# davidnabergoj/nfmc

Hardware: AMD Instinct MI355X
Metric: chain-steps/sec (n_chains x iters / s), jump_mala + RealNVP, d=64 (higher is better)
Workload: dtype f32

## Files before the change

### include/nfmc_hip.h

```cpp
#ifndef NFMC_HIP_H
#define NFMC_HIP_H

#include <stdint.h>

#ifdef __cplusplus
extern "C" {
#endif

typedef void* nfmc_stream_t;

#define NFMC_ABI_VERSION 4

enum {
    NFMC_OK = 0,
    NFMC_EINVAL = -1,
    NFMC_ESHAPE = -2,
    NFMC_EALIGN = -3,
    NFMC_EUNSUPPORTED = -4,
    NFMC_ESCRATCH = -5
};

enum {
    NFMC_POT_QUADRATIC = 0,
    NFMC_POT_FUNNEL = 1,
    NFMC_POT_GAUSSIAN_MIXTURE = 2,
    NFMC_POT_LOGISTIC_REGRESSION = 3,
    NFMC_POT_GAUSSIAN_FULL = 4,
    NFMC_POT_ROSENBROCK = 5,
    NFMC_POT_STOCHASTIC_VOLATILITY = 6,
    NFMC_POT_SPARSE_LOGISTIC_REGRESSION = 7,
    NFMC_POT_LATTICE_PHI4 = 8,
    NFMC_POT_ITEM_RESPONSE = 9,
    NFMC_POT_VARYING_EFFECTS = 10,
    NFMC_POT_PARTICLES = 11,
    NFMC_POT_LATENT_GAUSSIAN = 12
};

typedef struct {
    int32_t kind;
    int32_t n_components;
    const float* a;
    const float* b;
    float a_scalar;
    float b_scalar;
} NfmcPotential;

typedef struct {
    uint64_t seed;
    uint64_t chain_offset;
    uint32_t step0;
    uint32_t rounds;
    const float* replay_normals;
    const float* replay_uniforms;
} NfmcRng;

enum { NFMC_CNT_ACCEPTED = 0, NFMC_CNT_ATTEMPTED = 1, NFMC_CNT_NONFINITE = 2, NFMC_CNT_WORDS = 4 };

typedef struct {
    double* sum_x;
    double* sum_x2;
    unsigned long long* counters;
    double* scratch;
    int64_t scratch_bytes;
    int32_t defer;
    int32_t tail_slot;
} NfmcStats;

int64_t nfmc_stats_scratch_bytes(int32_t d);

int nfmc_stats_fold_f32(const NfmcStats* stats, int32_t d, uint64_t attempted, unsigned long long* jump_counters,
                        uint64_t jump_attempted, nfmc_stream_t stream);

typedef struct {
    int32_t d;
    int32_t n_coupling;
    int32_t n_hidden;
    int32_t n_hidden_layers;
    float min_scale;
    int32_t n_bins;
    const float* ea0_log_scale;
    const float* ea0_shift;
    const float* ea1_log_scale;
    const float* ea1_shift;
    const float* weights;
    int64_t layer_stride;
    float spline_bound;
    int32_t reserved;
    float* scratch;
    int64_t scratch_bytes;
} NfmcRealNVP;

int64_t nfmc_flow_scratch_bytes(const NfmcRealNVP* flow, int64_t n, int32_t with_gradient);

int32_t nfmc_realnvp_padded_hidden(int32_t n_hidden);
int64_t nfmc_realnvp_layer_floats(int32_t d, int32_t n_hidden, int32_t n_hidden_layers);
int64_t nfmc_coupling_layer_floats(int32_t d, int32_t n_hidden, int32_t n_hidden_layers, int32_t n_bins);

typedef struct {
    float* base;
    int32_t stride;
    int32_t countdown;
    int32_t ring_rows;
    int32_t row;
} NfmcSampleStore;

enum {
    NFMC_TUNE_STEP_SIZE = 0,
    NFMC_TUNE_LOG_SMOOTH = 1,
    NFMC_TUNE_ERROR_SUM = 2,
    NFMC_TUNE_ITERATION = 3,
    NFMC_TUNE_ANCHOR = 4,
    NFMC_TUNE_LOG_RAW = 5,
    NFMC_TUNE_TARGET = 6,
    NFMC_TUNE_KAPPA = 7,
    NFMC_TUNE_GAMMA = 8,
    NFMC_TUNE_IMD_ADJUSTMENT = 9,
    NFMC_TUNE_TICKET = 10,
    NFMC_TUNE_WORDS = 12
};
typedef struct {
    double* state;
    float* inv_mass_diag;
    int32_t tune_step_size;
    int32_t tune_inv_mass_diag;
    int32_t every;
    int32_t reserved;
} NfmcTune;
int64_t nfmc_tune_state_doubles(int32_t d);

int nfmc_sampler_layout(int32_t d, int32_t pot_kind, int32_t* cpl, int32_t* lpc);

typedef struct {
    NfmcRealNVP flow;
    int32_t adjusted;
    int32_t reserved;
    unsigned long long* counters;
    const float* replay_latent;
    const float* replay_uniform;
    uint8_t* mask_out;
    float* log_ratio_out;
} NfmcJumpTail;

typedef struct {
    float* x;
    int64_t n;
    int32_t d;
    int32_t n_steps;
    float step_size;
    int32_t adjust;
    const float* inv_mass_diag;
    NfmcPotential pot;
    NfmcRng rng;
    NfmcStats stats;
    NfmcSampleStore samples;
    uint8_t* masks_out;
    float* log_ratio_out;
    const NfmcJumpTail* jump;
    NfmcTune tune;
} NfmcMalaArgs;

int nfmc_mala_steps_f32(const NfmcMalaArgs* args, nfmc_stream_t stream);

typedef struct {
    float* x;
    int64_t n;
    int32_t d;
    int32_t n_steps;
    float step_size;
    int32_t n_leapfrog;
    int32_t adjust;
    int32_t reserved;
    const float* inv_mass_diag;
    NfmcPotential pot;
    NfmcRng rng;
    NfmcStats stats;
    NfmcSampleStore samples;
    uint8_t* masks_out;
    float* log_ratio_out;
    const NfmcJumpTail* jump;
    NfmcTune tune;
} NfmcHmcArgs;

int nfmc_hmc_steps_f32(const NfmcHmcArgs* args, nfmc_stream_t stream);

int nfmc_realnvp_forward_f32(const NfmcRealNVP* flow, const float* x, int64_t n, float* z, float* logdet,
                             float* log_prob, nfmc_stream_t stream);

int nfmc_realnvp_inverse_f32(const NfmcRealNVP* flow, const float* z, int64_t n, float* x, float* logdet,
                             float* log_q, const NfmcRng* rng, nfmc_stream_t stream);

typedef struct {
    float* x;
    float* logq;
    int64_t n;
    int32_t n_steps;
    int32_t logq_cached;
    int32_t adjusted;
    int32_t reserved;
    NfmcRealNVP flow;
    NfmcPotential pot;
    NfmcRng rng;
    NfmcStats stats;
    NfmcSampleStore samples;
    uint8_t* masks_out;
    float* log_ratio_out;
} NfmcFlowMhArgs;

int nfmc_flow_mh_steps_f32(const NfmcFlowMhArgs* args, nfmc_stream_t stream);

int nfmc_flow_mh_supported_f32(const NfmcFlowMhArgs* args);

enum { NFMC_INNER_MALA = 0, NFMC_INNER_HMC = 1 };
#define NFMC_JUMP_RUN_MAX_PARTS 4
typedef struct {
    int32_t inner_kind;
    int32_t n_parts;
    const void* inner;
    const NfmcFlowMhArgs* jump;
    int32_t n_outer;
    int32_t n_inner;
} NfmcJumpRun;

int nfmc_jump_run_f32(const NfmcJumpRun* run, nfmc_stream_t stream);

#define NFMC_IMH_PARALLEL_MAX_STEPS 65536
int64_t nfmc_imh_parallel_work_bytes(int64_t n, int32_t d, int32_t n_steps);
int nfmc_imh_parallel_f32(const NfmcFlowMhArgs* args, void* work, int64_t work_bytes, nfmc_stream_t stream);
int nfmc_imh_parallel_supported_f32(const NfmcFlowMhArgs* args);

typedef struct {
    float* z;
    int64_t n;
    int32_t n_steps;
    int32_t n_leapfrog;
    float step_size;
    int32_t adjust;
    const float* inv_mass_diag;
    NfmcRealNVP flow;
    NfmcPotential pot;
    NfmcRng rng;
    NfmcStats stats;
    NfmcSampleStore samples;
    uint8_t* masks_out;
    float* log_ratio_out;
    float* scratch;
    int64_t scratch_bytes;
} NfmcNeutraHmcArgs;

int64_t nfmc_neutra_scratch_bytes(int64_t n, int32_t d, int32_t n_hidden, int32_t n_hidden_layers, int32_t n_coupling);

int nfmc_neutra_hmc_steps_f32(const NfmcNeutraHmcArgs* args, nfmc_stream_t stream);

int nfmc_neutra_potential_grad_f32(const NfmcRealNVP* flow, const NfmcPotential* pot, const float* z, int64_t n,
                                   float* u_out, float* grad_out, nfmc_stream_t stream);

typedef struct {
    NfmcRealNVP flow;
    const float* x;
    int64_t n;
    float* grad_out;
    float* logq_out;
} NfmcFlowLogqGradArgs;

int nfmc_flow_logq_grad_f32(const NfmcFlowLogqGradArgs* args, nfmc_stream_t stream);
int nfmc_flow_logq_grad_supported_f32(const NfmcFlowLogqGradArgs* args);

typedef struct {
    NfmcRealNVP flow;
    NfmcPotential pot;
    float* x;
    const float* grad_u;
    float* logq_out;
    int64_t n;
    float step_size;
    int32_t reserved;
} NfmcDlmcStepArgs;

int nfmc_dlmc_step_f32(const NfmcDlmcStepArgs* args, nfmc_stream_t stream);
int nfmc_dlmc_step_supported_f32(const NfmcDlmcStepArgs* args);

typedef struct {
    float* x;
    const float* x_prime;
    int64_t n;
    int32_t d;
    int32_t n_carry;
    const float* log_ratio;
    const float* uniforms;
    float* carry[2];
    const float* carry_prime[2];
    NfmcRng rng;
    int32_t rng_tag;
    int32_t reserved;
    NfmcStats stats;
    uint8_t* mask_out;
} NfmcSelectArgs;

int nfmc_mh_accept_select_f32(const NfmcSelectArgs* args, nfmc_stream_t stream);

int nfmc_langevin_propose_f32(const float* x, const float* grad_u, const float* inv_mass_diag, float step_size,
                              int64_t n, int32_t d, const NfmcRng* rng, float* x_prime, nfmc_stream_t stream);
int nfmc_langevin_log_ratio_f32(const float* x, const float* x_prime, const float* u, const float* u_prime,
                                const float* grad_u, const float* grad_u_prime, const float* inv_mass_diag,
                                float step_size, int64_t n, int32_t d, float* log_ratio, nfmc_stream_t stream);

int nfmc_moments_update_f32(const float* x, int64_t rows, int32_t d, const NfmcStats* stats, nfmc_stream_t stream);

int nfmc_philox_normals_f32(const NfmcRng* rng, int32_t tag, int64_t n, int32_t d, float* out, nfmc_stream_t stream);
int nfmc_philox_uniforms_f32(const NfmcRng* rng, int32_t tag, int64_t n, float* out, nfmc_stream_t stream);

#define NFMC_MAX_STEPS_PER_CALL 512
typedef struct {
    float lr, beta1, beta2, eps, weight_decay;
    int32_t step;
} NfmcAdamW;

typedef struct {
    NfmcRealNVP flow;
    float* params;
    float* adam_m;
    float* adam_v;
    int64_t n_params;
    int64_t ea_off;
    float* partial;
    int64_t partial_floats;
    float* status;
    const float* x_val;
    int64_t n_val;
    float* params_prev;
    float* best;
    float* run_state;
    float* scratch;
    int64_t scratch_bytes;
} NfmcFlowFit;

typedef struct {
    int32_t n_epochs;
    int32_t early_stopping;
    int32_t early_stopping_threshold;
    int32_t keep_best_weights;
    int32_t skip_nonfinite;
    int32_t reserved;
} NfmcFitControl;
enum {
    NFMC_FIT_BEST_LOSS = 0,
    NFMC_FIT_SINCE_BEST = 1,
    NFMC_FIT_APPLIED = 2,
    NFMC_FIT_STOPPED = 3,
    NFMC_FIT_DIVERGED = 4,
    NFMC_FIT_LAST_LOSS = 5,
    NFMC_FIT_LAST_VAL = 6,
    NFMC_FIT_BOOKED = 7,
    NFMC_FIT_STATE_FLOATS = 8
};

int nfmc_flow_fit_supported_f32(const NfmcRealNVP* flow);
int64_t nfmc_flow_fit_partial_floats(int64_t n, int64_t n_params);
int64_t nfmc_flow_fit_workspace(const NfmcRealNVP* flow, int64_t n, int64_t n_val, int64_t n_params, int64_t* partial_floats);
int nfmc_flow_fit_step_f32(const NfmcFlowFit* fit, const float* x, int64_t n, const NfmcAdamW* opt, nfmc_stream_t stream);
int nfmc_flow_variational_fit_step_f32(const NfmcFlowFit* fit, const NfmcPotential* pot, const float* z, int64_t n,
                                       const NfmcAdamW* opt, nfmc_stream_t stream);
int nfmc_flow_fit_epochs_f32(const NfmcFlowFit* fit, const NfmcPotential* pot, const float* x, int64_t n,
                             int64_t epoch_stride, const NfmcAdamW* opt, const NfmcFitControl* ctl, int32_t first_call,
                             int32_t n_calls, nfmc_stream_t stream);

#define NFMC_BLOB_MAX_PIECES 16
typedef struct {
    float* param;
    int64_t vec_off;
    int32_t rows, cols;
    int32_t vec_row_stride, vec_col_stride;
} NfmcBlobPiece;
int nfmc_flow_blob_copy_f32(float* vec, const NfmcBlobPiece* pieces, int32_t n_pieces, int32_t to_vector, nfmc_stream_t stream);

#define NFMC_PRP_ROUNDS 6
int nfmc_rows_sample_f32(const float* x, int64_t n, int32_t d, uint64_t seed, int64_t first, float* out, int64_t m,
                         int64_t* index_out, nfmc_stream_t stream);
int64_t nfmc_rows_sample_index(int64_t n, uint64_t seed, int64_t i);

typedef struct {
    int32_t abi_version;
    int32_t max_d_sampler;
    int32_t max_d_flow;
    int32_t max_hidden_valu;
    int32_t max_hidden;
    int32_t max_steps_per_call;
} NfmcLimits;

int nfmc_limits(NfmcLimits* out);
const char* nfmc_error_string(int code);
const char* nfmc_build_digest(void);

#ifdef __cplusplus
}
#endif
#endif
```

### nfmc_amd/csrc/misc_kernels.hip

```cpp
#include "common.hpp"

namespace nfmc {

__global__ void __launch_bounds__(kBlock) philox_normals_kernel(NfmcRng rng, uint32_t tag, int64_t n, int d, int nblk,
                                                                float* __restrict__ out) {
    const int64_t total = n * nblk;
    for (int64_t t = (int64_t)blockIdx.x * kBlock + threadIdx.x; t < total; t += (int64_t)gridDim.x * kBlock) {
        const int64_t row = t / nblk;
        const int blk = (int)(t - row * nblk);
        float z[4];
        if (rng.rounds == 7)
            philox_normal4<7>((uint32_t)(rng.chain_offset + (uint64_t)row), rng.step0, (uint32_t)blk, tag, (uint32_t)rng.seed,
                              (uint32_t)(rng.seed >> 32), z);
        else
            philox_normal4<10>((uint32_t)(rng.chain_offset + (uint64_t)row), rng.step0, (uint32_t)blk, tag, (uint32_t)rng.seed,
                               (uint32_t)(rng.seed >> 32), z);
#pragma unroll
        for (int k = 0; k < 4; ++k)
            if (4 * blk + k < d) out[row * d + 4 * blk + k] = z[k];
    }
}

__device__ __forceinline__ float stream_uniform(const NfmcRng& rng, uint32_t tag, int64_t row) {
    const uint32_t gchain = (uint32_t)(rng.chain_offset + (uint64_t)row);
    const uint32_t k0 = (uint32_t)rng.seed, k1 = (uint32_t)(rng.seed >> 32);
    const bool r7 = rng.rounds == 7;
    if (tag == kTagAccept) {
        const uint4 r = r7 ? philox4x32<7>(gchain, rng.step0 >> 2, 0u, kTagAccept, k0, k1)
                           : philox4x32<10>(gchain, rng.step0 >> 2, 0u, kTagAccept, k0, k1);
        return u32_to_uniform(pick_word(r, rng.step0 & 3u));
    }
    const uint4 r = r7 ? philox4x32<7>(gchain, rng.step0, 0u, tag, k0, k1) : philox4x32<10>(gchain, rng.step0, 0u, tag, k0, k1);
    return u32_to_uniform(r.x);
}

__global__ void __launch_bounds__(kBlock) philox_uniforms_kernel(NfmcRng rng, uint32_t tag, int64_t n,
                                                                 float* __restrict__ out) {
    for (int64_t row = (int64_t)blockIdx.x * kBlock + threadIdx.x; row < n; row += (int64_t)gridDim.x * kBlock)
        out[row] = stream_uniform(rng, tag, row);
}

__global__ void __launch_bounds__(kBlock) moments_kernel(const float* __restrict__ x, int64_t rows, int d, int dp,
                                                         double* __restrict__ scratch) {
    const int64_t per = (rows + gridDim.x - 1) / gridDim.x;
    const int64_t r0 = (int64_t)blockIdx.x * per;
    const int64_t r1 = r0 + per < rows ? r0 + per : rows;
    double* out = scratch + (size_t)blockIdx.x * (2 * dp + kStatTail);
    for (int c = threadIdx.x; c < dp; c += kBlock) {
        double s = 0.0, s2 = 0.0;
        if (c < d)
            for (int64_t r = r0; r < r1; ++r) {
                const float v = x[r * d + c];
                s += (double)v;
                s2 += (double)v * (double)v;
            }
        out[c] = s;
        out[dp + c] = s2;
    }
    if (threadIdx.x < kStatTail) out[2 * dp + threadIdx.x] = 0.0;
}

template <int CPL, int LPC>
__global__ void __launch_bounds__(kBlock) select_kernel(NfmcSelectArgs a, int64_t tiles) {
    constexpr int CPW = kWave / LPC;
    const int lane = threadIdx.x & 63, wave = threadIdx.x >> 6;
    const int g = lane % LPC, cw = lane / LPC;
    const int d = a.d;
    float sx[CPL], sxx[CPL];
#pragma unroll
    for (int i = 0; i < CPL; ++i) sx[i] = sxx[i] = 0.f;
    uint32_t n_acc = 0, n_bad = 0;
    for (int64_t tile = blockIdx.x; tile < tiles; tile += gridDim.x) {
        const int64_t row = (tile * kWavesPerBlock + wave) * CPW + cw;
        const bool active = row < a.n;
        bool accept = active;
        if (a.log_ratio && active) {
            const float lr = a.log_ratio[row];
            const float u = a.uniforms ? a.uniforms[row] : stream_uniform(a.rng, (uint32_t)a.rng_tag, row);
            accept = fast_ln(u) < lr;
            if (g == 0 && !(fabsf(lr) <= 3.0e38f)) n_bad++;
        }
        float x[CPL], xp[CPL];
        load_row<CPL, LPC, false>(a.x, row, d, g, active, x);
        load_row<CPL, LPC, false>(a.x_prime, row, d, g, active, xp);
        const uint64_t am = __ballot(accept);
#pragma unroll
        for (int i = 0; i < CPL; ++i) {
            x[i] = select_f32(am, xp[i], x[i]);
            sx[i] += x[i];
            sxx[i] = fmaf(x[i], x[i], sxx[i]);
        }
        if (accept) store_row<CPL, LPC, false>(a.x, row, d, g, true, x);
        if (g == 0 && active) {
            if (accept) {
                n_acc++;
                for (int k = 0; k < a.n_carry; ++k) a.carry[k][row] = a.carry_prime[k][row];
            }
            if (a.mask_out) a.mask_out[row] = accept ? 1 : 0;
        }
    }
    for (int m = 1; m < kWave; m <<= 1) {
        n_acc += __shfl_xor(n_acc, m, kWave);
        n_bad += __shfl_xor(n_bad, m, kWave);
    }
    if (a.stats.sum_x) block_stats_flush<CPL, LPC>(sx, sxx, n_acc, n_bad, a.stats);
}

__global__ void __launch_bounds__(kBlock) langevin_propose_kernel(const float* __restrict__ x,
                                                                  const float* __restrict__ grad_u,
                                                                  const float* __restrict__ imd, float h, float sqrt2h,
                                                                  int64_t n, int d, NfmcRng rng,
                                                                  float* __restrict__ x_prime) {
    const int nblk = (d + 3) / 4;
    const int64_t total = n * nblk;
    for (int64_t t = (int64_t)blockIdx.x * kBlock + threadIdx.x; t < total; t += (int64_t)gridDim.x * kBlock) {
        const int64_t row = t / nblk;
        const int blk = (int)(t - row * nblk);
        float z[4];
        if (rng.replay_normals) {
#pragma unroll
            for (int k = 0; k < 4; ++k) z[k] = (4 * blk + k < d) ? rng.replay_normals[row * d + 4 * blk + k] : 0.f;
        } else {
            philox_normal4((uint32_t)(rng.chain_offset + (uint64_t)row), rng.step0, (uint32_t)blk, kTagNoise,
                           (uint32_t)rng.seed, (uint32_t)(rng.seed >> 32), z);
        }
#pragma unroll
        for (int k = 0; k < 4; ++k) {
            const int c = 4 * blk + k;
            if (c < d) {
                const float m = imd ? imd[c] : 1.f;
                const int64_t o = row * d + c;
                x_prime[o] = fmaf(sqrt2h / m, z[k], fmaf((-h) / (m * m), grad_u[o], x[o]));
            }
        }
    }
}

__global__ void __launch_bounds__(kBlock) langevin_log_ratio_kernel(
    const float* __restrict__ x, const float* __restrict__ xp, const float* __restrict__ u,
    const float* __restrict__ up, const float* __restrict__ gu, const float* __restrict__ gup,
    const float* __restrict__ imd, float h, int64_t n, int d, float* __restrict__ out) {
    const int lane = threadIdx.x & 63;
    const int64_t wid = ((int64_t)blockIdx.x * kBlock + threadIdx.x) >> 6;
    const int64_t nw = ((int64_t)gridDim.x * kBlock) >> 6;
    const float inv4h = 1.f / (4.f * h);
    for (int64_t row = wid; row < n; row += nw) {
        float acc = 0.f;
        for (int c = lane; c < d; c += kWave) {
            const float m = imd ? imd[c] : 1.f;
            const float A = 1.f / (m * m);
            const int64_t o = row * d + c;
            const float tf = (xp[o] - x[o]) + h * A * gu[o];
            const float tb = (x[o] - xp[o]) + h * A * gup[o];
            acc += inv4h * (1.f / A) * (tf * tf - tb * tb);
        }
        acc = group_allreduce<64>(acc);
        if (lane == 0) out[row] = (u[row] - up[row]) + acc;
    }
}

static int grid_for(int64_t work_items) {
    int64_t g = (work_items + kBlock - 1) / kBlock;
    return (int)(g < 1 ? 1 : (g > kMaxGrid ? kMaxGrid : g));
}

}

using namespace nfmc;

extern "C" int nfmc_philox_normals_f32(const NfmcRng* rng, int32_t tag, int64_t n, int32_t d, float* out,
                                       nfmc_stream_t stream) {
    if (!rng || !out || n <= 0 || d <= 0 || !rng_rounds_ok(*rng, true)) return NFMC_EINVAL;
    const int nblk = (d + 3) / 4;
    hipLaunchKernelGGL(philox_normals_kernel, dim3(grid_for(n * nblk)), dim3(kBlock), 0, (hipStream_t)stream, *rng,
                       (uint32_t)tag, n, d, nblk, out);
    NFMC_HIP_CHECK_LAUNCH();
    return NFMC_OK;
}

extern "C" int nfmc_philox_uniforms_f32(const NfmcRng* rng, int32_t tag, int64_t n, float* out, nfmc_stream_t stream) {
    if (!rng || !out || n <= 0 || !rng_rounds_ok(*rng, true)) return NFMC_EINVAL;
    if (tag != (int)kTagAccept && tag != (int)kTagJump) return NFMC_EINVAL;
    hipLaunchKernelGGL(philox_uniforms_kernel, dim3(grid_for(n)), dim3(kBlock), 0, (hipStream_t)stream, *rng,
                       (uint32_t)tag, n, out);
    NFMC_HIP_CHECK_LAUNCH();
    return NFMC_OK;
}

extern "C" int nfmc_moments_update_f32(const float* x, int64_t rows, int32_t d, const NfmcStats* stats,
                                       nfmc_stream_t stream) {
    if (!x || !stats || !stats->sum_x || !stats->sum_x2 || !stats->counters || !stats->scratch) return NFMC_EINVAL;
    if (rows <= 0 || d <= 0) return NFMC_EINVAL;
    if (d > 1024) return NFMC_ESHAPE;
    const int dp = padded_d(d);
    int grid = (int)(rows < 1024 ? (rows + 3) / 4 : 256);
    if (grid < 1) grid = 1;
    if (stats->scratch_bytes < (int64_t)grid * (2 * dp + kStatTail) * (int64_t)sizeof(double)) return NFMC_ESCRATCH;
    if (stats->defer) return NFMC_EUNSUPPORTED;
    hipStream_t st = (hipStream_t)stream;
    hipLaunchKernelGGL(moments_kernel, dim3(grid), dim3(kBlock), 0, st, x, rows, (int)d, dp, stats->scratch);
    NFMC_HIP_CHECK_LAUNCH();
    hipLaunchKernelGGL(stats_finish_kernel<true>, dim3(stats_finish_grid(dp)), dim3(kFinishBlock), 0, st, stats->scratch, grid, dp, (int)d, *stats, 0ull);
    NFMC_HIP_CHECK_LAUNCH();
    return NFMC_OK;
}

extern "C" int nfmc_stats_fold_f32(const NfmcStats* stats, int32_t d, uint64_t attempted,
                                   unsigned long long* jump_counters, uint64_t jump_attempted, nfmc_stream_t stream) {
    if (!stats || !stats->sum_x || !stats->sum_x2 || !stats->counters || !stats->scratch) return NFMC_EINVAL;
    if (d <= 0) return NFMC_EINVAL;
    if (d > 1024) return NFMC_ESHAPE;
    const int dp = padded_d(d);
    if (stats->scratch_bytes < stats_scratch_doubles(dp) * (int64_t)sizeof(double)) return NFMC_ESCRATCH;
    hipLaunchKernelGGL(stats_finish_kernel<true>, dim3(stats_finish_grid(dp)), dim3(kFinishBlock), 0, (hipStream_t)stream,
                       stats->scratch, kMaxGrid, dp, (int)d, *stats, (unsigned long long)attempted, jump_counters,
                       (unsigned long long)jump_attempted);
    NFMC_HIP_CHECK_LAUNCH();
    return NFMC_OK;
}

template <int CPL, int LPC>
static void launch_select(const NfmcSelectArgs& a, int64_t tiles, int grid, hipStream_t st) {
    hipLaunchKernelGGL((select_kernel<CPL, LPC>), dim3(grid), dim3(kBlock), 0, st, a, tiles);
}

extern "C" int nfmc_mh_accept_select_f32(const NfmcSelectArgs* args, nfmc_stream_t stream) {
    if (!args || !args->x || !args->x_prime) return NFMC_EINVAL;
    NfmcSelectArgs a = *args;
    if (a.n <= 0 || a.d <= 0 || a.n_carry < 0 || a.n_carry > 2) return NFMC_EINVAL;
    if (int rr = rng_default_only(a.rng)) return rr;
    if (a.d > 1024) return NFMC_ESHAPE;
    for (int k = 0; k < a.n_carry; ++k)
        if (!a.carry[k] || !a.carry_prime[k]) return NFMC_EINVAL;
    if (a.stats.sum_x && (!a.stats.sum_x2 || !a.stats.counters || !a.stats.scratch)) return NFMC_EINVAL;
    if (a.rng_tag != (int)kTagAccept && a.rng_tag != (int)kTagJump) return NFMC_EINVAL;
    const int dp = padded_d(a.d);
    const int lpc = dp / 4 > 64 ? 64 : dp / 4;
    const int cpl = dp / lpc;
    const int cpw = kWave / lpc;
    const int64_t tiles = (a.n + (int64_t)kWavesPerBlock * cpw - 1) / ((int64_t)kWavesPerBlock * cpw);
    const int grid = (int)(tiles < kMaxGrid ? tiles : kMaxGrid);
    if (a.stats.sum_x && a.stats.scratch_bytes < (int64_t)grid * (2 * dp + kStatTail) * (int64_t)sizeof(double))
        return NFMC_ESCRATCH;
    if (check_defer(a.stats, dp, a.d)) return NFMC_EINVAL;
    hipStream_t st = (hipStream_t)stream;
    if (cpl == 4) {
        switch (lpc) {
            case 1: launch_select<4, 1>(a, tiles, grid, st); break;
            case 2: launch_select<4, 2>(a, tiles, grid, st); break;
            case 4: launch_select<4, 4>(a, tiles, grid, st); break;
            case 8: launch_select<4, 8>(a, tiles, grid, st); break;
            case 16: launch_select<4, 16>(a, tiles, grid, st); break;
            case 32: launch_select<4, 32>(a, tiles, grid, st); break;
            default: launch_select<4, 64>(a, tiles, grid, st); break;
        }
    } else if (cpl == 8) {
        launch_select<8, 64>(a, tiles, grid, st);
    } else {
        launch_select<16, 64>(a, tiles, grid, st);
    }
    NFMC_HIP_CHECK_LAUNCH();
    if (a.stats.sum_x && !a.stats.defer) {
        hipLaunchKernelGGL(stats_finish_kernel<true>, dim3(stats_finish_grid(dp)), dim3(kFinishBlock), 0, st, a.stats.scratch, grid, dp, a.d, a.stats,
                           (unsigned long long)a.n);
        NFMC_HIP_CHECK_LAUNCH();
    }
    return NFMC_OK;
}

extern "C" int nfmc_langevin_propose_f32(const float* x, const float* grad_u, const float* inv_mass_diag,
                                         float step_size, int64_t n, int32_t d, const NfmcRng* rng, float* x_prime,
                                         nfmc_stream_t stream) {
    if (!x || !grad_u || !rng || !x_prime || n <= 0 || d <= 0 || !(step_size > 0.f)) return NFMC_EINVAL;
    if (int rr = rng_default_only(*rng)) return rr;
    const float sqrt2h = (float)sqrt(2.0 * (double)step_size);
    hipLaunchKernelGGL(langevin_propose_kernel, dim3(grid_for(n * ((d + 3) / 4))), dim3(kBlock), 0, (hipStream_t)stream,
                       x, grad_u, inv_mass_diag, step_size, sqrt2h, n, (int)d, *rng, x_prime);
    NFMC_HIP_CHECK_LAUNCH();
    return NFMC_OK;
}

extern "C" int nfmc_langevin_log_ratio_f32(const float* x, const float* x_prime, const float* u, const float* u_prime,
                                           const float* grad_u, const float* grad_u_prime, const float* inv_mass_diag,
                                           float step_size, int64_t n, int32_t d, float* log_ratio,
                                           nfmc_stream_t stream) {
    if (!x || !x_prime || !u || !u_prime || !grad_u || !grad_u_prime || !log_ratio) return NFMC_EINVAL;
    if (n <= 0 || d <= 0 || !(step_size > 0.f)) return NFMC_EINVAL;
    hipLaunchKernelGGL(langevin_log_ratio_kernel, dim3(grid_for(n * 64)), dim3(kBlock), 0, (hipStream_t)stream, x,
                       x_prime, u, u_prime, grad_u, grad_u_prime, inv_mass_diag, step_size, n, (int)d, log_ratio);
    NFMC_HIP_CHECK_LAUNCH();
    return NFMC_OK;
}

extern "C" int nfmc_limits(NfmcLimits* out) {
    if (!out) return NFMC_EINVAL;
    out->abi_version = NFMC_ABI_VERSION;
    out->max_d_sampler = 1024;
    out->max_d_flow = 512;
    out->max_hidden_valu = 32;
    out->max_hidden = 128;
    out->max_steps_per_call = NFMC_MAX_STEPS_PER_CALL;
    return NFMC_OK;
}

extern "C" const char* nfmc_error_string(int code) {
    switch (code) {
        case NFMC_OK: return "ok";
        case NFMC_EINVAL: return "invalid argument (NULL pointer or non-positive size)";
        case NFMC_ESHAPE: return "shape outside the supported range (see nfmc_limits)";
        case NFMC_EALIGN: return "pointer alignment";
        case NFMC_EUNSUPPORTED: return "no kernel for this request";
        case NFMC_ESCRATCH: return "statistics scratch buffer too small (nfmc_stats_scratch_bytes)";
        default: return code > 0 ? hipGetErrorString((hipError_t)code) : "unknown nfmc error";
    }
}
```

### nfmc_amd/csrc/sampler_impl.hpp

```cpp
#pragma once

#include "flow_b.hpp"

namespace nfmc {

template <int CPL, int LPC, bool FAST>
struct MassCoef {
    float c1_s, c2_s, hA_s, cg_s, kap_s;
    float c1[FAST ? 1 : CPL], c2[FAST ? 1 : CPL], hA[FAST ? 1 : CPL], invA[FAST ? 1 : CPL];
    float m[FAST ? 1 : CPL], rs[FAST ? 1 : CPL], cg[FAST ? 1 : CPL], kap[FAST ? 1 : CPL];

    template <class PotT>
    __device__ __forceinline__ void init_quadratic(const PotT& pot, bool rw) {
        cg_s = rw ? 0.f : c1_s * (2.f * pot.aa(0));
        kap_s = rw ? pot.aa(0) : pot.aa(0) * pot.aa(0) * hA_s;
        if constexpr (!FAST) {
#pragma unroll
            for (int i = 0; i < CPL; ++i) {
                cg[i] = rw ? 0.f : c1[i] * (2.f * pot.aa(i));
                kap[i] = rw ? pot.aa(i) : pot.aa(i) * pot.aa(i) * hA[i];
            }
        }
    }
    __device__ __forceinline__ float CG(int i) const { return FAST ? cg_s : cg[FAST ? 0 : i]; }
    __device__ __forceinline__ float KAP(int i) const { return FAST ? kap_s : kap[FAST ? 0 : i]; }

    __device__ __forceinline__ void init(float h, float sqrt2h, const float* __restrict__ imd, int g, int d,
                                         bool rw = false) {
        c1_s = rw ? 0.f : -h;
        c2_s = rw ? 1.f : sqrt2h;
        hA_s = h;
        if constexpr (!FAST) {
#pragma unroll
            for (int i = 0; i < CPL; ++i) {
                const int c = coord_of<CPL, LPC>(g, i);
                const bool ok = c < d;
                const float mm = (ok && imd) ? imd[c] : 1.f;
                const float A = 1.f / (mm * mm);
                c1[i] = (ok && !rw) ? (-h) / (mm * mm) : 0.f;
                c2[i] = ok ? (rw ? mm : sqrt2h / mm) : 0.f;
                hA[i] = ok ? h * A : 0.f;
                invA[i] = ok ? 1.f / A : 0.f;
                m[i] = ok ? mm : 0.f;
                rs[i] = ok ? 1.f / sqrtf(mm) : 0.f;
            }
        }
    }
    __device__ __forceinline__ float C1(int i) const { return FAST ? c1_s : c1[FAST ? 0 : i]; }
    __device__ __forceinline__ float C2(int i) const { return FAST ? c2_s : c2[FAST ? 0 : i]; }
    __device__ __forceinline__ float HA(int i) const { return FAST ? hA_s : hA[FAST ? 0 : i]; }
    __device__ __forceinline__ float IA(int i) const { return FAST ? 1.f : invA[FAST ? 0 : i]; }
    __device__ __forceinline__ float M(int i) const { return FAST ? 1.f : m[FAST ? 0 : i]; }
    __device__ __forceinline__ float RS(int i) const { return FAST ? 1.f : rs[FAST ? 0 : i]; }
};

template <int CPL, int LPC, bool ON>
struct StatShift {
    float c[ON ? CPL : 1];
    __device__ __forceinline__ void init(const NfmcTune& tn, int g, int d, bool active) {
        if constexpr (ON) {
            const double* __restrict__ src = tn.state + NFMC_TUNE_WORDS + 2 * CPL * LPC + kStatTail;
#pragma unroll
            for (int i = 0; i < CPL; ++i) {
                const int k = coord_of<CPL, LPC>(g, i);
                c[i] = (active && k < d) ? (float)src[k] : 0.f;
            }
        }
    }
    __device__ __forceinline__ float operator()(const float (&x)[CPL], int i) const {
        if constexpr (ON) return x[i] - c[i];
        else return x[i];
    }
};

template <int CPL, int LPC, int R = 10, bool REPLAY = true>
__device__ __forceinline__ void draw_normals(const NfmcRng& rng, uint32_t tag, uint32_t gchain, int64_t row, int64_t n,
                                             int d, int g, int s, float (&e)[CPL]) {
    if (REPLAY && rng.replay_normals) {
        const float* p = rng.replay_normals + ((int64_t)s * n + row) * d;
#pragma unroll
        for (int i = 0; i < CPL; ++i) {
            const int c = coord_of<CPL, LPC>(g, i);
            e[i] = (row < n && c < d) ? p[c] : 0.f;
        }
    } else {
        const uint32_t k0 = (uint32_t)rng.seed, k1 = (uint32_t)(rng.seed >> 32);
#pragma unroll
        for (int b = 0; b < CPL / 4; ++b) {
            const uint4 r = philox4x32<R, true>(gchain, rng.step0 + (uint32_t)s, (uint32_t)(b * LPC + g), tag, k0, k1);
            const nfmc_f2 z0 = box_muller_pk(r.x, r.y), z1 = box_muller_pk(r.z, r.w);
            e[4 * b] = z0.x;
            e[4 * b + 1] = z0.y;
            e[4 * b + 2] = z1.x;
            e[4 * b + 3] = z1.y;
        }
    }
}

template <int LPC, int R = 10, bool REPLAY = true>
struct AcceptLnU {
    uint4 r;
    float4* mine;
    const float* chain;
    uint32_t base;
    __device__ __forceinline__ AcceptLnU(float4* slab, int g) {
        if constexpr (LPC > 1) {
            mine = slab + threadIdx.x;
            chain = reinterpret_cast<const float*>(slab + (threadIdx.x - g));
        }
    }
    __device__ __forceinline__ float draw(const NfmcRng& rng, uint32_t gchain, int64_t row, int64_t n, int g, int s) {
        if (REPLAY && rng.replay_uniforms) return fast_ln(row < n ? rng.replay_uniforms[(int64_t)s * n + row] : 0.5f);
        const uint32_t step = rng.step0 + (uint32_t)s, k0 = (uint32_t)rng.seed, k1 = (uint32_t)(rng.seed >> 32);
        if constexpr (LPC == 1) {
            if (s == 0 || (step & 3u) == 0u) r = philox4x32<R>(gchain, step >> 2, 0u, kTagAccept, k0, k1);
            return fast_ln(u32_to_uniform(pick_word(r, step & 3u)));
        } else {
            if (s == 0 || step - base == 4u * LPC || step == 0u) {
                base = step & ~3u;
                const uint4 w = philox4x32<R>(gchain, (base >> 2) + (uint32_t)g, 0u, kTagAccept, k0, k1);
                *mine = make_float4(fast_ln(u32_to_uniform(w.x)), fast_ln(u32_to_uniform(w.y)),
                                    fast_ln(u32_to_uniform(w.z)), fast_ln(u32_to_uniform(w.w)));
                __builtin_amdgcn_wave_barrier();
            }
            return chain[step - base];
        }
    }
};

struct JumpDev {
    NfmcRealNVP flow;
    int adjusted;
    const float* replay_latent;
    const float* replay_uniform;
    uint8_t* mask_out;
    float* log_ratio_out;
};

template <int CPL, int LPC, int HP, class FlowT, class PotT>
__device__ __forceinline__ bool jump_once(float (&x)[CPL], const FlowT& fl, const PotT& pot,
                                          const JumpDev& j, uint64_t seed, uint32_t step, uint32_t gchain, int64_t row,
                                          int64_t n, int d, int g, bool active, float& lr_out, bool& bad) {
    const bool revl = (j.flow.n_coupling & 1) != 0;
    float part;
    {
        const auto ctx = pot.prepare(x, g, d);
        float w[CPL];
        part = 0.f;
#pragma unroll
        for (int i = 0; i < CPL; ++i) {
            part += pot.term(ctx, i, x[i]);
            w[i] = x[i];
        }
        part += fl.forward(w);
#pragma unroll
        for (int i = 0; i < CPL; ++i) part = fmaf(-0.5f * w[i], w[i], part);
    }
    float xp[CPL];
    draw_latent<CPL, LPC>(xp, j.replay_latent, seed, step, gchain, row, n, d, g, revl);
#pragma unroll
    for (int i = 0; i < CPL; ++i) part = fmaf(0.5f * xp[i], xp[i], part);
    part += fl.inverse(xp);
    {
        const auto ctx = pot.prepare(xp, g, d);
#pragma unroll
        for (int i = 0; i < CPL; ++i) part -= pot.term(ctx, i, xp[i]);
    }
    const float lr = group_allreduce<LPC>(part);
    bool accept = true;
    bad = false;
    if (j.adjusted) {
        float u;
        if (j.replay_uniform) {
            u = active ? j.replay_uniform[row] : 0.5f;
        } else {
            const uint4 r = philox4x32_10(gchain, step, 0u, kTagJump, (uint32_t)seed, (uint32_t)(seed >> 32));
            u = u32_to_uniform(r.x);
        }
        accept = fast_ln(u) < lr;
        bad = active && !(fabsf(lr) <= 3.0e38f);
    }
    accept = accept && active;
    const uint64_t am = __ballot(accept);
#pragma unroll
    for (int i = 0; i < CPL; ++i) x[i] = select_f32(am, xp[i], x[i]);
    lr_out = lr;
    return accept;
}

template <int CPL, int LPC, template <int, int, bool> class Pot, bool FAST, int JHP, int RR = 10, bool LEAN = false,
          bool TUNE = false>
__global__ void __launch_bounds__(kBlock, NFMC_WPE) mala_kernel(NfmcMalaArgs a, float sqrt2h, int64_t tiles, JumpDev jd) {
    static_assert(!LEAN || JHP == 0, "the jump tail keeps its own outputs");
    static_assert(!TUNE || (JHP == 0 && !FAST && !LEAN), "tuning launches run the general kernels without a jump tail");
    extern __shared__ __attribute__((aligned(16))) float flow_lds[];
    __shared__ float4 accept_slab[LPC > 1 ? kBlock : 1];
    constexpr int CPW = kWave / LPC;
    const int lane = threadIdx.x & 63, wave = threadIdx.x >> 6;
    const int g = lane % LPC, cw = lane / LPC;
    const int d = a.d;
    const int64_t n = a.n;
    const double h_dev = a.tune.state ? a.tune.state[NFMC_TUNE_STEP_SIZE] : 0.0;
    const float h = a.tune.state ? (float)h_dev : a.step_size;
    if (a.tune.state) sqrt2h = (float)sqrt(2.0 * h_dev);
    const bool adjust = (a.adjust & 1) != 0, rw = (a.adjust & 2) != 0;
    const float inv4h = rw ? 0.f : 1.f / (4.f * h);

    MassCoef<CPL, LPC, FAST> mc;
    mc.init(h, sqrt2h, a.inv_mass_diag, g, d, rw);
    Pot<CPL, LPC, FAST> pot;
    if constexpr (!Pot<CPL, LPC, FAST>::kStaged) pot.init(a.pot, g, d);
    if constexpr (Pot<CPL, LPC, FAST>::kQuadratic) mc.init_quadratic(pot, rw);
    FlowB<CPL, LPC, JHP == 0 ? 4 : JHP, true, (FAST && CPL >= 8 && JHP > 0)> fl;
    if constexpr (JHP > 0) {
        decltype(fl)::Img::stage(flow_lds, jd.flow, kBlock);
        __syncthreads();
        fl.init(flow_lds, jd.flow, g);
    }
    if constexpr (Pot<CPL, LPC, FAST>::kStaged)
        init_staged(pot, a.pot, g, d, flow_lds,
                    JHP > 0 ? decltype(fl)::Img::total_floats(jd.flow.n_hidden_layers, jd.flow.n_coupling) : 0);

    float sx[CPL], sxx[CPL];
#pragma unroll
    for (int i = 0; i < CPL; ++i) sx[i] = sxx[i] = 0.f;
    StatShift<CPL, LPC, TUNE> shift;
    uint32_t n_acc = 0, n_bad = 0, j_acc = 0, j_bad = 0;
    constexpr unsigned long long leaders = group_leaders(LPC);

    for (int64_t tile = blockIdx.x; tile < tiles; tile += gridDim.x) {
        const int64_t row = (tile * kWavesPerBlock + wave) * CPW + cw;
        const bool active = row < n;
        const uint32_t gchain = (uint32_t)(a.rng.chain_offset + (uint64_t)row);
        float x[CPL];
        load_row<CPL, LPC, FAST>(a.x, row, d, g, active, x);
        shift.init(a.tune, g, d, active);
        AcceptLnU<LPC, RR, !LEAN> au(accept_slab, g);
        StoreCursor keep(a.samples);
        const uint64_t live = __ballot(active);
        float sq = 0.f, sq_prop = 0.f;
        if constexpr (Pot<CPL, LPC, FAST>::kQuadratic && FAST) {
#pragma unroll
            for (int i = 0; i < CPL; ++i) sq = fmaf(x[i], x[i], sq);
        }

        for (int s = 0; s < a.n_steps; ++s) {
            float e[CPL], xp[CPL];
            draw_normals<CPL, LPC, RR, !LEAN>(a.rng, kTagNoise, gchain, row, n, d, g, s, e);
            float lr = 0.f;
            if constexpr (Pot<CPL, LPC, FAST>::kQuadratic && FAST) {
                nfmc_f2 sp = {0.f, 0.f};
                const nfmc_f2 cg = {mc.CG(0), mc.CG(0)}, c2 = {mc.C2(0), mc.C2(0)};
#pragma unroll
                for (int i = 0; i < CPL; i += 2) {
                    const nfmc_f2 xi = {x[i], x[i + 1]}, ei = {e[i], e[i + 1]};
                    const nfmc_f2 p = __builtin_elementwise_fma(c2, ei, __builtin_elementwise_fma(cg, xi, xi));
                    xp[i] = p.x;
                    xp[i + 1] = p.y;
                    sp = __builtin_elementwise_fma(p, p, sp);
                }
                sq_prop = sp.x + sp.y;
                {
#pragma clang fp contract(off)
                    lr = mc.KAP(0) * (sq - sq_prop);
                }
            } else if constexpr (Pot<CPL, LPC, FAST>::kQuadratic) {
#pragma unroll
                for (int i = 0; i < CPL; ++i) {
                    const float t = x[i] - pot.bb(i);
                    xp[i] = fmaf(mc.C2(i), e[i], fmaf(mc.CG(i), t, x[i]));
                    const float tp = xp[i] - pot.bb(i);
                    lr = fmaf(mc.KAP(i) * (t - tp), t + tp, lr);
                }
            } else {
                const auto ctx = pot.prepare(x, g, d);
#pragma unroll
                for (int i = 0; i < CPL; ++i)
                    xp[i] = fmaf(mc.C2(i), e[i], fmaf(mc.C1(i), pot.grad(ctx, i, x[i]), x[i]));
                if (adjust) {
                    const auto ctxp = pot.prepare(xp, g, d);
#pragma unroll
                    for (int i = 0; i < CPL; ++i) {
                        const float gj = pot.grad(ctx, i, x[i]), gp = pot.grad(ctxp, i, xp[i]);
                        const float tf = (xp[i] - x[i]) + mc.HA(i) * gj;
                        const float tb = (x[i] - xp[i]) + mc.HA(i) * gp;
                        lr += (pot.term(ctx, i, x[i]) - pot.term(ctxp, i, xp[i])) +
                              inv4h * mc.IA(i) * (tf * tf - tb * tb);
                    }
                }
            }
            uint64_t am = live;
            if (adjust) {
                lr = group_allreduce<LPC, Pot<CPL, LPC, FAST>::kQuadratic && FAST>(lr);
                const float ln_u = au.draw(a.rng, gchain, row, n, g, s);
                am &= __ballot(ln_u < lr);
                n_bad += (uint32_t)__popcll(__ballot(!(fabsf(lr) <= 3.0e38f)) & live & leaders);
            }
            n_acc += (uint32_t)__popcll(am & leaders);
            if constexpr (Pot<CPL, LPC, FAST>::kQuadratic && FAST) assign_where<CPL>(am, x, xp, sq, sq_prop);
#pragma unroll
            for (int i = 0; i < CPL; ++i) {
                if constexpr (!(Pot<CPL, LPC, FAST>::kQuadratic && FAST)) x[i] = select_f32(am, xp[i], x[i]);
                const float xs = shift(x, i);
                sx[i] += xs;
                sxx[i] = fmaf(xs, xs, sxx[i]);
            }
            if constexpr (!LEAN) {
                if (float* kept = keep.next(n * d)) store_row<CPL, LPC, FAST>(kept, row, d, g, active, x);
                if (g == 0 && active) {
                    if (a.masks_out) a.masks_out[(int64_t)s * n + row] = (am >> lane) & 1u;
                    if (a.log_ratio_out) a.log_ratio_out[(int64_t)s * n + row] = lr;
                }
            }
        }
        if constexpr (JHP > 0) {
            float lr;
            bool bad;
            fl.launder();
            const bool acc = jump_once<CPL, LPC, JHP>(x, fl, pot, jd, a.rng.seed, a.rng.step0 + (uint32_t)a.n_steps, gchain,
                                                      row, n, d, g, active, lr, bad);
            j_acc += (uint32_t)__popcll(__ballot(acc) & leaders);
            j_bad += (uint32_t)__popcll(__ballot(bad) & leaders);
#pragma unroll
            for (int i = 0; i < CPL; ++i) {
                const float xs = shift(x, i);
                sx[i] += xs;
                sxx[i] = fmaf(xs, xs, sxx[i]);
            }
            if (float* kept = keep.next(n * d)) store_row<CPL, LPC, FAST>(kept, row, d, g, active, x);
            if (g == 0 && active) {
                if (jd.mask_out) jd.mask_out[row] = acc ? 1 : 0;
                if (jd.log_ratio_out) jd.log_ratio_out[row] = lr;
            }
        }
        store_row<CPL, LPC, FAST>(a.x, row, d, g, active, x);
    }
    if (a.stats.sum_x) block_stats_flush<CPL, LPC>(sx, sxx, n_acc, n_bad, a.stats, j_acc, j_bad);
}

template <int CPL, int LPC, template <int, int, bool> class Pot, bool FAST, int JHP, int RR = 10, bool TUNE = false>
__global__ void __launch_bounds__(kBlock, NFMC_WPE) hmc_kernel(NfmcHmcArgs a, int64_t tiles, JumpDev jd) {
    static_assert(!TUNE || (JHP == 0 && !FAST), "tuning launches run the general kernels without a jump tail");
    extern __shared__ __attribute__((aligned(16))) float flow_lds[];
    __shared__ float4 accept_slab[LPC > 1 ? kBlock : 1];
    constexpr int CPW = kWave / LPC;
    const int lane = threadIdx.x & 63, wave = threadIdx.x >> 6;
    const int g = lane % LPC, cw = lane / LPC;
    const int d = a.d;
    const int64_t n = a.n;
    const float h = a.tune.state ? (float)a.tune.state[NFMC_TUNE_STEP_SIZE] : a.step_size, hh = h / 2;

    MassCoef<CPL, LPC, FAST> mc;
    mc.init(h, 0.f, a.inv_mass_diag, g, d);
    Pot<CPL, LPC, FAST> pot;
    if constexpr (!Pot<CPL, LPC, FAST>::kStaged) pot.init(a.pot, g, d);
    FlowB<CPL, LPC, JHP == 0 ? 4 : JHP, true, (FAST && CPL >= 8 && JHP > 0)> fl;
    if constexpr (JHP > 0) {
        decltype(fl)::Img::stage(flow_lds, jd.flow, kBlock);
        __syncthreads();
        fl.init(flow_lds, jd.flow, g);
    }
    if constexpr (Pot<CPL, LPC, FAST>::kStaged)
        init_staged(pot, a.pot, g, d, flow_lds,
                    JHP > 0 ? decltype(fl)::Img::total_floats(jd.flow.n_hidden_layers, jd.flow.n_coupling) : 0);

    float sx[CPL], sxx[CPL];
#pragma unroll
    for (int i = 0; i < CPL; ++i) sx[i] = sxx[i] = 0.f;
    StatShift<CPL, LPC, TUNE> shift;
    uint32_t n_acc = 0, n_bad = 0, j_acc = 0, j_bad = 0;
    constexpr unsigned long long leaders = group_leaders(LPC);

    for (int64_t tile = blockIdx.x; tile < tiles; tile += gridDim.x) {
        const int64_t row = (tile * kWavesPerBlock + wave) * CPW + cw;
        const bool active = row < n;
        const uint32_t gchain = (uint32_t)(a.rng.chain_offset + (uint64_t)row);
        float x[CPL];
        load_row<CPL, LPC, FAST>(a.x, row, d, g, active, x);
        shift.init(a.tune, g, d, active);
        AcceptLnU<LPC, RR> au(accept_slab, g);
        StoreCursor keep(a.samples);

        for (int s = 0; s < a.n_steps; ++s) {
            float p[CPL], q[CPL];
            draw_normals<CPL, LPC, RR>(a.rng, kTagNoise, gchain, row, n, d, g, s, p);
            float dh = 0.f;
            {
                const auto ctx = pot.prepare(x, g, d);
#pragma unroll
                for (int i = 0; i < CPL; ++i) {
                    p[i] *= mc.RS(i);
                    q[i] = x[i];
                    dh += pot.term(ctx, i, x[i]) + 0.5f * (p[i] * p[i] * mc.M(i));
                }
            }
            if constexpr (Pot<CPL, LPC, FAST>::kQuadratic && FAST) {
                const float cq = hh * (2.f * pot.aa(0)), cq2 = 2.f * cq;
                const int L = a.n_leapfrog;
                if (L > 0) {
#pragma unroll
                    for (int i = 0; i < CPL; ++i) p[i] = fmaf(-cq, q[i], p[i]);
                    for (int l = 0; l + 1 < L; ++l) {
#pragma unroll
                        for (int i = 0; i < CPL; ++i) {
                            q[i] = fmaf(h, p[i], q[i]);
                            p[i] = fmaf(-cq2, q[i], p[i]);
                        }
                    }
#pragma unroll
                    for (int i = 0; i < CPL; ++i) {
                        q[i] = fmaf(h, p[i], q[i]);
                        p[i] = fmaf(-cq, q[i], p[i]);
                    }
                }
            } else {
                const int L = a.n_leapfrog;
                if (L > 0) {
                    const auto c0 = pot.prepare(q, g, d);
#pragma unroll
                    for (int i = 0; i < CPL; ++i) p[i] = fmaf(-hh, pot.grad(c0, i, q[i]), p[i]);
                    for (int l = 0; l < L; ++l) {
#pragma unroll
                        for (int i = 0; i < CPL; ++i) q[i] = fmaf(h, p[i] * mc.M(i), q[i]);
                        const auto c1 = pot.prepare(q, g, d);
                        const float hs = l + 1 < L ? h : hh;
#pragma unroll
                        for (int i = 0; i < CPL; ++i) p[i] = fmaf(-hs, pot.grad(c1, i, q[i]), p[i]);
                    }
                }
            }
            bool accept = true;
            float lr = 0.f;
            if (a.adjust) {
                const auto ctx = pot.prepare(q, g, d);
#pragma unroll
                for (int i = 0; i < CPL; ++i) dh -= pot.term(ctx, i, q[i]) + 0.5f * (p[i] * p[i] * mc.M(i));
                lr = group_allreduce<LPC>(dh);
                accept = au.draw(a.rng, gchain, row, n, g, s) < lr;
                n_bad += (uint32_t)__popcll(__ballot(active && !(fabsf(lr) <= 3.0e38f)) & leaders);
            }
            accept = accept && active;
            const uint64_t am = __ballot(accept);
            n_acc += (uint32_t)__popcll(am & leaders);
#pragma unroll
            for (int i = 0; i < CPL; ++i) {
                x[i] = select_f32(am, q[i], x[i]);
                const float xs = shift(x, i);
                sx[i] += xs;
                sxx[i] = fmaf(xs, xs, sxx[i]);
            }
            if (float* kept = keep.next(n * d)) store_row<CPL, LPC, FAST>(kept, row, d, g, active, x);
            if (g == 0 && active) {
                if (a.masks_out) a.masks_out[(int64_t)s * n + row] = accept ? 1 : 0;
                if (a.log_ratio_out) a.log_ratio_out[(int64_t)s * n + row] = lr;
            }
        }
        if constexpr (JHP > 0) {
            float lr;
            bool bad;
            fl.launder();
            const bool acc = jump_once<CPL, LPC, JHP>(x, fl, pot, jd, a.rng.seed, a.rng.step0 + (uint32_t)a.n_steps, gchain,
                                                      row, n, d, g, active, lr, bad);
            j_acc += (uint32_t)__popcll(__ballot(acc) & leaders);
            j_bad += (uint32_t)__popcll(__ballot(bad) & leaders);
#pragma unroll
            for (int i = 0; i < CPL; ++i) {
                const float xs = shift(x, i);
                sx[i] += xs;
                sxx[i] = fmaf(xs, xs, sxx[i]);
            }
            if (float* kept = keep.next(n * d)) store_row<CPL, LPC, FAST>(kept, row, d, g, active, x);
            if (g == 0 && active) {
                if (jd.mask_out) jd.mask_out[row] = acc ? 1 : 0;
                if (jd.log_ratio_out) jd.log_ratio_out[row] = lr;
            }
        }
        store_row<CPL, LPC, FAST>(a.x, row, d, g, active, x);
    }
    if (a.stats.sum_x) block_stats_flush<CPL, LPC>(sx, sxx, n_acc, n_bad, a.stats, j_acc, j_bad);
}


struct Cfg {
    int cpl, lpc;
};

constexpr bool is_default_cfg(int cpl, int lpc) {
    return !((cpl == 4 && lpc == 16) || (cpl == 16 && lpc != 64));
}
template <int CPL, int LPC, int JHP>
constexpr bool cfg_instantiated(int kind) {
    return !pot_kind(kind)->own_units && (JHP > 0 || is_default_cfg(CPL, LPC) || !pot_kind(kind)->default_cfg_only);
}

template <int CPL, int LPC, int JHP>
size_t sampler_lds(const NfmcPotential& p, const JumpDev& jd) {
    size_t lds = 0;
    if constexpr (JHP > 0)
        lds = (size_t)FlowImage<CPL, LPC, JHP>::total_floats(jd.flow.n_hidden_layers, jd.flow.n_coupling) * sizeof(float);
    return lds_with_potential(lds, p, CPL, LPC);
}

template <int CPL, int LPC, template <int, int, bool> class POT, bool F, int JHP>
int launch_mala_kernel(const NfmcMalaArgs& a, const JumpDev& jd, size_t lds, int64_t tiles, int grid, float sqrt2h,
                       hipStream_t st) {
    auto kern = mala_kernel<CPL, LPC, POT, F, JHP>;
    if constexpr (JHP == 0 && !F) {
        if (a.tune.state) kern = mala_kernel<CPL, LPC, POT, F, JHP, 10, false, true>;
    }
    return launch_lds(kern, grid, kBlock, lds, st, a, sqrt2h, tiles, jd);
}

template <int CPL, int LPC, template <int, int, bool> class POT, bool F, int JHP>
int launch_hmc_kernel(const NfmcHmcArgs& a, const JumpDev& jd, size_t lds, int64_t tiles, int grid, hipStream_t st) {
    auto kern = hmc_kernel<CPL, LPC, POT, F, JHP>;
    if constexpr (JHP == 0 && !F) {
        if (a.tune.state) kern = hmc_kernel<CPL, LPC, POT, F, JHP, 10, true>;
    }
    return launch_lds(kern, grid, kBlock, lds, st, a, tiles, jd);
}

template <int CPL, int LPC, int JHP>
int launch_mala_cfg(const NfmcMalaArgs& a, const JumpDev& jd, bool fast, int64_t tiles, int grid, float sqrt2h,
                    hipStream_t st) {
    const size_t lds = sampler_lds<CPL, LPC, JHP>(a.pot, jd);
    if (lds > 120 * 1024 || !cfg_instantiated<CPL, LPC, JHP>(a.pot.kind)) return NFMC_EUNSUPPORTED;
    const bool lean = !a.masks_out && !a.log_ratio_out && !a.samples.base && !a.rng.replay_normals && !a.rng.replay_uniforms;
#define NFMC_L(POT, F) return launch_mala_kernel<CPL, LPC, POT, F, JHP>(a, jd, lds, tiles, grid, sqrt2h, st);
    if (rng_rounds(a.rng) == 7) {
        if constexpr (JHP == 0) {
            if (fast && a.pot.kind == NFMC_POT_QUADRATIC) {
                auto kern = lean ? mala_kernel<CPL, LPC, QuadraticPot, true, 0, 7, true>
                                 : mala_kernel<CPL, LPC, QuadraticPot, true, 0, 7>;
                hipLaunchKernelGGL(kern, dim3(grid), dim3(kBlock), lds, st, a, sqrt2h, tiles, jd);
                return NFMC_OK;
            }
        }
        return NFMC_EUNSUPPORTED;
    }
    if (a.pot.kind == NFMC_POT_GAUSSIAN_MIXTURE) {
        NFMC_L(MixturePot, false)
    } else if (a.pot.kind == NFMC_POT_LOGISTIC_REGRESSION) {
        if constexpr (cfg_instantiated<CPL, LPC, JHP>(NFMC_POT_LOGISTIC_REGRESSION)) NFMC_L(LogRegPot, false)
    } else if (a.pot.kind == NFMC_POT_FUNNEL) {
        if (fast) NFMC_L(FunnelPot, true) else NFMC_L(FunnelPot, false)
    } else {
        if constexpr (JHP == 0) {
            if (fast && lean) {
                auto kern = mala_kernel<CPL, LPC, QuadraticPot, true, 0, 10, true>;
                hipLaunchKernelGGL(kern, dim3(grid), dim3(kBlock), lds, st, a, sqrt2h, tiles, jd);
                return NFMC_OK;
            }
        }
        if (fast) NFMC_L(QuadraticPot, true) else NFMC_L(QuadraticPot, false)
    }
#undef NFMC_L
    return NFMC_EUNSUPPORTED;
}

template <int CPL, int LPC, int JHP>
int launch_hmc_cfg(const NfmcHmcArgs& a, const JumpDev& jd, bool fast, int64_t tiles, int grid, hipStream_t st) {
    const size_t lds = sampler_lds<CPL, LPC, JHP>(a.pot, jd);
    if (lds > 120 * 1024 || !cfg_instantiated<CPL, LPC, JHP>(a.pot.kind)) return NFMC_EUNSUPPORTED;
#define NFMC_L(POT, F) return launch_hmc_kernel<CPL, LPC, POT, F, JHP>(a, jd, lds, tiles, grid, st);
    if (rng_rounds(a.rng) == 7) {
        if constexpr (JHP == 0) {
            if (fast && a.pot.kind == NFMC_POT_QUADRATIC) {
                auto kern = hmc_kernel<CPL, LPC, QuadraticPot, true, 0, 7>;
                hipLaunchKernelGGL(kern, dim3(grid), dim3(kBlock), lds, st, a, tiles, jd);
                return NFMC_OK;
            }
        }
        return NFMC_EUNSUPPORTED;
    }
    if (a.pot.kind == NFMC_POT_GAUSSIAN_MIXTURE) {
        NFMC_L(MixturePot, false)
    } else if (a.pot.kind == NFMC_POT_LOGISTIC_REGRESSION) {
        if constexpr (cfg_instantiated<CPL, LPC, JHP>(NFMC_POT_LOGISTIC_REGRESSION)) NFMC_L(LogRegPot, false)
    } else if (a.pot.kind == NFMC_POT_FUNNEL) {
        if (fast) NFMC_L(FunnelPot, true) else NFMC_L(FunnelPot, false)
    } else {
        if (fast) NFMC_L(QuadraticPot, true) else NFMC_L(QuadraticPot, false)
    }
#undef NFMC_L
    return NFMC_EUNSUPPORTED;
}

#define NFMC_FOR_CFG(M)                                                                                             \
    M(4, 1) M(4, 2) M(4, 4) M(4, 8) M(4, 16) M(8, 8) M(16, 4) M(8, 16) M(16, 8) M(8, 32) M(16, 16) M(8, 64) M(16, 32) \
        M(16, 64)
#define NFMC_FOR_DEFAULT_CFG(M) M(4, 1) M(4, 2) M(4, 4) M(4, 8) M(8, 8) M(8, 16) M(8, 32) M(8, 64) M(16, 64)
#define NFMC_FOR_JUMP_CFG(M) M(4, 1) M(4, 2) M(4, 4) M(4, 8) M(8, 8) M(8, 16) M(8, 32) M(8, 64)
#define NFMC_CFG_ENTRY(CPL, LPC) {CPL, LPC},
constexpr Cfg kJumpCfgs[] = {NFMC_FOR_JUMP_CFG(NFMC_CFG_ENTRY)};

template <template <int, int, bool> class POT>
int launch_mala_kind(const NfmcMalaArgs& a, const JumpDev& jd, Cfg c, int jhp, int64_t tiles, int grid, float sqrt2h,
                     hipStream_t st) {
    if (rng_rounds(a.rng) != 10) return NFMC_EUNSUPPORTED;
#define NFMC_AT(JHP, CPL, LPC)                                                       \
    if (jhp == JHP && c.cpl == CPL && c.lpc == LPC) {                                \
        const size_t lds = sampler_lds<CPL, LPC, JHP>(a.pot, jd);                    \
        if (lds > 120 * 1024) return NFMC_EUNSUPPORTED;                              \
        return launch_mala_kernel<CPL, LPC, POT, false, JHP>(a, jd, lds, tiles, grid, sqrt2h, st); \
    }
#define M0(CPL, LPC) NFMC_AT(0, CPL, LPC)
#define M4(CPL, LPC) NFMC_AT(4, CPL, LPC)
#define M8(CPL, LPC) NFMC_AT(8, CPL, LPC)
    NFMC_FOR_DEFAULT_CFG(M0) NFMC_FOR_JUMP_CFG(M4) NFMC_FOR_JUMP_CFG(M8)
#undef NFMC_AT
    return NFMC_EUNSUPPORTED;
}
template <template <int, int, bool> class POT>
int launch_hmc_kind(const NfmcHmcArgs& a, const JumpDev& jd, Cfg c, int jhp, int64_t tiles, int grid, hipStream_t st) {
    if (rng_rounds(a.rng) != 10) return NFMC_EUNSUPPORTED;
#define NFMC_AT(JHP, CPL, LPC)                                                       \
    if (jhp == JHP && c.cpl == CPL && c.lpc == LPC) {                                \
        const size_t lds = sampler_lds<CPL, LPC, JHP>(a.pot, jd);                    \
        if (lds > 120 * 1024) return NFMC_EUNSUPPORTED;                              \
        return launch_hmc_kernel<CPL, LPC, POT, false, JHP>(a, jd, lds, tiles, grid, st); \
    }
    NFMC_FOR_DEFAULT_CFG(M0) NFMC_FOR_JUMP_CFG(M4) NFMC_FOR_JUMP_CFG(M8)
#undef NFMC_AT
#undef M0
#undef M4
#undef M8
    return NFMC_EUNSUPPORTED;
}
#define NFMC_EXTERN_KIND(KIND, POT)                                                                                       \
    static_assert(kPotKinds[KIND].own_units, #POT);                                                                       \
    extern template int launch_mala_kind<POT>(const NfmcMalaArgs&, const JumpDev&, Cfg, int, int64_t, int, float, hipStream_t); \
    extern template int launch_hmc_kind<POT>(const NfmcHmcArgs&, const JumpDev&, Cfg, int, int64_t, int, hipStream_t);
NFMC_FOR_OWN_UNIT_POT(NFMC_EXTERN_KIND)
#undef NFMC_EXTERN_KIND

int launch_mala_j0(const NfmcMalaArgs&, const JumpDev&, Cfg, bool, int64_t, int, float, hipStream_t);
int launch_mala_j4(const NfmcMalaArgs&, const JumpDev&, Cfg, bool, int64_t, int, float, hipStream_t);
int launch_mala_j8(const NfmcMalaArgs&, const JumpDev&, Cfg, bool, int64_t, int, float, hipStream_t);
int launch_hmc_j0(const NfmcHmcArgs&, const JumpDev&, Cfg, bool, int64_t, int, hipStream_t);
int launch_hmc_j4(const NfmcHmcArgs&, const JumpDev&, Cfg, bool, int64_t, int, hipStream_t);
int launch_hmc_j8(const NfmcHmcArgs&, const JumpDev&, Cfg, bool, int64_t, int, hipStream_t);

}
```

### nfmc_amd/csrc/sampler_kernels.hip

```cpp
#include <mutex>

#include "run_parts.hpp"
#include "sampler_impl.hpp"

namespace nfmc {

static const Cfg kCfgs[] = {{4, 1}, {4, 2}, {4, 4}, {4, 8}, {8, 8}, {4, 16}, {16, 4}, {8, 16}, {16, 8}, {8, 32}, {16, 16}, {8, 64}, {16, 32}, {16, 64}};

static Cfg choose_cfg(int d, bool with_jump, bool default_only) {
    const Cfg* list = with_jump ? kJumpCfgs : kCfgs;
    const int len = with_jump ? (int)(sizeof(kJumpCfgs) / sizeof(Cfg)) : (int)(sizeof(kCfgs) / sizeof(Cfg));
    int c = 0, l = 0;
    const char* e = getenv("NFMC_SAMPLER_CFG");
    const bool named = e && sscanf(e, "%d,%d", &c, &l) == 2 && (!default_only || is_default_cfg(c, l));
    Cfg best = {0, 0};
    for (int i = 0; i < len; ++i) {
        const Cfg& k = list[i];
        if (k.cpl * k.lpc < d) continue;
        if (named && k.cpl == c && k.lpc == l) return k;
        if (best.cpl == 0 || k.cpl * k.lpc < best.cpl * best.lpc) best = k;
    }
    return best;
}

static bool aligned16(const void* p) { return ((uintptr_t)p & 15u) == 0; }

template <class Args>
static int check_common(const Args* a) {
    if (!a || !a->x) return NFMC_EINVAL;
    if (a->n <= 0 || a->d <= 0 || a->n_steps <= 0) return NFMC_EINVAL;
    if (a->n_steps > NFMC_MAX_STEPS_PER_CALL) return NFMC_ESHAPE;
    if (a->d > 1024) return NFMC_ESHAPE;
    if (!(a->step_size > 0.f)) return NFMC_EINVAL;
    if (int rc = check_potential(a->pot, a->d, PotFamily::kRegister)) return rc;
    if (((uintptr_t)a->x & 3u) != 0) return NFMC_EALIGN;
    if (!store_ok(a->samples)) return NFMC_EINVAL;
    if (!rng_rounds_ok(a->rng, true)) return NFMC_EINVAL;
    if ((a->rng.replay_normals == nullptr) != (a->rng.replay_uniforms == nullptr) && (a->adjust & 1)) return NFMC_EINVAL;
    if (a->stats.sum_x && (!a->stats.sum_x2 || !a->stats.counters || !a->stats.scratch)) return NFMC_EINVAL;
    if (a->jump) {
        const NfmcJumpTail& j = *a->jump;
        if (j.flow.d != a->d || !j.counters) return NFMC_EINVAL;
        if (!j.flow.ea0_log_scale || !j.flow.ea0_shift || !j.flow.ea1_log_scale || !j.flow.ea1_shift) return NFMC_EINVAL;
        if (j.flow.n_coupling > 0 && !j.flow.weights) return NFMC_EINVAL;
        if (j.flow.n_hidden <= 0 || j.flow.n_hidden_layers <= 0) return NFMC_EINVAL;
        if (j.flow.n_hidden > 8 || a->d > 512 || j.flow.n_bins != 0) return NFMC_EUNSUPPORTED;
        if (!a->stats.sum_x) return NFMC_EINVAL;
        if (j.adjusted && (j.replay_latent != nullptr) != (j.replay_uniform != nullptr)) return NFMC_EINVAL;
    }
    return NFMC_OK;
}

template <class Args>
static bool fast_path(const Args* a, const Cfg& c) {
    return a->d == c.cpl * c.lpc && a->inv_mass_diag == nullptr && a->pot.a == nullptr && a->pot.b == nullptr &&
           (a->pot.kind != NFMC_POT_QUADRATIC || a->pot.b_scalar == 0.f) && aligned16(a->x) &&
           (!a->samples.base || aligned16(a->samples.base));
}

constexpr int kTuneGrid = 256;
template <int NCHUNK>
__global__ void __launch_bounds__(kFinishBlock) tune_finish_kernel(double* __restrict__ scratch, int nblocks, int dp, int d,
                                                                   NfmcStats st, NfmcTune tn, unsigned long long attempted) {
    __shared__ double part[kFinishSlices][kFinishCols];
    const int width = 2 * dp + kStatTail;
    const int col = threadIdx.x % kFinishCols, slice = threadIdx.x / kFinishCols;
    double* __restrict__ totals = tn.state + NFMC_TUNE_WORDS;
    constexpr int kGroups = 5, kRows = 8;
    for (int t0 = 0; t0 < width; t0 += kGroups * kFinishCols) {
        double acc[kGroups];
#pragma unroll
        for (int gi = 0; gi < kGroups; ++gi) acc[gi] = 0.0;
#pragma unroll
        for (int r0 = 0; r0 < NCHUNK * kRows * kFinishSlices; r0 += kRows * kFinishSlices) {
            double v[kGroups][kRows];
#pragma unroll
            for (int gi = 0; gi < kGroups; ++gi) {
                const int t = t0 + gi * kFinishCols + col;
#pragma unroll
                for (int u = 0; u < kRows; ++u) {
                    const int b = r0 + slice + u * kFinishSlices;
                    v[gi][u] = (t < width && b < nblocks) ? scratch[(size_t)b * width + t] : 0.0;
                }
            }
#pragma unroll
            for (int gi = 0; gi < kGroups; ++gi) {
                const int t = t0 + gi * kFinishCols + col;
#pragma unroll
                for (int u = 0; u < kRows; ++u) acc[gi] += v[gi][u];
#pragma unroll
                for (int u = 0; u < kRows; ++u) {
                    const int b = r0 + slice + u * kFinishSlices;
                    if (t < width && b < nblocks) scratch[(size_t)b * width + t] = 0.0;
                }
            }
            __builtin_amdgcn_sched_barrier(0);
        }
#pragma unroll
        for (int gi = 0; gi < kGroups; ++gi) {
            const int t = t0 + gi * kFinishCols + col;
            const double p0 = acc[gi];
            __syncthreads();
            part[slice][col] = p0;
            __syncthreads();
            if (slice == 0 && t < width) {
                double s = 0.0;
#pragma unroll
                for (int k = 0; k < kFinishSlices; ++k) s += part[k][col];
                totals[t] = s;
                if (t == 2 * dp) {
                    st.counters[NFMC_CNT_ACCEPTED] += (unsigned long long)(s + 0.5);
                    st.counters[NFMC_CNT_ATTEMPTED] += attempted;
                } else if (t == 2 * dp + 1) {
                    st.counters[NFMC_CNT_NONFINITE] += (unsigned long long)(s + 0.5);
                }
            }
        }
    }
    __syncthreads();
    const double n_tot = (double)attempted;
    double* __restrict__ shift = tn.state + NFMC_TUNE_WORDS + 2 * dp + kStatTail;
    const bool tune_imd = tn.tune_inv_mass_diag && tn.inv_mass_diag && n_tot > 1.0;
    const double beta = tn.state[NFMC_TUNE_IMD_ADJUSTMENT];
    for (int j = threadIdx.x; j < d; j += kFinishBlock) {
        const double c = shift[j], s1 = totals[j], s2 = totals[dp + j];
        st.sum_x[j] += s1 + n_tot * c;
        st.sum_x2[j] += s2 + c * (2.0 * s1 + n_tot * c);
        if (tune_imd) {
            double var = (s2 - s1 * s1 / n_tot) / (n_tot - 1.0);
            var = var > 0.0 ? var : 0.0;
            tn.inv_mass_diag[j] = (float)(beta * var + (1.0 - beta) * (double)tn.inv_mass_diag[j]);
        }
        if (n_tot > 0.0) shift[j] = (double)(float)(c + s1 / n_tot);
    }
    if (threadIdx.x == 0 && tn.tune_step_size) {
        const double acc = totals[2 * dp];
        const double err = tn.state[NFMC_TUNE_TARGET] - acc / n_tot;
        const double S = tn.state[NFMC_TUNE_ERROR_SUM] + err;
        const double it = tn.state[NFMC_TUNE_ITERATION];
        const double log_raw = tn.state[NFMC_TUNE_ANCHOR] - S / (sqrt(it) * tn.state[NFMC_TUNE_GAMMA]);
        const double w = pow(it, -tn.state[NFMC_TUNE_KAPPA]);
        const double log_smooth = w * log_raw + (1.0 - w) * tn.state[NFMC_TUNE_LOG_SMOOTH];
        tn.state[NFMC_TUNE_ERROR_SUM] = S;
        tn.state[NFMC_TUNE_LOG_RAW] = log_raw;
        tn.state[NFMC_TUNE_LOG_SMOOTH] = log_smooth;
        tn.state[NFMC_TUNE_ITERATION] = it + 1.0;
        tn.state[NFMC_TUNE_STEP_SIZE] = exp(log_smooth);
    }
}

constexpr int kTuneFoldSlabs = 128, kTuneFoldWgs = 16;
__global__ void __launch_bounds__(kFinishBlock) tune_fold_kernel(double* __restrict__ scratch, int nblocks, int width,
                                                                 double* __restrict__ partial) {
    __shared__ double part[kFinishSlices][kFinishCols];
    const int col = threadIdx.x % kFinishCols, slice = threadIdx.x / kFinishCols;
    const int b0 = blockIdx.x * kTuneFoldSlabs;
    double* __restrict__ dst = partial + (size_t)blockIdx.x * width;
    constexpr int kGroups = 5, kRows = kTuneFoldSlabs / kFinishSlices;
    for (int t0 = 0; t0 < width; t0 += kGroups * kFinishCols) {
        double v[kGroups][kRows];
#pragma unroll
        for (int gi = 0; gi < kGroups; ++gi) {
            const int t = t0 + gi * kFinishCols + col;
#pragma unroll
            for (int u = 0; u < kRows; ++u) {
                const int b = b0 + slice + u * kFinishSlices;
                v[gi][u] = (t < width && b < nblocks) ? scratch[(size_t)b * width + t] : 0.0;
            }
        }
#pragma unroll
        for (int gi = 0; gi < kGroups; ++gi) {
            const int t = t0 + gi * kFinishCols + col;
            double acc = 0.0;
#pragma unroll
            for (int u = 0; u < kRows; ++u) acc += v[gi][u];
#pragma unroll
            for (int u = 0; u < kRows; ++u) {
                const int b = b0 + slice + u * kFinishSlices;
                if (t < width && b < nblocks) scratch[(size_t)b * width + t] = 0.0;
            }
            __syncthreads();
            part[slice][col] = acc;
            __syncthreads();
            if (slice == 0 && t < width) {
                double sum = 0.0;
#pragma unroll
                for (int k = 0; k < kFinishSlices; ++k) sum += part[k][col];
                dst[t] = sum;
            }
        }
    }
}

static int tune_grid(int64_t tiles, int dp, int64_t scratch_bytes, bool* two_level) {
    const int64_t width = 2 * dp + kStatTail;
    *two_level = tiles > kTuneGrid && scratch_bytes >= (int64_t)kMaxGrid * width * (int64_t)sizeof(double) && !getenv("NFMC_TUNE_ONE_LEVEL");
    const int cap = *two_level ? kMaxGrid - kTuneFoldWgs : kTuneGrid;
    return (int)(tiles < cap ? tiles : cap);
}

static void tune_update(const NfmcStats& stats, const NfmcTune& tune, int grid, bool two_level, int dp, int d, unsigned long long attempted,
                        hipStream_t st) {
    const int width = 2 * dp + kStatTail;
    if (two_level) {
        double* partial = stats.scratch + (size_t)(kMaxGrid - kTuneFoldWgs) * width;
        const int wgs = (grid + kTuneFoldSlabs - 1) / kTuneFoldSlabs;
        hipLaunchKernelGGL(tune_fold_kernel, dim3(wgs), dim3(kFinishBlock), 0, st, stats.scratch, grid, width, partial);
        hipLaunchKernelGGL(tune_finish_kernel<1>, dim3(1), dim3(kFinishBlock), 0, st, partial, wgs, dp, d, stats, tune, attempted);
    } else {
        hipLaunchKernelGGL(tune_finish_kernel<1>, dim3(1), dim3(kFinishBlock), 0, st, stats.scratch, grid, dp, d, stats, tune, attempted);
    }
}

template <class Args>
static int check_tune(const Args& a, int dp) {
    if (!a.tune.state) return NFMC_OK;
    if (!a.stats.sum_x || a.stats.defer || a.jump) return NFMC_EINVAL;
    if (a.tune.tune_inv_mass_diag && (!a.tune.inv_mass_diag || a.tune.inv_mass_diag != a.inv_mass_diag)) return NFMC_EINVAL;
    if (dp != padded_d(a.d)) return NFMC_EINVAL;
    return NFMC_OK;
}

#define NFMC_KIND_CASE(KIND, POT) \
    case KIND: return launch_mala_kind<POT>(a, jd, c, jhp, tiles, grid, sqrt2h, st);
static int launch_mala(const NfmcMalaArgs& a, const JumpDev& jd, Cfg c, int jhp, bool fast, int64_t tiles, int grid,
                       float sqrt2h, hipStream_t st) {
    switch (a.pot.kind) { NFMC_FOR_OWN_UNIT_POT(NFMC_KIND_CASE) }
    return jhp == 0 ? launch_mala_j0(a, jd, c, fast, tiles, grid, sqrt2h, st)
                    : (jhp == 4 ? launch_mala_j4(a, jd, c, fast, tiles, grid, sqrt2h, st)
                                : launch_mala_j8(a, jd, c, fast, tiles, grid, sqrt2h, st));
}
#undef NFMC_KIND_CASE
#define NFMC_KIND_CASE(KIND, POT) \
    case KIND: return launch_hmc_kind<POT>(a, jd, c, jhp, tiles, grid, st);
static int launch_hmc(const NfmcHmcArgs& a, const JumpDev& jd, Cfg c, int jhp, bool fast, int64_t tiles, int grid,
                      hipStream_t st) {
    switch (a.pot.kind) { NFMC_FOR_OWN_UNIT_POT(NFMC_KIND_CASE) }
    return jhp == 0 ? launch_hmc_j0(a, jd, c, fast, tiles, grid, st)
                    : (jhp == 4 ? launch_hmc_j4(a, jd, c, fast, tiles, grid, st) : launch_hmc_j8(a, jd, c, fast, tiles, grid, st));
}
#undef NFMC_KIND_CASE

static JumpDev jump_dev(const NfmcJumpTail* j) {
    JumpDev jd = {};
    if (j) {
        jd.flow = j->flow;
        jd.adjusted = j->adjusted;
        jd.replay_latent = j->replay_latent;
        jd.replay_uniform = j->replay_uniform;
        jd.mask_out = j->mask_out;
        jd.log_ratio_out = j->log_ratio_out;
    }
    return jd;
}

}

using namespace nfmc;

extern "C" int64_t nfmc_stats_scratch_bytes(int32_t d) {
    if (d <= 0 || d > 1024) return 0;
    return stats_scratch_doubles(padded_d(d)) * (int64_t)sizeof(double);
}

extern "C" int64_t nfmc_tune_state_doubles(int32_t d) {
    if (d <= 0 || d > 1024) return 0;
    return NFMC_TUNE_WORDS + 3 * padded_d(d) + kStatTail;
}

extern "C" int nfmc_sampler_layout(int32_t d, int32_t pot_kind_id, int32_t* cpl, int32_t* lpc) {
    if (!cpl || !lpc || d <= 0) return NFMC_EINVAL;
    if (d > 1024) return NFMC_ESHAPE;
    const PotKind* pk = pot_kind(pot_kind_id);
    if (!pk) return NFMC_EUNSUPPORTED;
    const Cfg c = choose_cfg(d, false, pk->default_cfg_only);
    if (!c.cpl) return NFMC_ESHAPE;
    *cpl = c.cpl;
    *lpc = c.lpc;
    return NFMC_OK;
}

template <class Args, class Launch>
static int sampler_steps(const Args* args, hipStream_t st, Launch launch, const LaunchPart* part = nullptr) {
    Args a = *args;
    const int jhp = a.jump ? (a.jump->flow.n_hidden <= 4 ? 4 : 8) : 0;
    const Cfg c = choose_cfg(a.d, jhp > 0, pot_kind(a.pot.kind)->default_cfg_only);
    if (!c.cpl) return NFMC_ESHAPE;
    const bool fast = fast_path(&a, c) && !a.tune.state;
    const int dp = c.cpl * c.lpc;
    const int cpw = kWave / c.lpc;
    const int64_t tiles = (a.n + (int64_t)kWavesPerBlock * cpw - 1) / ((int64_t)kWavesPerBlock * cpw);
    bool two_level = false;
    const int gcap = part ? part->grid_cap : kMaxGrid;
    const int grid = a.tune.state ? tune_grid(tiles, dp, a.stats.scratch_bytes, &two_level) : (int)(tiles < gcap ? tiles : gcap);
    if (a.stats.sum_x && a.stats.scratch_bytes < (int64_t)grid * (2 * dp + kStatTail) * (int64_t)sizeof(double))
        return NFMC_ESCRATCH;
    if (check_defer(a.stats, dp, a.d)) return NFMC_EINVAL;
    if (int rc = check_tune(a, dp)) return rc;
    if (part && a.stats.sum_x) a.stats.scratch += (size_t)part->slab0 * (2 * dp + kStatTail);
    const JumpDev jd = jump_dev(a.jump);
    unsigned long long* jc = a.jump ? a.jump->counters : nullptr;
    a.jump = nullptr;
    if (a.tune.state) {
        const int every = (a.tune.every > 0 && a.tune.every < a.n_steps) ? a.tune.every : a.n_steps;
        const int total = a.n_steps;
        for (int s0 = 0; s0 < total; s0 += every) {
            const int k = total - s0 < every ? total - s0 : every;
            Args b = a;
            b.n_steps = k;
            b.rng.step0 = a.rng.step0 + (uint32_t)s0;
            if (a.rng.replay_normals) b.rng.replay_normals = a.rng.replay_normals + (int64_t)s0 * a.n * a.d;
            if (a.rng.replay_uniforms) b.rng.replay_uniforms = a.rng.replay_uniforms + (int64_t)s0 * a.n;
            if (a.masks_out) b.masks_out = a.masks_out + (int64_t)s0 * a.n;
            if (a.log_ratio_out) b.log_ratio_out = a.log_ratio_out + (int64_t)s0 * a.n;
            if (int rc = launch(b, jd, c, 0, fast, tiles, grid)) return rc;
            tune_update(a.stats, a.tune, grid, two_level, dp, a.d, (unsigned long long)a.n * (unsigned long long)k, st);
            NFMC_HIP_CHECK_LAUNCH();
            store_advance(a.samples, k);
        }
        return NFMC_OK;
    }
    if (int rc = launch(a, jd, c, jhp, fast, tiles, grid)) return rc;
    NFMC_HIP_CHECK_LAUNCH();
    if (a.stats.sum_x && !a.stats.defer) {
        hipLaunchKernelGGL(stats_finish_kernel<true>, dim3(stats_finish_grid(dp)), dim3(kFinishBlock), 0, st, a.stats.scratch,
                           grid, dp, a.d, a.stats, (unsigned long long)a.n * (unsigned long long)a.n_steps, jc,
                           (unsigned long long)a.n);
        NFMC_HIP_CHECK_LAUNCH();
    }
    return NFMC_OK;
}

static int mala_steps(const NfmcMalaArgs* args, hipStream_t st, const LaunchPart* part) {
    if (int rc = check_common(args)) return rc;
    const float sqrt2h = (float)sqrt(2.0 * (double)args->step_size);
    return sampler_steps(args, st, [=](const NfmcMalaArgs& a, const JumpDev& jd, Cfg c, int jhp, bool fast, int64_t tiles, int grid) {
        return launch_mala(a, jd, c, jhp, fast, tiles, grid, sqrt2h, st);
    }, part);
}

static int hmc_steps(const NfmcHmcArgs* args, hipStream_t st, const LaunchPart* part) {
    if (int rc = check_common(args)) return rc;
    if (args->n_leapfrog <= 0) return NFMC_EINVAL;
    return sampler_steps(args, st, [=](const NfmcHmcArgs& a, const JumpDev& jd, Cfg c, int jhp, bool fast, int64_t tiles, int grid) {
        return launch_hmc(a, jd, c, jhp, fast, tiles, grid, st);
    }, part);
}

extern "C" int nfmc_mala_steps_f32(const NfmcMalaArgs* args, nfmc_stream_t stream) {
    return mala_steps(args, (hipStream_t)stream, nullptr);
}

extern "C" int nfmc_hmc_steps_f32(const NfmcHmcArgs* args, nfmc_stream_t stream) {
    return hmc_steps(args, (hipStream_t)stream, nullptr);
}


static int side_streams(int count, hipStream_t* out) {
    constexpr int kMaxDevices = 64;
    static std::mutex mu;
    static hipStream_t streams[kMaxDevices][NFMC_JUMP_RUN_MAX_PARTS - 1] = {};
    int dev = 0;
    if (hipError_t e = hipGetDevice(&dev)) return (int)e;
    if (dev < 0 || dev >= kMaxDevices) return NFMC_EUNSUPPORTED;
    std::lock_guard<std::mutex> lock(mu);
    for (int i = 0; i < count; ++i) {
        if (!streams[dev][i])
            if (hipError_t e = hipStreamCreateWithFlags(&streams[dev][i], hipStreamNonBlocking)) return (int)e;
        out[i] = streams[dev][i];
    }
    return NFMC_OK;
}

static int64_t sampler_tile_chains(int d, int pot_kind_id) {
    const PotKind* pk = pot_kind(pot_kind_id);
    const Cfg c = choose_cfg(d, false, pk && pk->default_cfg_only);
    return c.cpl ? (int64_t)kWavesPerBlock * (kWave / c.lpc) : 0;
}

template <class Args, class Steps>
static int jump_run(const NfmcJumpRun& r, const Args& inner, hipStream_t st, Steps steps) {
    const NfmcFlowMhArgs& jump = *r.jump;
    const int64_t n = inner.n;
    const int d = inner.d, K = r.n_inner, T = r.n_outer;
    if (T <= 0 || K <= 0 || r.n_parts < 1 || r.n_parts > NFMC_JUMP_RUN_MAX_PARTS) return NFMC_EINVAL;
    if (!inner.x || n <= 0 || d <= 0 || jump.x != inner.x || jump.n != n || jump.flow.d != d || !jump.logq) return NFMC_EINVAL;
    if (jump.rng.seed != inner.rng.seed || jump.rng.chain_offset != inner.rng.chain_offset || jump.rng.rounds != inner.rng.rounds)
        return NFMC_EINVAL;
    if (inner.jump || inner.tune.state || inner.samples.base || jump.samples.base || inner.masks_out || jump.masks_out ||
        inner.log_ratio_out || jump.log_ratio_out || inner.rng.replay_normals || inner.rng.replay_uniforms ||
        jump.rng.replay_normals || jump.rng.replay_uniforms)
        return NFMC_EINVAL;
    if ((inner.stats.sum_x != nullptr) != (jump.stats.sum_x != nullptr)) return NFMC_EINVAL;
    if (inner.stats.sum_x && (!inner.stats.defer || !jump.stats.defer || inner.stats.scratch != jump.stats.scratch)) return NFMC_EINVAL;

    int parts = r.n_parts;
    int64_t m = n;
    if (parts > 1) {
        const int64_t ti = sampler_tile_chains(d, inner.pot.kind), tj = flow_mh_tile_chains(jump);
        if (ti <= 0 || tj <= 0) {
            parts = 1;
        } else {
            const int64_t tile = ti > tj ? ti : tj, per = (n + parts - 1) / parts;
            m = (per + tile - 1) / tile * tile;
        }
    }
    const int share = (kMaxGrid + parts - 1) / parts;
    int used = 0;
    while (used < parts && (int64_t)used * m < n) ++used;

    hipStream_t streams[NFMC_JUMP_RUN_MAX_PARTS] = {st};
    hipEvent_t events[2 * NFMC_JUMP_RUN_MAX_PARTS] = {};
    const int n_events = used > 1 ? 2 * (used - 1) : 0;
    if (used > 1) {
        if (int rc = side_streams(used - 1, streams + 1)) return rc;
        for (int p = 0; p < n_events; ++p)
            if (hipError_t e = hipEventCreateWithFlags(&events[p], hipEventDisableTiming)) {
                for (int q = 0; q < p; ++q) (void)hipEventDestroy(events[q]);
                return (int)e;
            }
    }
    const char* stagger_env = getenv("NFMC_JUMP_STAGGER");
    const bool stagger = !(stagger_env && atoi(stagger_env) == 0);

    int rc = NFMC_OK;
    for (int i = 0; i < T && !rc; ++i) {
        const uint32_t base = inner.rng.step0 + (uint32_t)i * (uint32_t)(K + 1);
        for (int p = 0; p < used && !rc; ++p) {
            const int64_t lo = (int64_t)p * m, np = (n - lo < m ? n - lo : m);
            const LaunchPart lp = {p * share, share < kMaxGrid - p * share ? share : kMaxGrid - p * share, n};
            const LaunchPart* part = parts > 1 ? &lp : nullptr;
            if (i == 0 && p > 0) {
                if (hipError_t e = hipStreamWaitEvent(streams[p], events[p - 1], 0)) rc = (int)e;
            }
            if (i == 0 && p + 1 < used && !stagger && !rc)
                if (hipError_t e = hipEventRecord(events[p], streams[p])) rc = (int)e;
            for (int off = 0; off < K && !rc; off += NFMC_MAX_STEPS_PER_CALL) {
                Args b = inner;
                b.x = inner.x + lo * d;
                b.n = np;
                b.n_steps = K - off < NFMC_MAX_STEPS_PER_CALL ? K - off : NFMC_MAX_STEPS_PER_CALL;
                b.rng.chain_offset = inner.rng.chain_offset + (uint64_t)lo;
                b.rng.step0 = base + (uint32_t)off;
                rc = steps(&b, streams[p], part);
            }
            if (i == 0 && p + 1 < used && (stagger || rc)) {
                hipError_t e = hipEventRecord(events[p], streams[p]);
                if (e != hipSuccess && !rc) rc = (int)e;
            }
            if (rc) break;
            NfmcFlowMhArgs j = jump;
            j.x = jump.x + lo * d;
            j.logq = jump.logq + lo;
            j.n = np;
            j.n_steps = 1;
            j.logq_cached = 0;
            j.rng.chain_offset = jump.rng.chain_offset + (uint64_t)lo;
            j.rng.step0 = base + (uint32_t)K;
            rc = flow_mh_steps(j, streams[p], part);
        }
    }

    for (int p = 1; p < used; ++p) {
        hipError_t e = hipEventRecord(events[used - 1 + p - 1], streams[p]);
        if (e == hipSuccess) e = hipStreamWaitEvent(st, events[used - 1 + p - 1], 0);
        if (e != hipSuccess && !rc) rc = (int)e;
    }
    for (int p = 0; p < n_events; ++p) (void)hipEventDestroy(events[p]);
    return rc;
}

extern "C" int nfmc_jump_run_f32(const NfmcJumpRun* run, nfmc_stream_t stream) {
    if (!run || !run->inner || !run->jump) return NFMC_EINVAL;
    hipStream_t st = (hipStream_t)stream;
    if (run->inner_kind == NFMC_INNER_MALA) return jump_run(*run, *(const NfmcMalaArgs*)run->inner, st, mala_steps);
    if (run->inner_kind == NFMC_INNER_HMC) return jump_run(*run, *(const NfmcHmcArgs*)run->inner, st, hmc_steps);
    return NFMC_EINVAL;
}
```

### nfmc_amd/flows.py

```python
import ctypes as C
import math
import os
from typing import Optional, Tuple

import numpy as np
import torch
import torch.nn as nn

from . import hip

MIN_SCALE = 1e-3


def default_hidden(d_a: int) -> int:
    return max(4, int(3 * math.log10(max(d_a, 1))))


class ElementwiseAffine(nn.Module):

    def __init__(self, d):
        super().__init__()
        self.log_scale = nn.Parameter(torch.zeros(d))
        self.shift = nn.Parameter(torch.zeros(d))


class ReversePermutation(nn.Module):
    """z[j] = x[d-1-j]; folded into the kernels' index arithmetic, never materialised."""


class AffineCoupling(nn.Module):

    def __init__(self, d, n_hidden=None, n_layers=2):
        super().__init__()
        self.d_a = d // 2
        self.d_b = d - self.d_a
        self.n_hidden = default_hidden(self.d_a) if n_hidden is None else int(n_hidden)
        self.n_layers = int(n_layers)
        if self.n_layers < 1:
            raise ValueError('conditioner needs at least one hidden layer')
        dims = [self.d_a] + [self.n_hidden] * self.n_layers + [2 * self.d_b]
        self.conditioner = nn.ModuleList([nn.Linear(dims[i], dims[i + 1]) for i in range(len(dims) - 1)])


RQS_BINS, RQS_BOUND = 8, 5.0


class RQSCoupling(AffineCoupling):

    def __init__(self, d, n_hidden=None, n_layers=2, n_bins=RQS_BINS):
        super().__init__(d, n_hidden, n_layers)
        self.n_bins = int(n_bins)
        dims = [self.d_a] + [self.n_hidden] * self.n_layers + [(3 * self.n_bins - 1) * self.d_b]
        self.conditioner = nn.ModuleList([nn.Linear(dims[i], dims[i + 1]) for i in range(len(dims) - 1)])


class RealNVP(nn.Module):

    min_scale = MIN_SCALE
    n_bins = 0
    spline_bound = RQS_BOUND
    coupling_class = AffineCoupling

    def __init__(self, event_shape, n_layers: int = 2, conditioner_kwargs: Optional[dict] = None, **kwargs):
        super().__init__()
        if isinstance(event_shape, int):
            event_shape = (event_shape,)
        self.event_shape = tuple(int(s) for s in event_shape)
        self.d = int(math.prod(self.event_shape))
        ck = dict(conditioner_kwargs or {})
        if 'n_hidden' in kwargs:
            ck.setdefault('n_hidden', kwargs['n_hidden'])
        self.n_coupling = int(n_layers)
        layers = [ElementwiseAffine(self.d)]
        for _ in range(self.n_coupling):
            layers += [ReversePermutation(), self._make_coupling(ck)]
        layers.append(ElementwiseAffine(self.d))
        self.layers = nn.ModuleList(layers)
        self._pack_cache = None

    def _make_coupling(self, ck):
        return AffineCoupling(self.d, ck.get('n_hidden'), ck.get('n_layers', 2))

    def __getstate__(self):
        state = self.__dict__.copy()
        state['_pack_cache'] = None
        state.pop('_mods_cache', None)
        state.pop('_device_fit', None)
        state.pop('_wide_scratch', None)
        return state

    @property
    def couplings(self):
        return [m for m in self.layers if isinstance(m, AffineCoupling)]

    @property
    def n_hidden(self):
        c = self.couplings
        return c[0].n_hidden if c else 4

    @property
    def n_hidden_layers(self):
        c = self.couplings
        return c[0].n_layers if c else 1

    def _version_key(self, device):
        mods = self.__dict__.get('_mods_cache')
        if mods is None:
            mods = self.__dict__['_mods_cache'] = [m for m in self.modules() if m._parameters]
        return (str(device),) + tuple((p.data_ptr(), p._version) for m in mods for p in m._parameters.values()
                                      if p is not None)

    def default_min_hidden(self) -> int:
        ok = (self.d in (64, 128) and 8 < self.n_hidden <= 32 and self.n_hidden_layers in (1, 2) and self.n_bins == 0
              and os.environ.get('NFMC_FLOW_NO_MFMA') is None)
        return 64 if ok else 0

    def packed(self, device, min_hidden: int = None):
        if min_hidden is None:
            min_hidden = self.default_min_hidden()
        key = self._version_key(device) + (int(min_hidden),)
        cache = self._pack_cache if isinstance(self._pack_cache, dict) else {}
        hit = cache.get(int(min_hidden))
        if hit is not None and hit[0] == key:
            return hit[1]
        lib = hip.lib()
        d, H, nhl = self.d, max(self.n_hidden, int(min_hidden)), self.n_hidden_layers
        hp = int(lib.nfmc_realnvp_padded_hidden(H))
        stride = int(lib.nfmc_coupling_layer_floats(d, H, nhl, self.n_bins))
        out_rows = (3 * self.n_bins - 1) * (d - d // 2) if self.n_bins else 2 * (d - d // 2)
        d_a, d_b = d // 2, d - d // 2
        if hp == 0:
            raise ValueError('RealNVP conditioner width %d is beyond the kernels (max 128)' % H)
        if stride == 0:
            raise ValueError('spline couplings run with conditioners of width <= 32 and %d bins' % RQS_BINS)
        with torch.no_grad():
            n_w = max(1, self.n_coupling * stride)
            ea_off = (n_w + 3) // 4 * 4
            d4 = (d + 3) // 4 * 4
            flat = np.zeros(ea_off + 4 * d4, dtype=np.float32)
            for li, cpl in enumerate(self.couplings):
                lin = list(cpl.conditioner)
                cur = [li * stride]

                def put(t, rows=None, cols=None, transpose=False):
                    t = t.detach().float().cpu().numpy()
                    if t.ndim == 1:
                        n_out = rows if rows is not None else t.shape[0]
                        flat[cur[0]:cur[0] + t.shape[0]] = t
                        cur[0] += n_out
                        return
                    if transpose:
                        view = flat[cur[0]:cur[0] + rows * cols].reshape(cols, rows)
                        view[:t.shape[1], :t.shape[0]] = t.T
                    else:
                        view = flat[cur[0]:cur[0] + rows * cols].reshape(rows, cols)
                        view[:t.shape[0], :t.shape[1]] = t
                    cur[0] += rows * cols

                if hp > 32:
                    put(lin[0].weight, hp, d_a)
                    put(lin[0].weight, hp, d_a, transpose=True)
                    put(lin[0].bias, hp)
                    for l in lin[1:-1]:
                        put(l.weight, hp, hp)
                        put(l.weight, hp, hp, transpose=True)
                        put(l.bias, hp)
                    put(lin[-1].weight, 2 * d_b, hp)
                    put(lin[-1].weight, 2 * d_b, hp, transpose=True)
                    put(lin[-1].bias)
                else:
                    put(lin[0].weight, hp, d_a, transpose=True)
                    put(lin[0].bias, hp)
                    for l in lin[1:-1]:
                        put(l.weight, hp, hp, transpose=True)
                        put(l.bias, hp)
                    put(lin[-1].weight, out_rows, hp)
                    put(lin[-1].bias)
                assert cur[0] == (li + 1) * stride, (cur[0], li, stride)
            ea0, ea1 = self.layers[0], self.layers[-1]
            for k, t in enumerate((ea0.log_scale, ea0.shift, ea1.log_scale, ea1.shift)):
                flat[ea_off + k * d4:ea_off + k * d4 + d] = t.detach().float().cpu().numpy()
            blob = torch.from_numpy(flat).to(device)
            keep = [blob] + [blob[ea_off + k * d4:ea_off + k * d4 + d] for k in range(4)]
        st = hip.NfmcRealNVP(d, self.n_coupling, H, nhl, float(self.min_scale), int(self.n_bins), hip.ptr(keep[1]),
                             hip.ptr(keep[2]), hip.ptr(keep[3]), hip.ptr(keep[4]), hip.ptr(keep[0]), stride,
                             float(self.spline_bound), 0)
        need = int(lib.nfmc_flow_scratch_bytes(C.byref(st), 1 << 40, 1))
        if need:
            ws = self.__dict__.get('_wide_scratch')
            if ws is None or ws.device != torch.device(device) or ws.numel() * 4 < need:
                ws = self.__dict__['_wide_scratch'] = torch.empty(need // 4, dtype=torch.float32, device=device)
            st.scratch, st.scratch_bytes = hip.ptr(ws), need
            keep.append(ws)
        cache[int(min_hidden)] = (key, (st, keep))
        self._pack_cache = cache
        return st, keep

    def _prep(self, v):
        dev = hip.require_gpu()
        n = v.shape[0]
        return dev, n, v.detach().to(dev, torch.float32).reshape(n, self.d).contiguous()

    def beyond_kernels(self) -> bool:
        lim = hip.limits()
        if self.d < 2 and self.n_coupling > 0:
            return True
        return self.d > lim.max_d_flow or self.n_hidden > (32 if self.n_bins else lim.max_hidden)

    def _composed(self, v, inverse: bool):
        from .flow_training import forward_torch, inverse_torch
        dev, n, vf = self._prep(v)
        if next(self.parameters()).device != dev:
            self.to(dev)
        with torch.no_grad():
            out, ld = (inverse_torch if inverse else forward_torch)(self, vf)
        return out.reshape(n, *self.event_shape), ld

    def forward(self, x):
        if self.beyond_kernels():
            return self._composed(x, False)
        dev, n, xf = self._prep(x)
        st, _keep = self.packed(dev)
        z = torch.empty_like(xf)
        ld = torch.empty(n, dtype=torch.float32, device=dev)
        hip.check(hip.lib().nfmc_realnvp_forward_f32(C.byref(st), hip.ptr(xf), n, hip.ptr(z), hip.ptr(ld), None,
                                                     hip.stream()), 'nfmc_realnvp_forward_f32')
        return z.reshape(n, *self.event_shape), ld

    def inverse(self, z):
        if self.beyond_kernels():
            return self._composed(z, True)
        dev, n, zf = self._prep(z)
        st, _keep = self.packed(dev)
        x = torch.empty_like(zf)
        ld = torch.empty(n, dtype=torch.float32, device=dev)
        hip.check(hip.lib().nfmc_realnvp_inverse_f32(C.byref(st), hip.ptr(zf), n, hip.ptr(x), hip.ptr(ld), None, None,
                                                     hip.stream()), 'nfmc_realnvp_inverse_f32')
        return x.reshape(n, *self.event_shape), ld


class NICE(RealNVP):

    min_scale = 1.0


class CRQNSF(RealNVP):

    n_bins = RQS_BINS

    def _make_coupling(self, ck):
        return RQSCoupling(self.d, ck.get('n_hidden'), ck.get('n_layers', 2), self.n_bins)


class Flow(nn.Module):

    def __init__(self, bijection: RealNVP):
        super().__init__()
        self.bijection = bijection
        self._sample_calls = 0
        self.seed = None

    @property
    def event_shape(self):
        return self.bijection.event_shape

    def get_device(self):
        return next(self.parameters()).device

    @staticmethod
    def _base_log_prob(z):
        zf = z.flatten(1)
        return -0.5 * (zf * zf).sum(-1) - 0.5 * zf.shape[1] * math.log(2.0 * math.pi)

    def log_prob(self, x):
        if self.bijection.beyond_kernels():
            z, ld = self.bijection.forward(x)
            return self._base_log_prob(z) + ld
        dev, n, xf = self.bijection._prep(x)
        st, _keep = self.bijection.packed(dev)
        lp = torch.empty(n, dtype=torch.float32, device=dev)
        hip.check(hip.lib().nfmc_realnvp_forward_f32(C.byref(st), hip.ptr(xf), n, None, None, hip.ptr(lp),
                                                     hip.stream()), 'nfmc_realnvp_forward_f32')
        return lp

    def sample(self, n, return_log_prob=False, no_grad=False, rng=None):
        dev = hip.require_gpu()
        if rng is None:
            if self.seed is None:
                self.seed = int(torch.randint(0, 2 ** 62, ()).item())
            rng = hip.make_rng(self.seed, 0, self._sample_calls)
            self._sample_calls += 1
        if self.bijection.beyond_kernels():
            z = torch.empty(n, self.bijection.d, dtype=torch.float32, device=dev)
            hip.check(hip.lib().nfmc_philox_normals_f32(C.byref(rng), hip.TAG_LATENT, n, self.bijection.d, hip.ptr(z),
                                                        hip.stream()), 'nfmc_philox_normals_f32')
            x, ld = self.bijection.inverse(z)
            return (x, self._base_log_prob(z) - ld) if return_log_prob else x
        st, _keep = self.bijection.packed(dev)
        x = torch.empty(n, self.bijection.d, dtype=torch.float32, device=dev)
        lq = torch.empty(n, dtype=torch.float32, device=dev) if return_log_prob else None
        hip.check(hip.lib().nfmc_realnvp_inverse_f32(C.byref(st), None, n, hip.ptr(x), None, hip.ptr(lq),
                                                     C.byref(rng), hip.stream()), 'nfmc_realnvp_inverse_f32')
        x = x.reshape(n, *self.event_shape)
        return (x, lq) if return_log_prob else x

    def fit(self, x_train, x_val=None, **kwargs):
        from .flow_training import fit as _fit
        return _fit(self, x_train, x_val, **kwargs)

    def variational_fit(self, log_prob_fn, **kwargs):
        from .flow_training import variational_fit as _vfit
        return _vfit(self, log_prob_fn, **kwargs)
```

### nfmc_amd/hip.py

```python
import ctypes as C
import os

import torch

HERE = os.path.dirname(os.path.abspath(__file__))
LIB_PATH = os.environ.get('NFMC_LIB', os.path.join(HERE, 'libnfmc_hip.so'))

OK, EINVAL, ESHAPE, EALIGN, EUNSUPPORTED, ESCRATCH = 0, -1, -2, -3, -4, -5
POT_QUADRATIC, POT_FUNNEL, POT_GAUSSIAN_MIXTURE, POT_LOGISTIC_REGRESSION, POT_GAUSSIAN_FULL, POT_ROSENBROCK = 0, 1, 2, 3, 4, 5
POT_STOCHASTIC_VOLATILITY = 6
POT_SPARSE_LOGISTIC_REGRESSION = 7
POT_LATTICE_PHI4 = 8
POT_ITEM_RESPONSE = 9
POT_VARYING_EFFECTS = 10
POT_PARTICLES = 11
POT_LATENT_GAUSSIAN = 12
MIXTURE_MAX_COMPONENTS = 8
TAG_NOISE, TAG_ACCEPT, TAG_LATENT, TAG_JUMP = 0, 1, 2, 3
CNT_ACCEPTED, CNT_ATTEMPTED, CNT_NONFINITE, CNT_WORDS = 0, 1, 2, 4
MAX_STEPS_PER_CALL = 512
IMH_PARALLEL_MAX_STEPS = 65536

c_fp = C.c_void_p
NFMC_ABI_VERSION = 4


class NfmcPotential(C.Structure):
    _fields_ = [('kind', C.c_int32), ('reserved', C.c_int32), ('a', c_fp), ('b', c_fp),
                ('a_scalar', C.c_float), ('b_scalar', C.c_float)]


class NfmcRng(C.Structure):
    _fields_ = [('seed', C.c_uint64), ('chain_offset', C.c_uint64), ('step0', C.c_uint32), ('rounds', C.c_uint32),
                ('replay_normals', c_fp), ('replay_uniforms', c_fp)]


class NfmcStats(C.Structure):
    _fields_ = [('sum_x', c_fp), ('sum_x2', c_fp), ('counters', c_fp), ('scratch', c_fp),
                ('scratch_bytes', C.c_int64), ('defer', C.c_int32), ('tail_slot', C.c_int32)]


class NfmcRealNVP(C.Structure):
    _fields_ = [('d', C.c_int32), ('n_coupling', C.c_int32), ('n_hidden', C.c_int32), ('n_hidden_layers', C.c_int32),
                ('min_scale', C.c_float), ('n_bins', C.c_int32),
                ('ea0_log_scale', c_fp), ('ea0_shift', c_fp), ('ea1_log_scale', c_fp), ('ea1_shift', c_fp),
                ('weights', c_fp), ('layer_stride', C.c_int64), ('spline_bound', C.c_float), ('reserved', C.c_int32),
                ('scratch', c_fp), ('scratch_bytes', C.c_int64)]


class NfmcSampleStore(C.Structure):
    _fields_ = [('base', c_fp), ('stride', C.c_int32), ('countdown', C.c_int32), ('ring_rows', C.c_int32), ('row', C.c_int32)]


class NfmcJumpTail(C.Structure):
    _fields_ = [('flow', NfmcRealNVP), ('adjusted', C.c_int32), ('reserved', C.c_int32), ('counters', c_fp),
                ('replay_latent', c_fp), ('replay_uniform', c_fp), ('mask_out', c_fp), ('log_ratio_out', c_fp)]


class NfmcTune(C.Structure):
    _fields_ = [('state', c_fp), ('inv_mass_diag', c_fp), ('tune_step_size', C.c_int32), ('tune_inv_mass_diag', C.c_int32),
                ('every', C.c_int32), ('reserved', C.c_int32)]


TUNE_STEP_SIZE, TUNE_LOG_SMOOTH, TUNE_ERROR_SUM, TUNE_ITERATION, TUNE_ANCHOR, TUNE_LOG_RAW = 0, 1, 2, 3, 4, 5
TUNE_TARGET, TUNE_KAPPA, TUNE_GAMMA, TUNE_IMD_ADJUSTMENT, TUNE_TICKET, TUNE_WORDS = 6, 7, 8, 9, 10, 12
STAT_TAIL = 4


def padded_d(d):
    p = 4
    while p < d:
        p <<= 1
    return p


def tune_shift_offset(d):
    return TUNE_WORDS + 2 * padded_d(d) + STAT_TAIL


WARMUP_STEP0 = 1 << 31


class NfmcMalaArgs(C.Structure):
    _fields_ = [('x', c_fp), ('n', C.c_int64), ('d', C.c_int32), ('n_steps', C.c_int32),
                ('step_size', C.c_float), ('adjust', C.c_int32), ('inv_mass_diag', c_fp),
                ('pot', NfmcPotential), ('rng', NfmcRng), ('stats', NfmcStats),
                ('samples', NfmcSampleStore), ('masks_out', c_fp), ('log_ratio_out', c_fp), ('jump', C.POINTER(NfmcJumpTail)),
                ('tune', NfmcTune)]


class NfmcHmcArgs(C.Structure):
    _fields_ = [('x', c_fp), ('n', C.c_int64), ('d', C.c_int32), ('n_steps', C.c_int32),
                ('step_size', C.c_float), ('n_leapfrog', C.c_int32), ('adjust', C.c_int32), ('reserved', C.c_int32),
                ('inv_mass_diag', c_fp), ('pot', NfmcPotential), ('rng', NfmcRng), ('stats', NfmcStats),
                ('samples', NfmcSampleStore), ('masks_out', c_fp), ('log_ratio_out', c_fp), ('jump', C.POINTER(NfmcJumpTail)),
                ('tune', NfmcTune)]


class NfmcFlowMhArgs(C.Structure):
    _fields_ = [('x', c_fp), ('logq', c_fp), ('n', C.c_int64), ('n_steps', C.c_int32), ('logq_cached', C.c_int32),
                ('adjusted', C.c_int32), ('reserved', C.c_int32), ('flow', NfmcRealNVP), ('pot', NfmcPotential),
                ('rng', NfmcRng), ('stats', NfmcStats), ('samples', NfmcSampleStore), ('masks_out', c_fp),
                ('log_ratio_out', c_fp)]


INNER_MALA, INNER_HMC = 0, 1
JUMP_RUN_MAX_PARTS = 4


class NfmcJumpRun(C.Structure):
    _fields_ = [('inner_kind', C.c_int32), ('n_parts', C.c_int32), ('inner', c_fp), ('jump', C.POINTER(NfmcFlowMhArgs)),
                ('n_outer', C.c_int32), ('n_inner', C.c_int32)]


class NfmcNeutraHmcArgs(C.Structure):
    _fields_ = [('z', c_fp), ('n', C.c_int64), ('n_steps', C.c_int32), ('n_leapfrog', C.c_int32),
                ('step_size', C.c_float), ('adjust', C.c_int32), ('inv_mass_diag', c_fp),
                ('flow', NfmcRealNVP), ('pot', NfmcPotential), ('rng', NfmcRng), ('stats', NfmcStats),
                ('samples', NfmcSampleStore), ('masks_out', c_fp), ('log_ratio_out', c_fp), ('scratch', c_fp),
                ('scratch_bytes', C.c_int64)]


class NfmcFlowLogqGradArgs(C.Structure):
    _fields_ = [('flow', NfmcRealNVP), ('x', c_fp), ('n', C.c_int64), ('grad_out', c_fp), ('logq_out', c_fp)]


class NfmcDlmcStepArgs(C.Structure):
    _fields_ = [('flow', NfmcRealNVP), ('pot', NfmcPotential), ('x', c_fp), ('grad_u', c_fp), ('logq_out', c_fp),
                ('n', C.c_int64), ('step_size', C.c_float), ('reserved', C.c_int32)]


class NfmcSelectArgs(C.Structure):
    _fields_ = [('x', c_fp), ('x_prime', c_fp), ('n', C.c_int64), ('d', C.c_int32), ('n_carry', C.c_int32),
                ('log_ratio', c_fp), ('uniforms', c_fp), ('carry', c_fp * 2), ('carry_prime', c_fp * 2),
                ('rng', NfmcRng), ('rng_tag', C.c_int32), ('reserved', C.c_int32), ('stats', NfmcStats),
                ('mask_out', c_fp)]


class NfmcAdamW(C.Structure):
    _fields_ = [('lr', C.c_float), ('beta1', C.c_float), ('beta2', C.c_float), ('eps', C.c_float),
                ('weight_decay', C.c_float), ('step', C.c_int32)]


class NfmcFlowFit(C.Structure):
    _fields_ = [('flow', NfmcRealNVP), ('params', c_fp), ('adam_m', c_fp), ('adam_v', c_fp), ('n_params', C.c_int64),
                ('ea_off', C.c_int64), ('partial', c_fp), ('partial_floats', C.c_int64), ('status', c_fp),
                ('x_val', c_fp), ('n_val', C.c_int64), ('params_prev', c_fp), ('best', c_fp), ('run_state', c_fp),
                ('scratch', c_fp), ('scratch_bytes', C.c_int64)]


class NfmcBlobPiece(C.Structure):
    _fields_ = [('param', c_fp), ('vec_off', C.c_int64), ('rows', C.c_int32), ('cols', C.c_int32),
                ('vec_row_stride', C.c_int32), ('vec_col_stride', C.c_int32)]


class NfmcFitControl(C.Structure):
    _fields_ = [('n_epochs', C.c_int32), ('early_stopping', C.c_int32), ('early_stopping_threshold', C.c_int32),
                ('keep_best_weights', C.c_int32), ('skip_nonfinite', C.c_int32), ('reserved', C.c_int32)]


FIT_BEST_LOSS, FIT_SINCE_BEST, FIT_APPLIED, FIT_STOPPED, FIT_DIVERGED, FIT_LAST_LOSS, FIT_LAST_VAL, FIT_BOOKED = range(8)
FIT_STATE_FLOATS = 8


class NfmcLimits(C.Structure):
    _fields_ = [('abi_version', C.c_int32), ('max_d_sampler', C.c_int32), ('max_d_flow', C.c_int32),
                ('max_hidden_valu', C.c_int32), ('max_hidden', C.c_int32), ('max_steps_per_call', C.c_int32)]


SYMBOLS = [
    ('nfmc_stats_scratch_bytes', C.c_int64, [C.c_int32]),
    ('nfmc_tune_state_doubles', C.c_int64, [C.c_int32]),
    ('nfmc_sampler_layout', C.c_int, [C.c_int32, C.c_int32, C.POINTER(C.c_int32), C.POINTER(C.c_int32)]),
    ('nfmc_mala_steps_f32', C.c_int, [C.POINTER(NfmcMalaArgs), c_fp]),
    ('nfmc_hmc_steps_f32', C.c_int, [C.POINTER(NfmcHmcArgs), c_fp]),
    ('nfmc_realnvp_padded_hidden', C.c_int32, [C.c_int32]),
    ('nfmc_realnvp_layer_floats', C.c_int64, [C.c_int32, C.c_int32, C.c_int32]),
    ('nfmc_coupling_layer_floats', C.c_int64, [C.c_int32, C.c_int32, C.c_int32, C.c_int32]),
    ('nfmc_flow_scratch_bytes', C.c_int64, [C.POINTER(NfmcRealNVP), C.c_int64, C.c_int32]),
    ('nfmc_realnvp_forward_f32', C.c_int, [C.POINTER(NfmcRealNVP), c_fp, C.c_int64, c_fp, c_fp, c_fp, c_fp]),
    ('nfmc_realnvp_inverse_f32', C.c_int, [C.POINTER(NfmcRealNVP), c_fp, C.c_int64, c_fp, c_fp, c_fp,
                                           C.POINTER(NfmcRng), c_fp]),
    ('nfmc_flow_mh_steps_f32', C.c_int, [C.POINTER(NfmcFlowMhArgs), c_fp]),
    ('nfmc_flow_mh_supported_f32', C.c_int, [C.POINTER(NfmcFlowMhArgs)]),
    ('nfmc_jump_run_f32', C.c_int, [C.POINTER(NfmcJumpRun), c_fp]),
    ('nfmc_imh_parallel_supported_f32', C.c_int, [C.POINTER(NfmcFlowMhArgs)]),
    ('nfmc_imh_parallel_work_bytes', C.c_int64, [C.c_int64, C.c_int32, C.c_int32]),
    ('nfmc_imh_parallel_f32', C.c_int, [C.POINTER(NfmcFlowMhArgs), c_fp, C.c_int64, c_fp]),
    ('nfmc_neutra_scratch_bytes', C.c_int64, [C.c_int64, C.c_int32, C.c_int32, C.c_int32, C.c_int32]),
    ('nfmc_neutra_hmc_steps_f32', C.c_int, [C.POINTER(NfmcNeutraHmcArgs), c_fp]),
    ('nfmc_neutra_potential_grad_f32', C.c_int, [C.POINTER(NfmcRealNVP), C.POINTER(NfmcPotential), c_fp, C.c_int64,
                                                 c_fp, c_fp, c_fp]),
    ('nfmc_flow_logq_grad_f32', C.c_int, [C.POINTER(NfmcFlowLogqGradArgs), c_fp]),
    ('nfmc_flow_logq_grad_supported_f32', C.c_int, [C.POINTER(NfmcFlowLogqGradArgs)]),
    ('nfmc_dlmc_step_f32', C.c_int, [C.POINTER(NfmcDlmcStepArgs), c_fp]),
    ('nfmc_dlmc_step_supported_f32', C.c_int, [C.POINTER(NfmcDlmcStepArgs)]),
    ('nfmc_mh_accept_select_f32', C.c_int, [C.POINTER(NfmcSelectArgs), c_fp]),
    ('nfmc_langevin_propose_f32', C.c_int, [c_fp, c_fp, c_fp, C.c_float, C.c_int64, C.c_int32, C.POINTER(NfmcRng),
                                            c_fp, c_fp]),
    ('nfmc_langevin_log_ratio_f32', C.c_int, [c_fp, c_fp, c_fp, c_fp, c_fp, c_fp, c_fp, C.c_float, C.c_int64,
                                              C.c_int32, c_fp, c_fp]),
    ('nfmc_moments_update_f32', C.c_int, [c_fp, C.c_int64, C.c_int32, C.POINTER(NfmcStats), c_fp]),
    ('nfmc_stats_fold_f32', C.c_int, [C.POINTER(NfmcStats), C.c_int32, C.c_uint64, c_fp, C.c_uint64, c_fp]),
    ('nfmc_philox_normals_f32', C.c_int, [C.POINTER(NfmcRng), C.c_int32, C.c_int64, C.c_int32, c_fp, c_fp]),
    ('nfmc_philox_uniforms_f32', C.c_int, [C.POINTER(NfmcRng), C.c_int32, C.c_int64, c_fp, c_fp]),
    ('nfmc_flow_fit_supported_f32', C.c_int, [C.POINTER(NfmcRealNVP)]),
    ('nfmc_flow_fit_partial_floats', C.c_int64, [C.c_int64, C.c_int64]),
    ('nfmc_flow_fit_workspace', C.c_int64, [C.POINTER(NfmcRealNVP), C.c_int64, C.c_int64, C.c_int64, C.POINTER(C.c_int64)]),
    ('nfmc_flow_fit_step_f32', C.c_int, [C.POINTER(NfmcFlowFit), c_fp, C.c_int64, C.POINTER(NfmcAdamW), c_fp]),
    ('nfmc_flow_variational_fit_step_f32', C.c_int, [C.POINTER(NfmcFlowFit), C.POINTER(NfmcPotential), c_fp, C.c_int64,
                                                    C.POINTER(NfmcAdamW), c_fp]),
    ('nfmc_flow_fit_epochs_f32', C.c_int, [C.POINTER(NfmcFlowFit), C.POINTER(NfmcPotential), c_fp, C.c_int64, C.c_int64,
                                          C.POINTER(NfmcAdamW), C.POINTER(NfmcFitControl), C.c_int32, C.c_int32, c_fp]),
    ('nfmc_flow_blob_copy_f32', C.c_int, [c_fp, C.POINTER(NfmcBlobPiece), C.c_int32, C.c_int32, c_fp]),
    ('nfmc_rows_sample_f32', C.c_int, [c_fp, C.c_int64, C.c_int32, C.c_uint64, C.c_int64, c_fp, C.c_int64, c_fp, c_fp]),
    ('nfmc_rows_sample_index', C.c_int64, [C.c_int64, C.c_uint64, C.c_int64]),
    ('nfmc_limits', C.c_int, [C.POINTER(NfmcLimits)]),
    ('nfmc_error_string', C.c_char_p, [C.c_int]),
    ('nfmc_build_digest', C.c_char_p, []),
]

_lib = None


def lib():
    global _lib
    if _lib is None:
        if not os.path.exists(LIB_PATH):
            raise RuntimeError(
                'nfmc_amd: %s is missing. Build it with `python -m nfmc_amd.build` (needs hipcc); the MI355X '
                'path has no CPU/eager fallback.' % LIB_PATH)
        handle = C.CDLL(LIB_PATH)
        probe = getattr(handle, 'nfmc_limits', None)
        if probe is None:
            raise RuntimeError('nfmc_amd: %s does not export nfmc_limits (not an nfmc_hip library?)' % LIB_PATH)
        probe.restype, probe.argtypes = C.c_int, [C.POINTER(NfmcLimits)]
        lim = NfmcLimits()
        rc = probe(C.byref(lim))
        if rc != 0 or lim.abi_version != NFMC_ABI_VERSION:
            raise RuntimeError('nfmc_amd: %s has ABI version %d (status %d); this package binds version %d. Rebuild it '
                               'with `python -m nfmc_amd.build --force`.' % (LIB_PATH, lim.abi_version, rc, NFMC_ABI_VERSION))
        for name, restype, argtypes in SYMBOLS:
            fn = getattr(handle, name)
            fn.restype = restype
            fn.argtypes = argtypes
        _lib = handle
    return _lib


class NfmcArgumentError(ValueError):

    def __init__(self, message, code):
        super().__init__(message)
        self.code = code

    @property
    def no_kernel(self):
        return self.code in (EUNSUPPORTED, ESHAPE)


def check(rc, what):
    if rc == 0:
        return
    msg = lib().nfmc_error_string(rc).decode()
    if rc < 0:
        raise NfmcArgumentError('%s: %s (code %d)' % (what, msg, rc), rc)
    raise RuntimeError('%s: HIP error %d: %s' % (what, rc, msg))


def supported(rc, what) -> bool:
    if rc in (EUNSUPPORTED, ESHAPE):
        return False
    check(rc, what)
    return True


def require_gpu():
    if not torch.cuda.is_available():
        raise RuntimeError('nfmc_amd needs a ROCm GPU (MI355X / gfx950); torch.cuda.is_available() is False. '
                           'There is no CPU fallback for the hot path.')
    return torch.device('cuda', torch.cuda.current_device())


def ptr(t, dtype=torch.float32):
    if t is None:
        return None
    if not t.is_cuda:
        raise ValueError('expected a GPU tensor')
    if t.dtype != dtype:
        raise ValueError('expected dtype %s, got %s' % (dtype, t.dtype))
    if not t.is_contiguous():
        raise ValueError('expected a contiguous tensor')
    return C.c_void_p(t.data_ptr())


_raw_stream = getattr(torch._C, '_cuda_getCurrentRawStream', None)


def stream():
    if _raw_stream is not None:
        return C.c_void_p(_raw_stream(torch.cuda.current_device()))
    return C.c_void_p(torch.cuda.current_stream().cuda_stream)


def build_digest():
    return lib().nfmc_build_digest().decode()


def limits():
    out = NfmcLimits()
    check(lib().nfmc_limits(C.byref(out)), 'nfmc_limits')
    return out


class DeviceStats:

    def __init__(self, d, device):
        self.d = d
        self.device = device
        self._buf = torch.zeros(2 * d + 2 * CNT_WORDS, dtype=torch.float64, device=device)
        self._sum_x = self._buf[:d]
        self._sum_x2 = self._buf[d:2 * d]
        self._counters = self._buf[2 * d:2 * d + CNT_WORDS].view(torch.int64)
        self._jump_counters = self._buf[2 * d + CNT_WORDS:].view(torch.int64)
        nbytes = int(lib().nfmc_stats_scratch_bytes(d))
        self.scratch = torch.zeros(nbytes // 8, dtype=torch.float64, device=device)
        self._pending = False
        self._attempted = 0
        self._jump_attempted = 0

    def _raw(self, defer=0, tail_slot=0, counters=None):
        return NfmcStats(ptr(self._sum_x, torch.float64), ptr(self._sum_x2, torch.float64),
                         ptr(self._counters if counters is None else counters, torch.int64),
                         ptr(self.scratch, torch.float64), self.scratch.numel() * 8, defer, tail_slot)

    def struct(self, defer=False, attempted=0, jump=False, jump_attempted=0):
        if not defer or os.environ.get('NFMC_STATS_DEFER', '1') == '0':
            self.fold()
            return self._raw(counters=self._jump_counters if jump else None)
        self._pending = True
        if jump:
            self._jump_attempted += int(attempted)
        else:
            self._attempted += int(attempted)
            self._jump_attempted += int(jump_attempted)
        return self._raw(1, 2 if jump else 0)

    def fold(self):
        if not self._pending:
            return
        st = self._raw()
        check(lib().nfmc_stats_fold_f32(C.byref(st), self.d, self._attempted, ptr(self._jump_counters, torch.int64),
                                        self._jump_attempted, stream()), 'nfmc_stats_fold_f32')
        self._pending = False
        self._attempted = 0
        self._jump_attempted = 0

    @property
    def sum_x(self):
        self.fold()
        return self._sum_x

    @property
    def sum_x2(self):
        self.fold()
        return self._sum_x2

    @property
    def counters(self):
        self.fold()
        return self._counters

    @property
    def jump_counters(self):
        self.fold()
        return self._jump_counters

    def host_totals(self):
        self.fold()
        h = self._buf.cpu()
        d = self.d
        return (h[:d], h[d:2 * d], h[2 * d:2 * d + CNT_WORDS].view(torch.int64),
                h[2 * d + CNT_WORDS:].view(torch.int64))

    def zero_(self):
        self.fold()
        self._buf.zero_()


def dense_store(t):
    if t is None:
        return NfmcSampleStore(None, 1, 0, 1, 0)
    return NfmcSampleStore(ptr(t), 1, 0, int(t.shape[0]), 0)


def store_struct(samples, k):
    if samples is None:
        return dense_store(None)
    if hasattr(samples, 'struct'):
        return samples.struct(k)
    if int(samples.shape[0]) != int(k):
        raise ValueError('dense sample view has %d rows for %d transitions' % (samples.shape[0], k))
    return dense_store(samples)


def null_stats():
    return NfmcStats(None, None, None, None, 0, 0, 0)


def make_rng(seed, chain_offset, step0, replay_normals=None, replay_uniforms=None, rounds=0):
    return NfmcRng(int(seed) & 0xFFFFFFFFFFFFFFFF, int(chain_offset), int(step0) & 0xFFFFFFFF, int(rounds),
                   ptr(replay_normals), ptr(replay_uniforms))
```

### nfmc_amd/samplers/common.py

```python
import ctypes as C
import math
import time
from typing import Optional

import torch

from .. import hip
from ..containers import DeviceSampleStore
from ..potentials import Potential, recognize


def resolve_target(target, event_shape, fuse='auto', x0=None, family=None) -> Optional[Potential]:
    if isinstance(target, Potential):
        return target if family is None or target.fused_in(family) else None
    if fuse in (False, 'never'):
        return None
    x_scale = None
    if x0 is not None and x0.numel() > 0:
        x_scale = float(x0.detach().abs().max())
    return recognize(target, event_shape, x_scale=x_scale)


class Replay:

    def __init__(self, normals, uniforms, device):
        self.normals = torch.as_tensor(normals, dtype=torch.float32).to(device).contiguous()
        self.normals = self.normals.reshape(self.normals.shape[0], self.normals.shape[1], -1)
        self.uniforms = None
        if uniforms is not None and torch.as_tensor(uniforms).numel() > 0:
            self.uniforms = torch.as_tensor(uniforms, dtype=torch.float32).to(device).contiguous()
        self.i_n = 0
        self.i_u = 0

    def take_uniforms(self, k=1):
        un = self.uniforms[self.i_u:self.i_u + k]
        assert un.shape[0] == k, 'replay uniforms exhausted'
        self.i_u += k
        return un

    def take(self, k, with_uniforms=True):
        nz = self.normals[self.i_n:self.i_n + k]
        assert nz.shape[0] == k, 'replay noise exhausted'
        self.i_n += k
        un = None
        if with_uniforms:
            un = self.uniforms[self.i_u:self.i_u + k]
            assert un.shape[0] == k, 'replay uniforms exhausted'
            self.i_u += k
        return nz, un


class Run:

    def __init__(self, sampler, x0):
        self.dev = hip.require_gpu()
        hip.lib()
        self.n = int(x0.shape[0])
        self.event_shape = tuple(x0.shape[1:])
        self.d = int(math.prod(self.event_shape)) if self.event_shape else 1
        self.sampler = sampler
        shard = sampler.shard
        self.shard = shard
        if shard is not None:
            lo, hi = shard.bounds(self.n)
            x0 = x0[lo:hi]
            self.chain_offset = lo
            self.n_global = self.n
            self.n = hi - lo
        else:
            self.chain_offset = 0
            self.n_global = self.n
        self.x = x0.detach().to(self.dev, torch.float32).reshape(self.n, self.d).contiguous().clone()
        self.stats = hip.DeviceStats(self.d, self.dev)
        if sampler.seed is None:
            seed = int(torch.randint(0, 2 ** 62, ()).item())
            if shard is not None:
                seed = shard.broadcast_int(seed)
        else:
            seed = int(sampler.seed)
        self.seed = seed
        self.rounds = int(getattr(sampler, 'rng_rounds', 10) or 10)
        if self.rounds not in (7, 10):
            raise ValueError('rng_rounds must be 10 (Philox4x32-10) or 7 (Philox4x32-7)')
        self.replay = None
        if sampler.replay is not None:
            normals, uniforms = sampler.replay
            self.replay = Replay(normals, uniforms, self.dev)
        self.t0 = time.time()
        self.kernel_events = None
        tk = getattr(sampler, 'time_kernels', False)
        self.kernel_event_filter = tk if isinstance(tk, str) else None
        if tk:
            self.kernel_events = []

    def timed(self, label):
        return _Timed(self, label)

    def rng(self, step0, k=0, adjusted=True):
        if self.replay is not None:
            nz, un = self.replay.take(k, with_uniforms=adjusted)
            self._keep = (nz, un)
            return hip.make_rng(self.seed, self.chain_offset, step0, nz, un, rounds=self.rounds)
        return hip.make_rng(self.seed, self.chain_offset, step0, rounds=self.rounds)

    def sync(self):
        torch.cuda.synchronize(self.dev)

    def time_is_up(self, t0, limit_seconds) -> bool:
        if limit_seconds is None:
            return False
        self.sync()
        up = time.time() - t0 >= limit_seconds
        if self.shard is not None and self.shard.world > 1:
            up = bool(self.shard.broadcast_int(1 if up else 0))
        return up

    def elapsed(self):
        self.sync()
        return time.time() - self.t0

    def sample_store(self, offered):
        p = self.sampler.params
        if not (p.store_samples and offered > 0):
            return None
        return DeviceSampleStore(self.n, self.d, self.dev, offered, getattr(p, 'thinning', 1),
                                 getattr(p, 'max_samples', None))

    def finish(self, out, t0, n_moments, store=None, **counters):
        last_sample = self.x.reshape(self.n, *self.event_shape).clone()
        sum_x, sum_x2, cnt, jc = self.stats.host_totals()
        st = out.statistics
        device = {'n_accepted_trajectories': int(cnt[hip.CNT_ACCEPTED]),
                  'n_attempted_trajectories': int(cnt[hip.CNT_ATTEMPTED])}
        if 'n_accepted_jumps' in st.COUNTERS:
            device.update(n_accepted_jumps=int(jc[hip.CNT_ACCEPTED]), n_attempted_jumps=int(jc[hip.CNT_ATTEMPTED]))
        st.update_counters(**{**device, **counters})
        st.n_nonfinite_log_ratios = int(cnt[hip.CNT_NONFINITE]) + int(jc[hip.CNT_NONFINITE])
        st.absorb_device_sums(sum_x.reshape(self.event_shape), sum_x2.reshape(self.event_shape), n_moments)
        if store is not None:
            out.running_samples.adopt_store(store, getattr(self.sampler.params, 'spill_to_host', False))
        out.running_samples.last_sample = last_sample
        st.update_elapsed_time(time.time() - t0)
        out.kernel_events = self.kernel_events
        if self.shard is not None:
            self.shard.merge_statistics(st)
        return out


class _Timed:
    def __init__(self, run, label):
        self.run, self.label = run, label

    def _on(self):
        sel = getattr(self.run, 'kernel_event_filter', None)
        return self.run.kernel_events is not None and (sel is None or sel == self.label)

    def __enter__(self):
        if self._on():
            self.e0 = torch.cuda.Event(enable_timing=True)
            self.e1 = torch.cuda.Event(enable_timing=True)
            self.e0.record(torch.cuda.current_stream())
        return self

    def __exit__(self, *exc):
        if self._on():
            self.e1.record(torch.cuda.current_stream())
            self.run.kernel_events.append((self.label, self.e0, self.e1))


def chunks(total, limit=hip.MAX_STEPS_PER_CALL):
    done = 0
    while done < total:
        k = min(limit, total - done)
        yield done, k
        done += k


def imd_tensor(kernel, dev):
    imd = kernel.inv_mass_diag
    if imd is None or bool((imd == 1).all()):
        return None
    return imd.detach().to(dev, torch.float32).contiguous()


class _NoBar:

    def __init__(self, iterable=None):
        self._it = iterable

    def __iter__(self):
        return iter(self._it)

    def update(self, n=1):
        pass

    def close(self):
        pass

    def set_postfix_str(self, s):
        pass


def progress(show, iterable=None, **kw):
    if not show:
        return _NoBar(iterable)
    from tqdm import tqdm
    return tqdm(iterable, **kw) if iterable is not None else tqdm(**kw)
```

### nfmc_amd/samplers/jump.py

```python
import ctypes as C
import math
import os
import time
from copy import deepcopy
from dataclasses import dataclass
from typing import Optional

import torch
from tqdm import tqdm

from .. import hip
from ..containers import (MCMCKernel, MCMCOutput, MCMCParameters, MCMCStatistics, NFMCKernel, NFMCParameters,
                          Sampler)
from ..flows import Flow, RealNVP
from ..tuning import train_val_split
from ..util import metropolis_acceptance_log_ratio
from .common import Run, chunks, progress, resolve_target
from .mcmc import HMC, MALA, MH, UHMC, ULA, Langevin, TargetFailure, _guarded


@dataclass
class JumpNFMCParameters(NFMCParameters):
    adjusted_jumps: bool = True
    fit_nf: bool = False
    warmup_fit_kwargs: dict = None
    n_jumps_before_training: int = 10

    def __post_init__(self):
        super().__post_init__()
        if self.warmup_fit_kwargs is None:
            self.warmup_fit_kwargs = {
                'early_stopping': True,
                'early_stopping_threshold': 50,
                'keep_best_weights': True,
                'n_samples': 1,
                'n_epochs': 500,
                'lr': 0.05
            }


@dataclass
class JumpNFMCStatistics(MCMCStatistics):
    n_accepted_jumps: int = 0
    n_attempted_jumps: int = 0

    COUNTERS = MCMCStatistics.COUNTERS + ('n_accepted_jumps', 'n_attempted_jumps')
    RATES = MCMCStatistics.RATES + ('jump_acceptance_rate',)

    @property
    def jump_acceptance_rate(self):
        return self.n_accepted_jumps / self.n_attempted_jumps if self.n_attempted_jumps else math.nan

    def _summary(self):
        rows = super()._summary()
        return [('MCMC acc-rate', rows[0][1]), ('Jump acc-rate', '%.2f' % self.jump_acceptance_rate)] + rows[1:]


class JumpNFMCOutput(MCMCOutput):
    def __init__(self, event_shape, *args, **kwargs):
        kwargs['statistics'] = JumpNFMCStatistics(event_shape)
        super().__init__(event_shape, *args, **kwargs)


def flow_is_native(flow) -> bool:
    bij = getattr(flow, 'bijection', None)
    if not isinstance(bij, RealNVP):
        return False
    return not bij.beyond_kernels()


def flow_fits_jump_tail(flow) -> bool:
    bij = getattr(flow, 'bijection', None)
    return (isinstance(bij, RealNVP) and bij.n_hidden <= 8 and bij.d <= 512 and bij.n_hidden_layers <= 4
            and bij.n_bins == 0)


def make_jump_tail(run: Run, flow, adjusted):
    st, keep = flow.bijection.packed(run.dev)
    t = hip.NfmcJumpTail()
    t.flow = st
    t.adjusted = 1 if adjusted else 0
    t.counters = hip.ptr(run.stats._jump_counters, torch.int64)
    t._keep = [keep]
    return t


def flow_mh_supported(run: Run, flow, pot, logq, adjusted=True) -> bool:
    a, _keep = _flow_mh_probe_args(run, flow, pot, logq, adjusted)
    return hip.supported(int(hip.lib().nfmc_flow_mh_supported_f32(C.byref(a))), 'nfmc_flow_mh_supported_f32')


def flow_mh_args(run: Run, flow, pot, logq, k, step0, cached, adjusted, stats_struct, samples=None, masks_out=None,
                 log_ratio_out=None):
    a = hip.NfmcFlowMhArgs()
    st, _keep = flow.bijection.packed(run.dev)
    a.x, a.logq, a.n, a.n_steps = hip.ptr(run.x), hip.ptr(logq), run.n, k
    a.logq_cached = 1 if cached else 0
    a.adjusted = 1 if adjusted else 0
    a.flow = st
    a.pot = pot.descriptor(run.dev)
    a.rng = run.rng(step0, k, adjusted=adjusted)
    a.stats = stats_struct
    a.samples = hip.store_struct(samples, k)
    a.masks_out = hip.ptr(masks_out, torch.uint8) if masks_out is not None else None
    a.log_ratio_out = hip.ptr(log_ratio_out) if log_ratio_out is not None else None
    a._keep = _keep
    return a


def launch_flow_mh(run: Run, flow, pot, logq, k, step0, cached, adjusted, stats_struct, samples=None,
                   masks_out=None, log_ratio_out=None):
    a = flow_mh_args(run, flow, pot, logq, k, step0, cached, adjusted, stats_struct, samples, masks_out, log_ratio_out)
    with run.timed('flow_mh_steps'):
        hip.check(hip.lib().nfmc_flow_mh_steps_f32(C.byref(a), hip.stream()), 'nfmc_flow_mh_steps_f32')


JUMP_PARTS = {hip.INNER_MALA: (2, 16384), hip.INNER_HMC: (2, 16384)}
JUMP_RUN_SLICE = 16


def launch_jump_run(run: Run, inner, flow, pot, logq, step0, n_outer, n_inner, n_parts, adjusted):
    n = run.n
    k = min(n_inner, hip.MAX_STEPS_PER_CALL)
    ia = inner._args(run, pot, k, step0, None, attempted=n * n_inner * n_outer)
    ja = flow_mh_args(run, flow, pot, logq, 1, step0 + n_inner, False, adjusted,
                      run.stats.struct(defer=True, attempted=n * n_outer, jump=True))
    r = hip.NfmcJumpRun()
    r.inner_kind = hip.INNER_HMC if isinstance(ia, hip.NfmcHmcArgs) else hip.INNER_MALA
    r.inner = C.cast(C.pointer(ia), C.c_void_p)
    r.jump = C.pointer(ja)
    r.n_outer, r.n_inner, r.n_parts = n_outer, n_inner, n_parts
    hip.check(hip.lib().nfmc_jump_run_f32(C.byref(r), hip.stream()), 'nfmc_jump_run_f32')


def _flow_mh_probe_args(run: Run, flow, pot, logq, adjusted):
    a = hip.NfmcFlowMhArgs()
    st, _keep = flow.bijection.packed(run.dev)
    a.x, a.logq, a.n, a.n_steps = hip.ptr(run.x), hip.ptr(logq), run.n, 1
    a.adjusted = 1 if adjusted else 0
    a.flow = st
    a.pot = pot.descriptor(run.dev)
    a.rng = hip.make_rng(run.seed, run.chain_offset, 0, rounds=run.rounds)
    a.stats = hip.null_stats()
    return a, _keep


def imh_parallel_ok(run: Run, flow, pot, logq) -> bool:
    bij = getattr(flow, 'bijection', None)
    if not flow_is_native(flow) or bij.n_hidden > 8 or bij.d > 512:
        return False
    if os.environ.get('NFMC_IMH_PARALLEL') == '0' or not pot.fused_in('imh_parallel'):
        return False
    a, _keep = _flow_mh_probe_args(run, flow, pot, logq, True)
    return hip.supported(int(hip.lib().nfmc_imh_parallel_supported_f32(C.byref(a))), 'nfmc_imh_parallel_supported_f32')


def launch_imh_parallel(run: Run, flow, pot, logq, k, step0, cached, stats_struct, samples=None, masks_out=None,
                        log_ratio_out=None):
    a = hip.NfmcFlowMhArgs()
    st, _keep = flow.bijection.packed(run.dev)
    a.x, a.logq, a.n, a.n_steps = hip.ptr(run.x), hip.ptr(logq), run.n, k
    a.logq_cached = 1 if cached else 0
    a.adjusted = 1
    a.flow = st
    a.pot = pot.descriptor(run.dev)
    a.rng = run.rng(step0, k, adjusted=True)
    a.stats = stats_struct
    a.samples = hip.store_struct(samples, k)
    a.masks_out = hip.ptr(masks_out, torch.uint8) if masks_out is not None else None
    a.log_ratio_out = hip.ptr(log_ratio_out) if log_ratio_out is not None else None
    nbytes = int(hip.lib().nfmc_imh_parallel_work_bytes(run.n, run.d, k))
    work = torch.empty(nbytes, dtype=torch.uint8, device=run.dev)
    with run.timed('imh_parallel'):
        hip.check(hip.lib().nfmc_imh_parallel_f32(C.byref(a), hip.ptr(work, torch.uint8), nbytes, hip.stream()),
                  'nfmc_imh_parallel_f32')
    return work


def split_flow_mh(run: Run, flow, target, event_shape, step, adjusted, stats_struct, logq=None):
    n, d = run.n, run.d
    with torch.no_grad():
        if flow_is_native(flow) or isinstance(flow, Flow):
            rng = hip.make_rng(run.seed, run.chain_offset, step, rounds=run.rounds)
            if run.replay is not None:
                nz, _ = run.replay.take(1, with_uniforms=False)
                x_prime, ld = flow.bijection.inverse(nz[0].reshape(n, *event_shape))
                zz = nz[0]
                f_xp = (-0.5 * (zz * zz).sum(-1) - 0.5 * d * 1.8378770664093453) - ld
                unif = None
            else:
                x_prime, f_xp = flow.sample(n, return_log_prob=True, rng=rng)
                unif = None
        else:
            x_prime, f_xp = flow.sample(n, return_log_prob=True)
            unif = None
        x_prime = x_prime.detach().to(run.dev, torch.float32).reshape(n, d).contiguous()
        f_xp = f_xp.detach().to(run.dev, torch.float32).contiguous()
        lr = None
        f_x = None
        target_calls = 0
        if adjusted:
            try:
                u_x = _guarded(target, run.x.reshape(n, *event_shape)).reshape(-1)
                u_xp = _guarded(target, x_prime.reshape(n, *event_shape)).reshape(-1)
                target_calls = 2 * n
                f_x = logq if logq is not None else _guarded(flow.log_prob, run.x.reshape(n, *event_shape))
                f_x = f_x.detach().to(run.dev, torch.float32).contiguous()
                lr = metropolis_acceptance_log_ratio(-u_x, -u_xp, f_x, f_xp).float().contiguous()
                if run.replay is not None and (flow_is_native(flow) or isinstance(flow, Flow)):
                    unif = run.replay.take_uniforms(1)[0].contiguous()
            except TargetFailure:
                lr = torch.full((n,), -math.inf, dtype=torch.float32, device=run.dev)
    st = hip.NfmcSelectArgs()
    st.x, st.x_prime, st.n, st.d = hip.ptr(run.x), hip.ptr(x_prime), n, d
    st.log_ratio = hip.ptr(lr) if lr is not None else None
    st.uniforms = hip.ptr(unif) if unif is not None else None
    st.n_carry = 0
    if logq is not None and adjusted:
        st.n_carry = 1
        st.carry[0] = hip.ptr(logq)
        st.carry_prime[0] = hip.ptr(f_xp)
    st.rng = hip.make_rng(run.seed, run.chain_offset, step, rounds=run.rounds)
    st.rng_tag = hip.TAG_JUMP
    st.stats = stats_struct
    st.mask_out = None
    hip.check(hip.lib().nfmc_mh_accept_select_f32(C.byref(st), hip.stream()), 'nfmc_mh_accept_select_f32')
    return target_calls


class JumpNFMC(Sampler):

    fuse_jump_tail = False

    jump_parts = None

    def __init__(self, event_shape, target, inner_sampler: Sampler, kernel: NFMCKernel = None,
                 params: JumpNFMCParameters = None):
        if kernel is None:
            kernel = NFMCKernel(event_shape)
        if params is None:
            params = JumpNFMCParameters()
        super().__init__(event_shape, target, kernel, params)
        self.inner_sampler = inner_sampler

    @property
    def name(self):
        return 'Jump MCMC'

    def _refit(self, flow, x_train, x_val):
        from ..flows import Flow
        if isinstance(flow, Flow):
            return flow.fit(x_train=x_train, x_val=x_val, **{'defer_check': True, **self.params.flow_fit_kwargs})
        flow.fit(x_train=x_train, x_val=x_val, **self.params.flow_fit_kwargs)
        return None

    def _jump_parts(self, inner, n):
        parts = self.jump_parts
        if parts is None and os.environ.get('NFMC_JUMP_PARTS'):
            parts = os.environ['NFMC_JUMP_PARTS']
        if parts is None:
            parts, n_min = JUMP_PARTS[hip.INNER_HMC if isinstance(inner, HMC) else hip.INNER_MALA]
            return parts if n >= n_min else 1
        parts = int(parts)
        if not 1 <= parts <= hip.JUMP_RUN_MAX_PARTS:
            raise ValueError('jump_parts must be 1 .. %d' % hip.JUMP_RUN_MAX_PARTS)
        return parts

    def warmup(self, x0, show_progress: bool = True, time_limit_seconds=None) -> MCMCOutput:
        inner_limit = 0.7 * time_limit_seconds if time_limit_seconds is not None else None
        t0 = time.time()
        self.inner_sampler.params.store_samples = True
        self.inner_sampler.shard = self.shard
        warmup_output = self.inner_sampler.warmup(x0, show_progress=show_progress, time_limit_seconds=inner_limit)
        x_train, x_val = train_val_split(warmup_output.samples_device, train_pct=self.params.train_pct,
                                         max_train_size=self.params.max_train_size,
                                         max_val_size=self.params.max_val_size, shard=self.shard)
        flow_params = deepcopy(self.kernel.flow.state_dict())
        fit_limit = time_limit_seconds - (time.time() - t0) if time_limit_seconds is not None else None
        try:
            self.kernel.flow.fit(x_train=x_train, x_val=x_val,
                                 **{**self.params.flow_fit_kwargs,
                                    **dict(show_progress=show_progress, time_limit_seconds=fit_limit)})
        except ValueError:
            self.kernel.flow.load_state_dict(flow_params)
        return warmup_output

    def sample(self, x0, show_progress: bool = True, time_limit_seconds=None) -> MCMCOutput:
        inner = self.inner_sampler
        if not inner.params.store_samples:
            raise ValueError("Inner sampler in jump HMC must store samples")
        run = Run(self, x0)
        n, d, event_shape = run.n, run.d, run.event_shape
        flow = self.kernel.flow
        T, K = int(self.params.n_iterations), int(inner.params.n_iterations)
        off = (False, 'never')
        pot = resolve_target(self.target, event_shape,
                             'never' if (self.fuse in off or getattr(inner, 'fuse', 'auto') in off) else 'auto', run.x,
                             family='mcmc')
        fused = pot is not None and flow_is_native(flow) and pot.fused_in('flow_mh')
        tail_ok = (self.fuse_jump_tail and fused and pot.jump_tail_ok() and flow_fits_jump_tail(flow) and not self.params.fit_nf
                   and isinstance(inner, (MALA, ULA, HMC, UHMC)))
        inner._cur_run = run
        inner._n_divergences = 0
        jump_target_calls = 0

        store = run.sample_store(T * (K + 1))
        fit_buf = torch.empty(K, n, d, dtype=torch.float32, device=run.dev) if self.params.fit_nf else None
        pending_fit = None
        logq = torch.empty(n, dtype=torch.float32, device=run.dev)
        probed = not fused

        def probe():
            nonlocal fused, tail_ok, probed
            if not probed and not flow_mh_supported(run, flow, pot, logq, self.params.adjusted_jumps):
                fused = tail_ok = False
            probed = True

        if tail_ok:
            probe()
        whole_run = (pot is not None and not tail_ok and not self.params.fit_nf and store is None and run.replay is None
                     and run.kernel_events is None and not show_progress and isinstance(inner, (Langevin, HMC))
                     and os.environ.get('NFMC_STATS_DEFER', '1') != '0')

        t0 = time.time()
        done = 0
        bar = progress(show_progress, range(T), desc='Jump MCMC')
        for i in bar:
            if i < done:
                continue
            if run.time_is_up(t0, time_limit_seconds):
                break
            if i > 0 and whole_run and fused:
                ts = T - i if time_limit_seconds is None else min(JUMP_RUN_SLICE, T - i)
                launch_jump_run(run, inner, flow, pot, logq, i * (K + 1), ts, K, self._jump_parts(inner, n),
                                self.params.adjusted_jumps)
                jump_target_calls += 2 * n * ts if self.params.adjusted_jumps else 0
                done = i + ts
                continue
            base = i * (K + 1)
            dense = fit_buf is not None
            tail_done = False
            if pot is not None:
                for off, k in chunks(K):
                    last = off + k == K
                    tail = None
                    if last and tail_ok:
                        tail = make_jump_tail(run, flow, self.params.adjusted_jumps)
                    view = fit_buf[off:off + k] if dense else store
                    if tail is not None and run.replay is not None:
                        rng_inner = run.rng(base + off, k, adjusted=inner.params.adjustment)
                        lat, un = run.replay.take(1, with_uniforms=self.params.adjusted_jumps)
                        tail.replay_latent = hip.ptr(lat[0].contiguous())
                        tail.replay_uniform = hip.ptr(un[0].contiguous()) if un is not None else None
                        tail._keep += [lat, un]
                        inner._launch(run, pot, k, base + off, view, jump=tail, rng=rng_inner)
                    else:
                        inner._launch(run, pot, k, base + off, view, jump=tail)
                    tail_done = tail is not None
            else:
                for off in range(K):
                    inner._split_step(run, base + off, fit_buf[off:off + 1] if dense else store)
            probe()
            if dense and store is not None:
                store.add_dense(fit_buf)
            if self.params.fit_nf and i >= self.params.n_jumps_before_training:
                x_train, x_val = train_val_split(fit_buf.reshape(K, n, *event_shape),
                                                 train_pct=self.params.train_pct,
                                                 max_train_size=self.params.max_train_size,
                                                 max_val_size=self.params.max_val_size, shard=self.shard)
                if pending_fit is not None:
                    pending_fit.result()
                pending_fit = self._refit(flow, x_train, x_val)
            if tail_done:
                jump_target_calls += 2 * n if self.params.adjusted_jumps else 0
            elif fused:
                launch_flow_mh(run, flow, pot, logq, 1, base + K, False, self.params.adjusted_jumps,
                               run.stats.struct(defer=True, attempted=n, jump=True), store)
                jump_target_calls += 2 * n if self.params.adjusted_jumps else 0
            else:
                jump_target_calls += split_flow_mh(run, flow, self.target, event_shape, base + K,
                                                   self.params.adjusted_jumps, run.stats.struct(jump=True))
                if store is not None:
                    store.add_dense(run.x[None])
            done = i + 1
            if show_progress:
                run.sync()
                bar.set_postfix_str(f'acc {int(run.stats.counters[hip.CNT_ACCEPTED])}/'
                                    f'{int(run.stats.counters[hip.CNT_ATTEMPTED])}')
        if pending_fit is not None:
            pending_fit.result()
        inner._cur_run = None
        calls, grads = inner._counts(n, K * done)
        out = JumpNFMCOutput(event_shape, kernel=self.kernel, store_samples=self.params.store_samples,
                             max_samples=getattr(self.params, 'max_samples', None))
        return run.finish(out, t0, n * done * (K + 1), store, n_divergences=inner._n_divergences,
                          n_target_calls=calls + jump_target_calls, n_target_gradient_calls=grads,
                          n_attempted_jumps=n * done)


def _make(inner_cls):
    class _Jump(JumpNFMC):
        def __init__(self, event_shape, target, kernel: NFMCKernel = None, params: JumpNFMCParameters = None,
                     inner_kernel: MCMCKernel = None, inner_params: MCMCParameters = None):
            super().__init__(event_shape, target, inner_cls(event_shape, target, inner_kernel, inner_params),
                             kernel, params)

    return _Jump


class JumpHMC(_make(HMC)):
    pass


class JumpUHMC(_make(UHMC)):
    pass


class JumpMALA(_make(MALA)):
    pass


class JumpULA(_make(ULA)):
    pass


class JumpMH(_make(MH)):
    pass
```

### nfmc_amd/samplers/mcmc.py

```python
import ctypes as C
import math
import os
import time
from copy import deepcopy
from dataclasses import dataclass
from typing import Any, Dict, Optional, Tuple, Union

import torch
from tqdm import tqdm

from .. import hip
from ..containers import MCMCKernel, MCMCOutput, MCMCParameters, Sampler
from ..tuning import DualAveraging, DualAveragingParams
from .common import Run, chunks, imd_tensor, progress, resolve_target


@dataclass
class MetropolisKernel(MCMCKernel):
    event_size: int
    inv_mass_diag: torch.Tensor = None
    step_size: float = 0.01
    da: DualAveraging = None
    da_params: DualAveragingParams = None

    def __post_init__(self):
        super().__post_init__()
        if self.inv_mass_diag is None:
            self.inv_mass_diag = torch.ones(self.event_size)
        else:
            self.inv_mass_diag = torch.as_tensor(self.inv_mass_diag, dtype=torch.float32)
            if tuple(self.inv_mass_diag.shape) != (self.event_size,):
                raise ValueError('inv_mass_diag must have event_size = %d entries, got shape %s'
                                 % (self.event_size, tuple(self.inv_mass_diag.shape)))
        if self.da_params is None:
            self.da_params = DualAveragingParams()
        if self.da is None:
            self.da = DualAveraging(self.step_size, self.da_params)


@dataclass
class MetropolisParameters(MCMCParameters):
    tune_inv_mass_diag: bool = True
    tune_step_size: bool = True
    adjustment: bool = True
    imd_adjustment: float = 1e-3
    tune_every: int = 1


class DeviceTuning:

    def __init__(self, sampler, run):
        k, p, da = sampler.kernel, sampler.params, sampler.kernel.da
        st = torch.zeros(int(hip.lib().nfmc_tune_state_doubles(run.d)), dtype=torch.float64)
        st[hip.TUNE_STEP_SIZE] = float(k.step_size)
        st[hip.TUNE_LOG_SMOOTH] = da.log_smooth
        st[hip.TUNE_ERROR_SUM] = da.error_sum
        st[hip.TUNE_ITERATION] = da.iteration
        st[hip.TUNE_ANCHOR] = da.anchor
        st[hip.TUNE_LOG_RAW] = da.log_raw if math.isfinite(da.log_raw) else 0.0
        st[hip.TUNE_TARGET] = da.params.target_acceptance_rate
        st[hip.TUNE_KAPPA] = da.params.kappa
        st[hip.TUNE_GAMMA] = da.params.gamma
        st[hip.TUNE_IMD_ADJUSTMENT] = p.imd_adjustment
        c0 = hip.tune_shift_offset(run.d)
        st[c0:c0 + run.d] = run.x.double().mean(0).float().double()
        self.state = st.to(run.dev)
        self.imd = k.inv_mass_diag.detach().to(run.dev, torch.float32).contiguous().clone()
        self.tune_step = bool(p.tune_step_size and p.adjustment)
        self.tune_imd = bool(p.tune_inv_mass_diag and run.n > 1)
        self.updates = 0

    def struct(self, every=0, n_steps=1):
        every = int(every) if every and every < n_steps else 0
        self.updates += -(-n_steps // every) if every else 1
        return hip.NfmcTune(hip.ptr(self.state, torch.float64), hip.ptr(self.imd), int(self.tune_step), int(self.tune_imd),
                            every, 0)

    def download(self, kernel):
        st = self.state.cpu()
        if self.tune_imd:
            kernel.inv_mass_diag = self.imd.cpu().to(kernel.inv_mass_diag.dtype)
        if self.tune_step and self.updates:
            da = kernel.da
            da.log_smooth, da.error_sum = float(st[hip.TUNE_LOG_SMOOTH]), float(st[hip.TUNE_ERROR_SUM])
            da.iteration, da.log_raw = int(round(float(st[hip.TUNE_ITERATION]))), float(st[hip.TUNE_LOG_RAW])
            kernel.step_size = float(st[hip.TUNE_STEP_SIZE])


@dataclass
class LangevinKernel(MetropolisKernel):
    event_size: int
    step_size: Optional[float] = None

    def __post_init__(self):
        if self.step_size is None:
            self.step_size = self.event_size ** (-1 / 3)
        super().__post_init__()

    def __repr__(self):
        return (f'log step: {math.log(self.step_size):.2f}, '
                f'mass norm: {torch.max(torch.abs(self.inv_mass_diag)):.2f}')


@dataclass
class LangevinParameters(MetropolisParameters):
    pass


@dataclass
class HMCKernel(MetropolisKernel):
    event_size: int
    n_leapfrog_steps: int = 20

    def __repr__(self):
        return (f'log step: {math.log(self.step_size):.2f}, '
                f'leapfrogs: {self.n_leapfrog_steps}, '
                f'mass norm: {torch.max(torch.abs(self.inv_mass_diag)):.2f}')


@dataclass
class HMCParameters(MetropolisParameters):
    pass


class TargetFailure(Exception):
    """The target raised ValueError: the reference's failure channel (langevin.py:111-114, hmc.py:117-120,
    mh.py:63-66): every chain rejects this step and the step counts as ONE divergence."""


def _guarded(fn, *args):
    try:
        return fn(*args)
    except hip.NfmcArgumentError:
        raise
    except ValueError as e:
        raise TargetFailure(str(e)) from e


def _value_and_grad(target, x, event_shape):
    with torch.enable_grad():
        xr = x.detach().reshape(x.shape[0], *event_shape).clone().requires_grad_(True)
        u = target(xr)
        g, = torch.autograd.grad(u.sum(), xr)
    return u.detach().reshape(-1).float().contiguous(), g.detach().reshape(x.shape).float().contiguous()


class MCMCSampler(Sampler):

    def __init__(self, event_shape, target, kernel: MCMCKernel, params: MCMCParameters,
                 data_transform=lambda v: v):
        super().__init__(event_shape, target, kernel, params)
        self.data_transform = data_transform

    @property
    def name(self):
        return "Generic MCMC"

    def propose(self, x: torch.Tensor) -> Tuple[torch.Tensor, torch.Tensor, int, int, int]:
        raise NotImplementedError

    def update_kernel(self, data: Dict[str, Any]):
        raise NotImplementedError

    def _launch(self, run: Run, pot, k, step0, samples, masks_out=None, log_ratio_out=None, jump=None, rng=None, tune=None):
        raise NotImplementedError

    def _counts(self, n, k):
        raise NotImplementedError

    def warmup(self, x0, show_progress: bool = True, time_limit_seconds=None) -> MCMCOutput:
        with torch.no_grad():
            warmup_copy = deepcopy(self)
        warmup_copy.params.tuning_mode()
        warmup_copy.params.n_iterations = self.params.n_warmup_iterations
        out = warmup_copy.sample(x0, show_progress=show_progress, time_limit_seconds=time_limit_seconds)
        self.kernel = warmup_copy.kernel
        new_params = warmup_copy.params
        new_params.n_iterations = self.params.n_iterations
        self.params = new_params
        self.params.sampling_mode()
        return out

    def sample(self, x0, show_progress: bool = True, time_limit_seconds=None) -> MCMCOutput:
        if self.params.tuning and int(getattr(self.params, 'tune_every', 1)) > hip.MAX_STEPS_PER_CALL:
            raise ValueError('tune_every must be at most %d, got %d'
                             % (hip.MAX_STEPS_PER_CALL, int(self.params.tune_every)))
        run = Run(self, x0)
        step0 = hip.WARMUP_STEP0 if self.params.tuning else 0
        n = run.n
        event_shape = run.event_shape
        out = MCMCOutput(event_shape, kernel=self.kernel, store_samples=self.params.store_samples,
                         max_samples=getattr(self.params, 'max_samples', None))
        out.statistics.data_transform = self.data_transform
        K = int(self.params.n_iterations)
        pot = resolve_target(self.target, event_shape, self.fuse, run.x, family='mcmc')
        store = run.sample_store(K)
        run.stats.zero_()
        self._n_divergences = 0
        t0 = time.time()
        done = 0
        label = f'{self.name} (tuning)' if self.params.tuning else self.name
        bar = progress(show_progress, total=K, desc=label)
        stepwise = self.params.tuning or pot is None
        limit = 1 if stepwise else (hip.MAX_STEPS_PER_CALL if time_limit_seconds is None and not show_progress else 32)
        tune = None
        if self.params.tuning:
            run.rounds = 10
        if (self.params.tuning and pot is not None and isinstance(self, MetropolisSampler)
                and (run.shard is None or run.shard.world == 1) and os.environ.get('NFMC_TUNE_DEVICE', '1') != '0'):
            tune = DeviceTuning(self, run)
            tune.every = max(1, int(getattr(self.params, 'tune_every', 1)))
            limit = hip.MAX_STEPS_PER_CALL if time_limit_seconds is None and not show_progress else max(32, tune.every)
            limit -= limit % tune.every
        while done < K:
            if run.time_is_up(t0, time_limit_seconds):
                break
            k = min(limit, K - done)
            if tune is not None:
                self._launch(run, pot, k, step0 + done, store, tune=tune)
            elif pot is not None:
                mask_buf = torch.empty(k, n, dtype=torch.uint8, device=run.dev) if self.params.tuning else None
                self._launch(run, pot, k, step0 + done, store, masks_out=mask_buf)
                mask = mask_buf[-1].bool() if mask_buf is not None else None
            else:
                mask = self._split_step(run, step0 + done, store)
            if self.params.tuning and tune is None:
                with torch.no_grad():
                    self.update_kernel({'x': run.x.reshape(n, *event_shape), 'mask': mask})
            done += k
            bar.update(k)
        bar.close()
        calls, grads = self._counts(n, done)
        run.finish(out, t0, n * done, store, n_target_calls=calls, n_target_gradient_calls=grads,
                   n_divergences=self._n_divergences)
        if tune is not None:
            tune.download(self.kernel)
        self._cur_run = None
        return out

    def _rejected_step(self, xf, n_calls, n_grads):
        n = xf.shape[0]
        self._last_log_ratio = torch.full((n,), -math.inf, dtype=torch.float32, device=xf.device)
        self._last_uniforms = None
        return xf, torch.zeros(n, dtype=torch.bool, device=xf.device), n_calls, n_grads, 1

    def _split_step(self, run: Run, step, sample_view):
        n, d = run.n, run.d
        self._cur_run, self._cur_step = run, step
        x_prime, mask_or_lr, n_calls, n_grads, n_divs = self.propose(run.x)
        self._n_divergences = getattr(self, '_n_divergences', 0) + int(n_divs)
        st = hip.NfmcSelectArgs()
        st.x, st.x_prime, st.n, st.d = hip.ptr(run.x), hip.ptr(x_prime), n, d
        st.n_carry = 0
        lr = self._last_log_ratio
        st.log_ratio = hip.ptr(lr) if lr is not None else None
        un = self._last_uniforms
        st.uniforms = hip.ptr(un) if un is not None else None
        st.rng = hip.make_rng(run.seed, run.chain_offset, step, rounds=run.rounds)
        st.rng_tag = hip.TAG_ACCEPT
        st.stats = run.stats.struct()
        mask = torch.empty(n, dtype=torch.uint8, device=run.dev)
        st.mask_out = hip.ptr(mask, torch.uint8)
        hip.check(hip.lib().nfmc_mh_accept_select_f32(C.byref(st), hip.stream()), 'nfmc_mh_accept_select_f32')
        if sample_view is not None:
            if hasattr(sample_view, 'add_dense'):
                sample_view.add_dense(run.x[None])
            else:
                sample_view[0].copy_(run.x)
        return mask.bool()


class MetropolisSampler(MCMCSampler):
    def update_kernel(self, data: Dict[str, Any]):
        x = data['x']
        mask = data['mask']
        shard = getattr(self, 'shard', None)
        sharded = shard is not None and shard.world > 1
        n_chains = x.shape[0]
        flat = x.flatten(1, -1)
        acc_rate = None
        if sharded:
            d = flat.shape[1]
            xd = flat.double()
            pack = torch.cat([xd.sum(0), (xd * xd).sum(0),
                              xd.new_tensor([float(n_chains), float(mask.sum()) if mask is not None else 0.0])])
            shard.all_reduce_sum_(pack)
            n_all = float(pack[2 * d])
            n_chains = int(round(n_all))
            var_all = ((pack[d:2 * d] - pack[:d] ** 2 / n_all) / max(n_all - 1.0, 1.0)).float()
            acc_rate = float(pack[2 * d + 1]) / n_all
        if n_chains > 1 and self.params.tune_inv_mass_diag:
            var = (var_all if sharded else torch.var(flat, dim=0)).to(self.kernel.inv_mass_diag)
            self.kernel.inv_mass_diag = (self.params.imd_adjustment * var
                                         + (1 - self.params.imd_adjustment) * self.kernel.inv_mass_diag)
        if self.params.tune_step_size and self.params.adjustment:
            if acc_rate is None:
                acc_rate = float(torch.mean(mask.float()))
            error = self.kernel.da_params.target_acceptance_rate - acc_rate
            self.kernel.da.step(error)
            self.kernel.step_size = self.kernel.da.value


class Langevin(MetropolisSampler):
    def __init__(self, event_shape, target, kernel: Optional[LangevinKernel] = None,
                 params: Optional[LangevinParameters] = None):
        if kernel is None:
            kernel = LangevinKernel(event_size=int(torch.prod(torch.as_tensor(event_shape))))
        if params is None:
            params = LangevinParameters()
        super().__init__(event_shape, target, kernel, params)

    @property
    def name(self):
        return 'LMC'

    def _counts(self, n, k):
        per = 2 * n if self.params.adjustment else n
        return per * k, per * k

    def _args(self, run, pot, k, step0, samples, masks_out=None, log_ratio_out=None, jump=None, rng=None, tune=None,
              attempted=None):
        a = hip.NfmcMalaArgs()
        a.x, a.n, a.d, a.n_steps = hip.ptr(run.x), run.n, run.d, k
        a.step_size = float(self.kernel.step_size)
        a.adjust = (1 if self.params.adjustment else 0) | (2 if getattr(self, 'random_walk', False) else 0)
        imd = tune.imd if tune is not None else imd_tensor(self.kernel, run.dev)
        a.inv_mass_diag = hip.ptr(imd)
        a.pot = pot.descriptor(run.dev)
        a.rng = rng if rng is not None else run.rng(step0, k, adjusted=self.params.adjustment)
        if tune is not None:
            a.stats = run.stats.struct()
            a.tune = tune.struct(getattr(tune, 'every', 0), k)
        else:
            a.stats = run.stats.struct(defer=True, attempted=run.n * k if attempted is None else attempted,
                                       jump_attempted=run.n if jump is not None else 0)
        a.samples = hip.store_struct(samples, k + (1 if jump is not None else 0))
        a.masks_out = hip.ptr(masks_out, torch.uint8) if masks_out is not None else None
        a.log_ratio_out = hip.ptr(log_ratio_out) if log_ratio_out is not None else None
        a.jump = C.pointer(jump) if jump is not None else None
        a._keep = imd
        return a

    def _launch(self, run, pot, k, step0, samples, **kw):
        a = self._args(run, pot, k, step0, samples, **kw)
        with run.timed('mala_steps'):
            hip.check(hip.lib().nfmc_mala_steps_f32(C.byref(a), hip.stream()), 'nfmc_mala_steps_f32')

    def propose(self, x):
        dev = hip.require_gpu()
        n = x.shape[0]
        xf = x.detach().to(dev, torch.float32).reshape(n, -1).contiguous()
        d = xf.shape[1]
        run = getattr(self, '_cur_run', None)
        step = getattr(self, '_cur_step', 0)
        seed = run.seed if run is not None else (self.seed or 0)
        off = run.chain_offset if run is not None else 0
        h = float(self.kernel.step_size)
        imd = imd_tensor(self.kernel, dev)
        lib = hip.lib()
        nz = un = None
        if run is not None and run.replay is not None:
            nz, _ = run.replay.take(1, with_uniforms=False)
        per = 2 * n if self.params.adjustment else n
        try:
            u, g = _guarded(_value_and_grad, self.target, xf, self.event_shape)
        except TargetFailure:
            return self._rejected_step(xf, per, per)
        x_prime = torch.empty_like(xf)
        rng = hip.make_rng(seed, off, step, nz, None, rounds=run.rounds if run is not None else 0)
        hip.check(lib.nfmc_langevin_propose_f32(hip.ptr(xf), hip.ptr(g), hip.ptr(imd), h, n, d, C.byref(rng),
                                                hip.ptr(x_prime), hip.stream()), 'nfmc_langevin_propose_f32')
        n_calls = n_grads = n
        self._last_log_ratio = None
        self._last_uniforms = None
        mask = torch.ones(n, dtype=torch.bool, device=dev)
        if self.params.adjustment:
            try:
                up, gp = _guarded(_value_and_grad, self.target, x_prime, self.event_shape)
            except TargetFailure:
                return self._rejected_step(xf, per, per)
            if nz is not None:
                un = run.replay.take_uniforms(1)
                self._last_uniforms = un[0].contiguous()
            lr = torch.empty(n, dtype=torch.float32, device=dev)
            hip.check(lib.nfmc_langevin_log_ratio_f32(hip.ptr(xf), hip.ptr(x_prime), hip.ptr(u), hip.ptr(up),
                                                      hip.ptr(g), hip.ptr(gp), hip.ptr(imd), h, n, d, hip.ptr(lr),
                                                      hip.stream()), 'nfmc_langevin_log_ratio_f32')
            self._last_log_ratio = lr
            n_calls += n
            n_grads += n
            if run is None:
                unif = torch.empty(n, dtype=torch.float32, device=dev)
                hip.check(lib.nfmc_philox_uniforms_f32(C.byref(rng), hip.TAG_ACCEPT, n, hip.ptr(unif), hip.stream()),
                          'nfmc_philox_uniforms_f32')
                mask = torch.log(unif) < lr
        return x_prime, mask, n_calls, n_grads, 0


class MALA(Langevin):
    def __init__(self, *args, **kwargs):
        super().__init__(*args, **kwargs)
        self.params.adjustment = True


class ULA(Langevin):
    def __init__(self, *args, **kwargs):
        super().__init__(*args, **kwargs)
        self.params.adjustment = False


@dataclass
class MHKernel(MetropolisKernel):
    event_size: int

    def __repr__(self):
        return (f'log step: {math.log(self.step_size):.2f}, '
                f'mass norm: {torch.max(torch.abs(self.inv_mass_diag)):.2f}')


@dataclass
class MHParameters(MetropolisParameters):
    imd_adjustment: float = 1e-5

    def __post_init__(self):
        self.tune_step_size = False
        self.tune_inv_mass_diag = True


class MH(Langevin):
    random_walk = True

    def __init__(self, event_shape, target, kernel: Optional[MHKernel] = None, params: Optional[MHParameters] = None):
        if kernel is None:
            kernel = MHKernel(event_size=int(torch.prod(torch.as_tensor(event_shape))))
        if params is None:
            params = MHParameters()
        MetropolisSampler.__init__(self, event_shape, target, kernel, params)

    @property
    def name(self):
        return "MH"

    def _counts(self, n, k):
        return (2 * n * k if self.params.adjustment else 0), 0

    def propose(self, x):
        dev = hip.require_gpu()
        n = x.shape[0]
        xf = x.detach().to(dev, torch.float32).reshape(n, -1).contiguous()
        d = xf.shape[1]
        run = getattr(self, '_cur_run', None)
        step = getattr(self, '_cur_step', 0)
        seed = run.seed if run is not None else (self.seed or 0)
        off = run.chain_offset if run is not None else 0
        replayed = run is not None and run.replay is not None
        if replayed:
            nz, _ = run.replay.take(1, with_uniforms=False)
            noise = nz[0]
        else:
            noise = torch.empty(n, d, dtype=torch.float32, device=dev)
            rng = hip.make_rng(seed, off, step, rounds=run.rounds if run is not None else 0)
            hip.check(hip.lib().nfmc_philox_normals_f32(C.byref(rng), hip.TAG_NOISE, n, d, hip.ptr(noise), hip.stream()),
                      'nfmc_philox_normals_f32')
        x_prime = (xf + noise * self.kernel.inv_mass_diag.to(dev, torch.float32)[None]).contiguous()
        self._last_log_ratio = None
        self._last_uniforms = None
        mask = torch.ones(n, dtype=torch.bool, device=dev)
        n_calls = 0
        if self.params.adjustment:
            try:
                with torch.no_grad():
                    lr = (_guarded(self.target, xf.reshape(n, *self.event_shape)).reshape(-1)
                          - _guarded(self.target, x_prime.reshape(n, *self.event_shape)).reshape(-1))
            except TargetFailure:
                return self._rejected_step(xf, 2 * n, 0)
            self._last_log_ratio = lr.float().contiguous()
            if replayed:
                self._last_uniforms = run.replay.take_uniforms(1)[0].contiguous()
            n_calls = 2 * n
            if run is None:
                unif = torch.empty(n, dtype=torch.float32, device=dev)
                rng = hip.make_rng(seed, off, step, rounds=run.rounds if run is not None else 0)
                hip.check(hip.lib().nfmc_philox_uniforms_f32(C.byref(rng), hip.TAG_ACCEPT, n, hip.ptr(unif), hip.stream()),
                          'nfmc_philox_uniforms_f32')
                mask = torch.log(unif) < self._last_log_ratio
        return x_prime, mask, n_calls, 0, 0


class RandomWalk(MH):
    def __init__(self, *args, **kwargs):
        super().__init__(*args, **kwargs)
        self.params.adjustment = False


class HMC(MetropolisSampler):
    def __init__(self, event_shape, target, kernel: Optional[HMCKernel] = None,
                 params: Optional[HMCParameters] = None):
        if kernel is None:
            kernel = HMCKernel(event_size=int(torch.prod(torch.as_tensor(event_shape))))
        if params is None:
            params = HMCParameters()
        super().__init__(event_shape, target, kernel, params)

    @property
    def name(self):
        return "HMC"

    def _counts(self, n, k):
        grads = 2 * self.kernel.n_leapfrog_steps * n
        calls = grads + (2 * n if self.params.adjustment else 0)
        return calls * k, grads * k

    def _args(self, run, pot, k, step0, samples, masks_out=None, log_ratio_out=None, jump=None, rng=None, tune=None,
              attempted=None):
        a = hip.NfmcHmcArgs()
        a.x, a.n, a.d, a.n_steps = hip.ptr(run.x), run.n, run.d, k
        a.step_size = float(self.kernel.step_size)
        a.n_leapfrog = int(self.kernel.n_leapfrog_steps)
        a.adjust = 1 if self.params.adjustment else 0
        imd = tune.imd if tune is not None else imd_tensor(self.kernel, run.dev)
        a.inv_mass_diag = hip.ptr(imd)
        a.pot = pot.descriptor(run.dev)
        a.rng = rng if rng is not None else run.rng(step0, k, adjusted=self.params.adjustment)
        if tune is not None:
            a.stats = run.stats.struct()
            a.tune = tune.struct(getattr(tune, 'every', 0), k)
        else:
            a.stats = run.stats.struct(defer=True, attempted=run.n * k if attempted is None else attempted,
                                       jump_attempted=run.n if jump is not None else 0)
        a.samples = hip.store_struct(samples, k + (1 if jump is not None else 0))
        a.masks_out = hip.ptr(masks_out, torch.uint8) if masks_out is not None else None
        a.log_ratio_out = hip.ptr(log_ratio_out) if log_ratio_out is not None else None
        a.jump = C.pointer(jump) if jump is not None else None
        a._keep = imd
        return a

    def _launch(self, run, pot, k, step0, samples, **kw):
        a = self._args(run, pot, k, step0, samples, **kw)
        with run.timed('hmc_steps'):
            hip.check(hip.lib().nfmc_hmc_steps_f32(C.byref(a), hip.stream()), 'nfmc_hmc_steps_f32')

    def propose(self, x):
        dev = hip.require_gpu()
        n = x.shape[0]
        xf = x.detach().to(dev, torch.float32).reshape(n, -1).contiguous()
        d = xf.shape[1]
        run = getattr(self, '_cur_run', None)
        step = getattr(self, '_cur_step', 0)
        seed = run.seed if run is not None else (self.seed or 0)
        off = run.chain_offset if run is not None else 0
        h = float(self.kernel.step_size)
        m = self.kernel.inv_mass_diag.to(dev, torch.float32)
        lib = hip.lib()
        replayed = run is not None and run.replay is not None
        if replayed:
            nz, _ = run.replay.take(1, with_uniforms=False)
            noise = nz[0]
        else:
            noise = torch.empty(n, d, dtype=torch.float32, device=dev)
            rng = hip.make_rng(seed, off, step, rounds=run.rounds if run is not None else 0)
            hip.check(lib.nfmc_philox_normals_f32(C.byref(rng), hip.TAG_NOISE, n, d, hip.ptr(noise), hip.stream()),
                      'nfmc_philox_normals_f32')
        p = noise * (1 / m.sqrt())
        p0 = p
        q = xf
        L = self.kernel.n_leapfrog_steps
        n_grads = 2 * L * n
        n_calls = n_grads + (2 * n if self.params.adjustment else 0)
        merged = bool(getattr(self, 'one_evaluation_per_position', False))
        u0 = u1 = None
        try:
            if merged:
                u0, g = _guarded(_value_and_grad, self.target, q, self.event_shape)
                u1 = u0
                for _ in range(L):
                    p = p - h / 2 * g
                    q = q + h * (p * m)
                    u1, g = _guarded(_value_and_grad, self.target, q, self.event_shape)
                    p = p - h / 2 * g
            else:
                for _ in range(L):
                    p = p - h / 2 * _guarded(_value_and_grad, self.target, q, self.event_shape)[1]
                    q = q + h * (p * m)
                    p = p - h / 2 * _guarded(_value_and_grad, self.target, q, self.event_shape)[1]
        except TargetFailure:
            return self._rejected_step(xf, n_calls, n_grads)
        n_calls = n_grads
        self._last_log_ratio = None
        self._last_uniforms = None
        mask = torch.ones(n, dtype=torch.bool, device=dev)
        if self.params.adjustment:
            try:
                with torch.no_grad():
                    if not merged:
                        u0 = _guarded(self.target, xf.reshape(n, *self.event_shape)).reshape(-1)
                        u1 = _guarded(self.target, q.reshape(n, *self.event_shape)).reshape(-1)
                    h0 = u0.reshape(-1) + 0.5 * (p0 ** 2 * m).sum(-1)
                    h1 = u1.reshape(-1) + 0.5 * (p ** 2 * m).sum(-1)
            except TargetFailure:
                return self._rejected_step(xf, n_grads + 2 * n, n_grads)
            self._last_log_ratio = (h0 - h1).float().contiguous()
            if replayed:
                self._last_uniforms = run.replay.take_uniforms(1)[0].contiguous()
            n_calls += 2 * n
            if run is None:
                unif = torch.empty(n, dtype=torch.float32, device=dev)
                rng = hip.make_rng(seed, off, step, rounds=run.rounds if run is not None else 0)
                hip.check(lib.nfmc_philox_uniforms_f32(C.byref(rng), hip.TAG_ACCEPT, n, hip.ptr(unif), hip.stream()),
                          'nfmc_philox_uniforms_f32')
                mask = torch.log(unif) < self._last_log_ratio
        return q.contiguous(), mask, n_calls, n_grads, 0


class UHMC(HMC):
    def __init__(self, *args, **kwargs):
        super().__init__(*args, **kwargs)
        self.params.adjustment = False
```

Before: 29.53 billion.

## Cut host-side setup: fuse initial copy, wider stats fold, pinned fetch and upload

The sampler kernels can now read starting rows straight from the caller's tensor through a new x_in pointer, which avoids a device clone before the first step. The stats fold uses a wider kernel spread over more blocks. Final totals are copied into a pinned host buffer asynchronously and waited on with an event, and flow weight blobs are uploaded through a ring of pinned staging slots. The aim is to shrink per-call host and launch overhead, at the cost of more global state, mutex-guarded per-device buffers, and extra invariants tying x_in to x.

```diff
diff --git a/include/nfmc_hip.h b/include/nfmc_hip.h
--- a/include/nfmc_hip.h
+++ b/include/nfmc_hip.h
@@ -71,6 +71,15 @@
 int nfmc_stats_fold_f32(const NfmcStats* stats, int32_t d, uint64_t attempted, unsigned long long* jump_counters,
                         uint64_t jump_attempted, nfmc_stream_t stream);
 
+#define NFMC_TOTALS_MAX_WORDS 4096
+int nfmc_stats_fold_fetch_f32(const NfmcStats* stats, int32_t d, uint64_t attempted, unsigned long long* jump_counters,
+                              uint64_t jump_attempted, const void* totals, int32_t words, nfmc_stream_t stream);
+int nfmc_stats_totals_wait(const void** host);
+
+#define NFMC_UPLOAD_SLOTS 4
+#define NFMC_UPLOAD_SLOT_BYTES (256 * 1024)
+int nfmc_upload_async(void* dst, const void* src, int64_t bytes, nfmc_stream_t stream);
+
 typedef struct {
     int32_t d;
     int32_t n_coupling;
@@ -157,6 +166,7 @@
     float* log_ratio_out;
     const NfmcJumpTail* jump;
     NfmcTune tune;
+    const float* x_in;
 } NfmcMalaArgs;
 
 int nfmc_mala_steps_f32(const NfmcMalaArgs* args, nfmc_stream_t stream);
@@ -179,6 +189,7 @@
     float* log_ratio_out;
     const NfmcJumpTail* jump;
     NfmcTune tune;
+    const float* x_in;
 } NfmcHmcArgs;
 
 int nfmc_hmc_steps_f32(const NfmcHmcArgs* args, nfmc_stream_t stream);
diff --git a/nfmc_amd/csrc/misc_kernels.hip b/nfmc_amd/csrc/misc_kernels.hip
--- a/nfmc_amd/csrc/misc_kernels.hip
+++ b/nfmc_amd/csrc/misc_kernels.hip
@@ -1,4 +1,9 @@
 #include "common.hpp"
+
+#include <stdlib.h>
+#include <string.h>
+
+#include <mutex>
 
 namespace nfmc {
 
@@ -159,6 +164,67 @@
     }
 }
 
+constexpr int kFoldCols = 4, kFoldChains = 4 * kFinishSlices, kFoldBlock = kFoldCols * kFoldChains, kFoldBatch = 8;
+
+__global__ void __launch_bounds__(kFoldBlock) stats_fold_wide_kernel(double* __restrict__ scratch, int nblocks, int dp, int d,
+                                                                     NfmcStats st, unsigned long long attempted,
+                                                                     unsigned long long* jump_counters,
+                                                                     unsigned long long jump_attempted) {
+    __shared__ double acc[kFoldChains][kFoldCols];
+    __shared__ double part[kFinishSlices][kFoldCols];
+    const int width = 2 * dp + kStatTail;
+    const int col = threadIdx.x % kFoldCols, chain = threadIdx.x / kFoldCols;
+    const int slice = chain % kFinishSlices, a = chain / kFinishSlices;
+    const int t = blockIdx.x * kFoldCols + col;
+    double p = 0.0;
+    if (t < width) {
+        const int groups = nblocks > slice + 3 * kFinishSlices ? (nblocks - slice - 3 * kFinishSlices + 4 * kFinishSlices - 1) / (4 * kFinishSlices) : 0;
+        double* row = scratch + (size_t)(slice + kFinishSlices * a) * width + t;
+        const size_t step = (size_t)4 * kFinishSlices * width;
+        int j = 0;
+        for (; j + kFoldBatch <= groups; j += kFoldBatch) {
+            double v[kFoldBatch];
+#pragma unroll
+            for (int k = 0; k < kFoldBatch; ++k) v[k] = row[(size_t)k * step];
+#pragma unroll
+            for (int k = 0; k < kFoldBatch; ++k) row[(size_t)k * step] = 0.0;
+#pragma unroll
+            for (int k = 0; k < kFoldBatch; ++k) p += v[k];
+            row += kFoldBatch * step;
+        }
+        for (; j < groups; ++j, row += step) p += take<true>(row);
+        if (a == 0)
+            for (int b = slice + 4 * kFinishSlices * groups; b < nblocks; b += kFinishSlices)
+                p += take<true>(scratch + (size_t)b * width + t);
+    }
+    acc[chain][col] = p;
+    __syncthreads();
+    if (a == 0)
+        part[slice][col] = (acc[slice][col] + acc[kFinishSlices + slice][col]) +
+                           (acc[2 * kFinishSlices + slice][col] + acc[3 * kFinishSlices + slice][col]);
+    __syncthreads();
+    if (chain == 0 && t < width) {
+        double s = 0.0;
+#pragma unroll
+        for (int k = 0; k < kFinishSlices; ++k) s += part[k][col];
+        if (t < dp) {
+            if (t < d) st.sum_x[t] += s;
+        } else if (t < 2 * dp) {
+            if (t - dp < d) st.sum_x2[t - dp] += s;
+        } else if (t == 2 * dp) {
+            st.counters[NFMC_CNT_ACCEPTED] += (unsigned long long)(s + 0.5);
+            st.counters[NFMC_CNT_ATTEMPTED] += attempted;
+        } else if (t == 2 * dp + 1) {
+            st.counters[NFMC_CNT_NONFINITE] += (unsigned long long)(s + 0.5);
+        } else if (t == 2 * dp + 2 && jump_counters) {
+            jump_counters[NFMC_CNT_ACCEPTED] += (unsigned long long)(s + 0.5);
+            jump_counters[NFMC_CNT_ATTEMPTED] += jump_attempted;
+        } else if (t == 2 * dp + 3 && jump_counters) {
+            jump_counters[NFMC_CNT_NONFINITE] += (unsigned long long)(s + 0.5);
+        }
+    }
+}
+
 static int grid_for(int64_t work_items) {
     int64_t g = (work_items + kBlock - 1) / kBlock;
     return (int)(g < 1 ? 1 : (g > kMaxGrid ? kMaxGrid : g));
@@ -205,6 +271,14 @@
     return NFMC_OK;
 }
 
+static bool fold_wide() {
+    static const bool on = [] {
+        const char* e = getenv("NFMC_FOLD_WIDE");
+        return !(e && atoi(e) == 0);
+    }();
+    return on;
+}
+
 extern "C" int nfmc_stats_fold_f32(const NfmcStats* stats, int32_t d, uint64_t attempted,
                                    unsigned long long* jump_counters, uint64_t jump_attempted, nfmc_stream_t stream) {
     if (!stats || !stats->sum_x || !stats->sum_x2 || !stats->counters || !stats->scratch) return NFMC_EINVAL;
@@ -212,10 +286,114 @@
     if (d > 1024) return NFMC_ESHAPE;
     const int dp = padded_d(d);
     if (stats->scratch_bytes < stats_scratch_doubles(dp) * (int64_t)sizeof(double)) return NFMC_ESCRATCH;
-    hipLaunchKernelGGL(stats_finish_kernel<true>, dim3(stats_finish_grid(dp)), dim3(kFinishBlock), 0, (hipStream_t)stream,
-                       stats->scratch, kMaxGrid, dp, (int)d, *stats, (unsigned long long)attempted, jump_counters,
-                       (unsigned long long)jump_attempted);
-    NFMC_HIP_CHECK_LAUNCH();
+    if (fold_wide()) {
+        const int grid = (2 * dp + kStatTail + kFoldCols - 1) / kFoldCols;
+        hipLaunchKernelGGL(stats_fold_wide_kernel, dim3(grid), dim3(kFoldBlock), 0, (hipStream_t)stream, stats->scratch,
+                           kMaxGrid, dp, (int)d, *stats, (unsigned long long)attempted, jump_counters,
+                           (unsigned long long)jump_attempted);
+    } else {
+        hipLaunchKernelGGL(stats_finish_kernel<true>, dim3(stats_finish_grid(dp)), dim3(kFinishBlock), 0, (hipStream_t)stream,
+                           stats->scratch, kMaxGrid, dp, (int)d, *stats, (unsigned long long)attempted, jump_counters,
+                           (unsigned long long)jump_attempted);
+    }
+    NFMC_HIP_CHECK_LAUNCH();
+    return NFMC_OK;
+}
+
+namespace {
+constexpr int kPinDevices = 64;
+struct PinnedTotals {
+    void* host = nullptr;
+    hipEvent_t landed = nullptr;
+    bool pending = false;
+};
+struct UploadSlot {
+    void* host = nullptr;
+    hipEvent_t copied = nullptr;
+    bool used = false;
+};
+struct UploadRing {
+    UploadSlot slot[NFMC_UPLOAD_SLOTS];
+    int next = 0;
+};
+std::mutex pin_mu;
+PinnedTotals pinned_totals[kPinDevices];
+UploadRing upload_ring[kPinDevices];
+
+int current_device(int* dev) {
+    if (hipError_t e = hipGetDevice(dev)) return (int)e;
+    return (*dev < 0 || *dev >= kPinDevices) ? NFMC_EUNSUPPORTED : NFMC_OK;
+}
+}
+
+extern "C" int nfmc_stats_fold_fetch_f32(const NfmcStats* stats, int32_t d, uint64_t attempted,
+                                         unsigned long long* jump_counters, uint64_t jump_attempted, const void* totals,
+                                         int32_t words, nfmc_stream_t stream) {
+    if (!totals || words <= 0 || words > NFMC_TOTALS_MAX_WORDS) return NFMC_EINVAL;
+    int dev = 0;
+    if (int rc = current_device(&dev)) return rc;
+    std::lock_guard<std::mutex> lock(pin_mu);
+    PinnedTotals& pt = pinned_totals[dev];
+    if (!pt.host) {
+        void* h = nullptr;
+        if (hipError_t e = hipHostMalloc(&h, (size_t)NFMC_TOTALS_MAX_WORDS * 8, hipHostMallocDefault)) return (int)e;
+        if (hipError_t e = hipEventCreateWithFlags(&pt.landed, hipEventDisableTiming)) {
+            (void)hipHostFree(h);
+            return (int)e;
+        }
+        pt.host = h;
+    }
+    if (int rc = nfmc_stats_fold_f32(stats, d, attempted, jump_counters, jump_attempted, stream)) return rc;
+    hipStream_t st = (hipStream_t)stream;
+    if (hipError_t e = hipMemcpyAsync(pt.host, totals, (size_t)words * 8, hipMemcpyDeviceToHost, st)) return (int)e;
+    if (hipError_t e = hipEventRecord(pt.landed, st)) return (int)e;
+    pt.pending = true;
+    return NFMC_OK;
+}
+
+extern "C" int nfmc_stats_totals_wait(const void** host) {
+    if (!host) return NFMC_EINVAL;
+    int dev = 0;
+    if (int rc = current_device(&dev)) return rc;
+    hipEvent_t ev = nullptr;
+    {
+        std::lock_guard<std::mutex> lock(pin_mu);
+        PinnedTotals& pt = pinned_totals[dev];
+        if (!pt.pending) return NFMC_EINVAL;
+        ev = pt.landed;
+        *host = pt.host;
+    }
+    if (hipError_t e = hipEventSynchronize(ev)) return (int)e;
+    return NFMC_OK;
+}
+
+extern "C" int nfmc_upload_async(void* dst, const void* src, int64_t bytes, nfmc_stream_t stream) {
+    if (!dst || !src || bytes <= 0) return NFMC_EINVAL;
+    int dev = 0;
+    if (int rc = current_device(&dev)) return rc;
+    hipStream_t st = (hipStream_t)stream;
+    std::lock_guard<std::mutex> lock(pin_mu);
+    UploadRing& ring = upload_ring[dev];
+    for (int64_t off = 0; off < bytes; off += NFMC_UPLOAD_SLOT_BYTES) {
+        const size_t piece = (size_t)(bytes - off < NFMC_UPLOAD_SLOT_BYTES ? bytes - off : NFMC_UPLOAD_SLOT_BYTES);
+        UploadSlot& s = ring.slot[ring.next];
+        if (!s.host) {
+            void* h = nullptr;
+            if (hipError_t e = hipHostMalloc(&h, NFMC_UPLOAD_SLOT_BYTES, hipHostMallocDefault)) return (int)e;
+            if (hipError_t e = hipEventCreateWithFlags(&s.copied, hipEventDisableTiming)) {
+                (void)hipHostFree(h);
+                return (int)e;
+            }
+            s.host = h;
+        }
+        if (s.used)
+            if (hipError_t e = hipEventSynchronize(s.copied)) return (int)e;
+        memcpy(s.host, (const char*)src + off, piece);
+        if (hipError_t e = hipMemcpyAsync((char*)dst + off, s.host, piece, hipMemcpyHostToDevice, st)) return (int)e;
+        if (hipError_t e = hipEventRecord(s.copied, st)) return (int)e;
+        s.used = true;
+        ring.next = (ring.next + 1) % NFMC_UPLOAD_SLOTS;
+    }
     return NFMC_OK;
 }
 
diff --git a/nfmc_amd/csrc/sampler_impl.hpp b/nfmc_amd/csrc/sampler_impl.hpp
--- a/nfmc_amd/csrc/sampler_impl.hpp
+++ b/nfmc_amd/csrc/sampler_impl.hpp
@@ -233,7 +233,7 @@
         const bool active = row < n;
         const uint32_t gchain = (uint32_t)(a.rng.chain_offset + (uint64_t)row);
         float x[CPL];
-        load_row<CPL, LPC, FAST>(a.x, row, d, g, active, x);
+        load_row<CPL, LPC, FAST>(a.x_in ? a.x_in : a.x, row, d, g, active, x);
         shift.init(a.tune, g, d, active);
         AcceptLnU<LPC, RR, !LEAN> au(accept_slab, g);
         StoreCursor keep(a.samples);
@@ -376,7 +376,7 @@
         const bool active = row < n;
         const uint32_t gchain = (uint32_t)(a.rng.chain_offset + (uint64_t)row);
         float x[CPL];
-        load_row<CPL, LPC, FAST>(a.x, row, d, g, active, x);
+        load_row<CPL, LPC, FAST>(a.x_in ? a.x_in : a.x, row, d, g, active, x);
         shift.init(a.tune, g, d, active);
         AcceptLnU<LPC, RR> au(accept_slab, g);
         StoreCursor keep(a.samples);
diff --git a/nfmc_amd/csrc/sampler_kernels.hip b/nfmc_amd/csrc/sampler_kernels.hip
--- a/nfmc_amd/csrc/sampler_kernels.hip
+++ b/nfmc_amd/csrc/sampler_kernels.hip
@@ -33,7 +33,8 @@
     if (a->d > 1024) return NFMC_ESHAPE;
     if (!(a->step_size > 0.f)) return NFMC_EINVAL;
     if (int rc = check_potential(a->pot, a->d, PotFamily::kRegister)) return rc;
-    if (((uintptr_t)a->x & 3u) != 0) return NFMC_EALIGN;
+    if (((uintptr_t)a->x & 3u) != 0 || ((uintptr_t)a->x_in & 3u) != 0) return NFMC_EALIGN;
+    if (a->x_in == a->x) return NFMC_EINVAL;
     if (!store_ok(a->samples)) return NFMC_EINVAL;
     if (!rng_rounds_ok(a->rng, true)) return NFMC_EINVAL;
     if ((a->rng.replay_normals == nullptr) != (a->rng.replay_uniforms == nullptr) && (a->adjust & 1)) return NFMC_EINVAL;
@@ -54,7 +55,7 @@
 template <class Args>
 static bool fast_path(const Args* a, const Cfg& c) {
     return a->d == c.cpl * c.lpc && a->inv_mass_diag == nullptr && a->pot.a == nullptr && a->pot.b == nullptr &&
-           (a->pot.kind != NFMC_POT_QUADRATIC || a->pot.b_scalar == 0.f) && aligned16(a->x) &&
+           (a->pot.kind != NFMC_POT_QUADRATIC || a->pot.b_scalar == 0.f) && aligned16(a->x) && aligned16(a->x_in) &&
            (!a->samples.base || aligned16(a->samples.base));
 }
 
@@ -308,6 +309,7 @@
             const int k = total - s0 < every ? total - s0 : every;
             Args b = a;
             b.n_steps = k;
+            if (s0 > 0) b.x_in = nullptr;
             b.rng.step0 = a.rng.step0 + (uint32_t)s0;
             if (a.rng.replay_normals) b.rng.replay_normals = a.rng.replay_normals + (int64_t)s0 * a.n * a.d;
             if (a.rng.replay_uniforms) b.rng.replay_uniforms = a.rng.replay_uniforms + (int64_t)s0 * a.n;
@@ -384,7 +386,7 @@
     const int64_t n = inner.n;
     const int d = inner.d, K = r.n_inner, T = r.n_outer;
     if (T <= 0 || K <= 0 || r.n_parts < 1 || r.n_parts > NFMC_JUMP_RUN_MAX_PARTS) return NFMC_EINVAL;
-    if (!inner.x || n <= 0 || d <= 0 || jump.x != inner.x || jump.n != n || jump.flow.d != d || !jump.logq) return NFMC_EINVAL;
+    if (!inner.x || inner.x_in == inner.x || n <= 0 || d <= 0 || jump.x != inner.x || jump.n != n || jump.flow.d != d || !jump.logq) return NFMC_EINVAL;
     if (jump.rng.seed != inner.rng.seed || jump.rng.chain_offset != inner.rng.chain_offset || jump.rng.rounds != inner.rng.rounds)
         return NFMC_EINVAL;
     if (inner.jump || inner.tune.state || inner.samples.base || jump.samples.base || inner.masks_out || jump.masks_out ||
@@ -438,6 +440,7 @@
             for (int off = 0; off < K && !rc; off += NFMC_MAX_STEPS_PER_CALL) {
                 Args b = inner;
                 b.x = inner.x + lo * d;
+                b.x_in = (inner.x_in && i == 0 && off == 0) ? inner.x_in + lo * d : nullptr;
                 b.n = np;
                 b.n_steps = K - off < NFMC_MAX_STEPS_PER_CALL ? K - off : NFMC_MAX_STEPS_PER_CALL;
                 b.rng.chain_offset = inner.rng.chain_offset + (uint64_t)lo;
diff --git a/nfmc_amd/flows.py b/nfmc_amd/flows.py
--- a/nfmc_amd/flows.py
+++ b/nfmc_amd/flows.py
@@ -180,7 +180,7 @@
             ea0, ea1 = self.layers[0], self.layers[-1]
             for k, t in enumerate((ea0.log_scale, ea0.shift, ea1.log_scale, ea1.shift)):
                 flat[ea_off + k * d4:ea_off + k * d4 + d] = t.detach().float().cpu().numpy()
-            blob = torch.from_numpy(flat).to(device)
+            blob = hip.upload(flat, device)
             keep = [blob] + [blob[ea_off + k * d4:ea_off + k * d4 + d] for k in range(4)]
         st = hip.NfmcRealNVP(d, self.n_coupling, H, nhl, float(self.min_scale), int(self.n_bins), hip.ptr(keep[1]),
                              hip.ptr(keep[2]), hip.ptr(keep[3]), hip.ptr(keep[4]), hip.ptr(keep[0]), stride,
diff --git a/nfmc_amd/hip.py b/nfmc_amd/hip.py
--- a/nfmc_amd/hip.py
+++ b/nfmc_amd/hip.py
@@ -20,6 +20,8 @@
 CNT_ACCEPTED, CNT_ATTEMPTED, CNT_NONFINITE, CNT_WORDS = 0, 1, 2, 4
 MAX_STEPS_PER_CALL = 512
 IMH_PARALLEL_MAX_STEPS = 65536
+TOTALS_MAX_WORDS = 4096
+UPLOAD_SLOTS, UPLOAD_SLOT_BYTES = 4, 256 * 1024
 
 c_fp = C.c_void_p
 NFMC_ABI_VERSION = 4
@@ -86,7 +88,7 @@
                 ('step_size', C.c_float), ('adjust', C.c_int32), ('inv_mass_diag', c_fp),
                 ('pot', NfmcPotential), ('rng', NfmcRng), ('stats', NfmcStats),
                 ('samples', NfmcSampleStore), ('masks_out', c_fp), ('log_ratio_out', c_fp), ('jump', C.POINTER(NfmcJumpTail)),
-                ('tune', NfmcTune)]
+                ('tune', NfmcTune), ('x_in', c_fp)]
 
 
 class NfmcHmcArgs(C.Structure):
@@ -94,7 +96,7 @@
                 ('step_size', C.c_float), ('n_leapfrog', C.c_int32), ('adjust', C.c_int32), ('reserved', C.c_int32),
                 ('inv_mass_diag', c_fp), ('pot', NfmcPotential), ('rng', NfmcRng), ('stats', NfmcStats),
                 ('samples', NfmcSampleStore), ('masks_out', c_fp), ('log_ratio_out', c_fp), ('jump', C.POINTER(NfmcJumpTail)),
-                ('tune', NfmcTune)]
+                ('tune', NfmcTune), ('x_in', c_fp)]
 
 
 class NfmcFlowMhArgs(C.Structure):
@@ -202,6 +204,10 @@
                                               C.c_int32, c_fp, c_fp]),
     ('nfmc_moments_update_f32', C.c_int, [c_fp, C.c_int64, C.c_int32, C.POINTER(NfmcStats), c_fp]),
     ('nfmc_stats_fold_f32', C.c_int, [C.POINTER(NfmcStats), C.c_int32, C.c_uint64, c_fp, C.c_uint64, c_fp]),
+    ('nfmc_stats_fold_fetch_f32', C.c_int, [C.POINTER(NfmcStats), C.c_int32, C.c_uint64, c_fp, C.c_uint64, c_fp, C.c_int32,
+                                            c_fp]),
+    ('nfmc_stats_totals_wait', C.c_int, [C.POINTER(C.c_void_p)]),
+    ('nfmc_upload_async', C.c_int, [c_fp, c_fp, C.c_int64, c_fp]),
     ('nfmc_philox_normals_f32', C.c_int, [C.POINTER(NfmcRng), C.c_int32, C.c_int64, C.c_int32, c_fp, c_fp]),
     ('nfmc_philox_uniforms_f32', C.c_int, [C.POINTER(NfmcRng), C.c_int32, C.c_int64, c_fp, c_fp]),
     ('nfmc_flow_fit_supported_f32', C.c_int, [C.POINTER(NfmcRealNVP)]),
@@ -282,6 +288,21 @@
     return torch.device('cuda', torch.cuda.current_device())
 
 
+def legacy(item) -> bool:
+    return item in os.environ.get('NFMC_CALL_LEGACY', '').split(',')
+
+
+def upload(array, device):
+    if legacy('d'):
+        return torch.from_numpy(array).to(device)
+    assert array.dtype.name == 'float32' and array.flags['C_CONTIGUOUS']
+    out = torch.empty(array.shape, dtype=torch.float32, device=device)
+    if array.size:
+        check(lib().nfmc_upload_async(C.c_void_p(out.data_ptr()), C.c_void_p(array.ctypes.data), array.nbytes, stream()),
+              'nfmc_upload_async')
+    return out
+
+
 def ptr(t, dtype=torch.float32):
     if t is None:
         return None
@@ -315,19 +336,39 @@
 
 class DeviceStats:
 
-    def __init__(self, d, device):
+    _pool = {}
+
+    def __init__(self, d, device, _buffers=None):
         self.d = d
         self.device = device
-        self._buf = torch.zeros(2 * d + 2 * CNT_WORDS, dtype=torch.float64, device=device)
+        if _buffers is not None:
+            self._buf, self.scratch = _buffers
+            self._buf.zero_()
+        else:
+            self._buf = torch.zeros(2 * d + 2 * CNT_WORDS, dtype=torch.float64, device=device)
         self._sum_x = self._buf[:d]
         self._sum_x2 = self._buf[d:2 * d]
         self._counters = self._buf[2 * d:2 * d + CNT_WORDS].view(torch.int64)
         self._jump_counters = self._buf[2 * d + CNT_WORDS:].view(torch.int64)
-        nbytes = int(lib().nfmc_stats_scratch_bytes(d))
-        self.scratch = torch.zeros(nbytes // 8, dtype=torch.float64, device=device)
+        if _buffers is None:
+            nbytes = int(lib().nfmc_stats_scratch_bytes(d))
+            self.scratch = torch.zeros(nbytes // 8, dtype=torch.float64, device=device)
         self._pending = False
         self._attempted = 0
         self._jump_attempted = 0
+
+    @classmethod
+    def acquire(cls, d, device):
+        free = cls._pool.get((str(device), d))
+        return cls(d, device, _buffers=free.pop() if free else None)
+
+    def release(self):
+        if self._pending or self._buf is None or legacy('3'):
+            return
+        free = self._pool.setdefault((str(self.device), self.d), [])
+        if len(free) < 2:
+            free.append((self._buf, self.scratch))
+        self._buf = self.scratch = self._sum_x = self._sum_x2 = self._counters = self._jump_counters = None
 
     def _raw(self, defer=0, tail_slot=0, counters=None):
         return NfmcStats(ptr(self._sum_x, torch.float64), ptr(self._sum_x2, torch.float64),
@@ -346,15 +387,21 @@
             self._jump_attempted += int(jump_attempted)
         return self._raw(1, 2 if jump else 0)
 
-    def fold(self):
+    def fold(self, fetch=False):
         if not self._pending:
-            return
+            return False
         st = self._raw()
-        check(lib().nfmc_stats_fold_f32(C.byref(st), self.d, self._attempted, ptr(self._jump_counters, torch.int64),
-                                        self._jump_attempted, stream()), 'nfmc_stats_fold_f32')
+        if fetch:
+            check(lib().nfmc_stats_fold_fetch_f32(C.byref(st), self.d, self._attempted, ptr(self._jump_counters, torch.int64),
+                                                  self._jump_attempted, ptr(self._buf, torch.float64), self._buf.numel(),
+                                                  stream()), 'nfmc_stats_fold_fetch_f32')
+        else:
+            check(lib().nfmc_stats_fold_f32(C.byref(st), self.d, self._attempted, ptr(self._jump_counters, torch.int64),
+                                            self._jump_attempted, stream()), 'nfmc_stats_fold_f32')
         self._pending = False
         self._attempted = 0
         self._jump_attempted = 0
+        return fetch
 
     @property
     def sum_x(self):
@@ -377,8 +424,14 @@
         return self._jump_counters
 
     def host_totals(self):
-        self.fold()
-        h = self._buf.cpu()
+        words = self._buf.numel()
+        if words <= TOTALS_MAX_WORDS and not legacy('c') and self.fold(fetch=True):
+            host = C.c_void_p()
+            check(lib().nfmc_stats_totals_wait(C.byref(host)), 'nfmc_stats_totals_wait')
+            h = torch.frombuffer((C.c_double * words).from_address(host.value), dtype=torch.float64).clone()
+        else:
+            self.fold()
+            h = self._buf.cpu()
         d = self.d
         return (h[:d], h[d:2 * d], h[2 * d:2 * d + CNT_WORDS].view(torch.int64),
                 h[2 * d + CNT_WORDS:].view(torch.int64))
diff --git a/nfmc_amd/samplers/common.py b/nfmc_amd/samplers/common.py
--- a/nfmc_amd/samplers/common.py
+++ b/nfmc_amd/samplers/common.py
@@ -70,8 +70,15 @@
         else:
             self.chain_offset = 0
             self.n_global = self.n
-        self.x = x0.detach().to(self.dev, torch.float32).reshape(self.n, self.d).contiguous().clone()
-        self.stats = hip.DeviceStats(self.d, self.dev)
+        x0 = x0.detach()
+        self._x_in = None
+        if (x0.is_cuda and x0.device == self.dev and x0.dtype == torch.float32 and x0.is_contiguous() and self.n > 0
+                and x0.data_ptr() % 16 == 0 and not hip.legacy('a')):
+            self._x_in = x0.reshape(self.n, self.d)
+            self._x = torch.empty(self.n, self.d, dtype=torch.float32, device=self.dev)
+        else:
+            self._x = x0.to(self.dev, torch.float32).reshape(self.n, self.d).contiguous().clone()
+        self.stats = hip.DeviceStats.acquire(self.d, self.dev)
         if sampler.seed is None:
             seed = int(torch.randint(0, 2 ** 62, ()).item())
             if shard is not None:
@@ -93,6 +100,23 @@
         if tk:
             self.kernel_events = []
 
+    @property
+    def x(self):
+        if self._x_in is not None:
+            self._x.copy_(self._x_in)
+            self._x_in = None
+        return self._x
+
+    @property
+    def start(self):
+        return self._x_in if self._x_in is not None else self._x
+
+    def fused_rows(self):
+        return self._x, self._x_in
+
+    def rows_filled(self):
+        self._x_in = None
+
     def timed(self, label):
         return _Timed(self, label)
 
@@ -127,8 +151,11 @@
                                  getattr(p, 'max_samples', None))
 
     def finish(self, out, t0, n_moments, store=None, **counters):
-        last_sample = self.x.reshape(self.n, *self.event_shape).clone()
+        last_sample = self.x.reshape(self.n, *self.event_shape)
+        if hip.legacy('3'):
+            last_sample = last_sample.clone()
         sum_x, sum_x2, cnt, jc = self.stats.host_totals()
+        self.stats.release()
         st = out.statistics
         device = {'n_accepted_trajectories': int(cnt[hip.CNT_ACCEPTED]),
                   'n_attempted_trajectories': int(cnt[hip.CNT_ATTEMPTED])}
diff --git a/nfmc_amd/samplers/jump.py b/nfmc_amd/samplers/jump.py
--- a/nfmc_amd/samplers/jump.py
+++ b/nfmc_amd/samplers/jump.py
@@ -91,10 +91,10 @@
 
 
 def flow_mh_args(run: Run, flow, pot, logq, k, step0, cached, adjusted, stats_struct, samples=None, masks_out=None,
-                 log_ratio_out=None):
+                 log_ratio_out=None, rows=None):
     a = hip.NfmcFlowMhArgs()
     st, _keep = flow.bijection.packed(run.dev)
-    a.x, a.logq, a.n, a.n_steps = hip.ptr(run.x), hip.ptr(logq), run.n, k
+    a.x, a.logq, a.n, a.n_steps = hip.ptr(run.x if rows is None else rows), hip.ptr(logq), run.n, k
     a.logq_cached = 1 if cached else 0
     a.adjusted = 1 if adjusted else 0
     a.flow = st
@@ -124,13 +124,14 @@
     k = min(n_inner, hip.MAX_STEPS_PER_CALL)
     ia = inner._args(run, pot, k, step0, None, attempted=n * n_inner * n_outer)
     ja = flow_mh_args(run, flow, pot, logq, 1, step0 + n_inner, False, adjusted,
-                      run.stats.struct(defer=True, attempted=n * n_outer, jump=True))
+                      run.stats.struct(defer=True, attempted=n * n_outer, jump=True), rows=run.fused_rows()[0])
     r = hip.NfmcJumpRun()
     r.inner_kind = hip.INNER_HMC if isinstance(ia, hip.NfmcHmcArgs) else hip.INNER_MALA
     r.inner = C.cast(C.pointer(ia), C.c_void_p)
     r.jump = C.pointer(ja)
     r.n_outer, r.n_inner, r.n_parts = n_outer, n_inner, n_parts
     hip.check(hip.lib().nfmc_jump_run_f32(C.byref(r), hip.stream()), 'nfmc_jump_run_f32')
+    run.rows_filled()
 
 
 def _flow_mh_probe_args(run: Run, flow, pot, logq, adjusted):
@@ -295,7 +296,7 @@
         T, K = int(self.params.n_iterations), int(inner.params.n_iterations)
         off = (False, 'never')
         pot = resolve_target(self.target, event_shape,
-                             'never' if (self.fuse in off or getattr(inner, 'fuse', 'auto') in off) else 'auto', run.x,
+                             'never' if (self.fuse in off or getattr(inner, 'fuse', 'auto') in off) else 'auto', run.start,
                              family='mcmc')
         fused = pot is not None and flow_is_native(flow) and pot.fused_in('flow_mh')
         tail_ok = (self.fuse_jump_tail and fused and pot.jump_tail_ok() and flow_fits_jump_tail(flow) and not self.params.fit_nf
diff --git a/nfmc_amd/samplers/mcmc.py b/nfmc_amd/samplers/mcmc.py
--- a/nfmc_amd/samplers/mcmc.py
+++ b/nfmc_amd/samplers/mcmc.py
@@ -193,7 +193,7 @@
                          max_samples=getattr(self.params, 'max_samples', None))
         out.statistics.data_transform = self.data_transform
         K = int(self.params.n_iterations)
-        pot = resolve_target(self.target, event_shape, self.fuse, run.x, family='mcmc')
+        pot = resolve_target(self.target, event_shape, self.fuse, run.start, family='mcmc')
         store = run.sample_store(K)
         run.stats.zero_()
         self._n_divergences = 0
@@ -321,7 +321,8 @@
     def _args(self, run, pot, k, step0, samples, masks_out=None, log_ratio_out=None, jump=None, rng=None, tune=None,
               attempted=None):
         a = hip.NfmcMalaArgs()
-        a.x, a.n, a.d, a.n_steps = hip.ptr(run.x), run.n, run.d, k
+        rows, rows_in = run.fused_rows()
+        a.x, a.x_in, a.n, a.d, a.n_steps = hip.ptr(rows), hip.ptr(rows_in), run.n, run.d, k
         a.step_size = float(self.kernel.step_size)
         a.adjust = (1 if self.params.adjustment else 0) | (2 if getattr(self, 'random_walk', False) else 0)
         imd = tune.imd if tune is not None else imd_tensor(self.kernel, run.dev)
@@ -345,6 +346,7 @@
         a = self._args(run, pot, k, step0, samples, **kw)
         with run.timed('mala_steps'):
             hip.check(hip.lib().nfmc_mala_steps_f32(C.byref(a), hip.stream()), 'nfmc_mala_steps_f32')
+        run.rows_filled()
 
     def propose(self, x):
         dev = hip.require_gpu()
@@ -514,7 +516,8 @@
     def _args(self, run, pot, k, step0, samples, masks_out=None, log_ratio_out=None, jump=None, rng=None, tune=None,
               attempted=None):
         a = hip.NfmcHmcArgs()
-        a.x, a.n, a.d, a.n_steps = hip.ptr(run.x), run.n, run.d, k
+        rows, rows_in = run.fused_rows()
+        a.x, a.x_in, a.n, a.d, a.n_steps = hip.ptr(rows), hip.ptr(rows_in), run.n, run.d, k
         a.step_size = float(self.kernel.step_size)
         a.n_leapfrog = int(self.kernel.n_leapfrog_steps)
         a.adjust = 1 if self.params.adjustment else 0
@@ -539,6 +542,7 @@
         a = self._args(run, pot, k, step0, samples, **kw)
         with run.timed('hmc_steps'):
             hip.check(hip.lib().nfmc_hmc_steps_f32(C.byref(a), hip.stream()), 'nfmc_hmc_steps_f32')
+        run.rows_filled()
 
     def propose(self, x):
         dev = hip.require_gpu()
```

Result: slower. 28.88 billion (-2.2%).
